# TACC/GraviT

Measured on AMD Instinct MI355X. Metric: Mrays/s (primary+shadow) at 1080p, 10M-tri scene, higher is better.
Workload: dtype f32; 1 GPU; soup-10000000: 10000000 random triangles (Philox seed 12345, half-extent 0.005), 1920x1080, eye (.5,.5,3)->(.5,.5,.5), fov 30deg, 1 point light at the eye, depth 1 (primary + 1 shadow ray), AO off; scheduler=image, 1 domain, harness=native, settle_frames=0, normal_mode=flat

## Files before the change

### gravit_amd/csrc/api.hip

```cpp
#include <atomic>
#include <chrono>
#include <cmath>
#include <cstdlib>
#include <condition_variable>
#include <functional>
#include <mutex>
#include <new>
#include <thread>

#include "gvt_internal.h"

size_t trav_spill_ints_per_thread();
int trav_block_threads();
void abi_pool_destroy(void *);

static thread_local std::string g_err;
static Ctx g_default_ctx;
static thread_local Ctx *tl_ctx = nullptr;
#define g_ctx (gctx())
Ctx &gctx() { return tl_ctx ? *tl_ctx : g_default_ctx; }

void set_error(const char *fmt, ...) {
  char buf[1024];
  va_list ap;
  va_start(ap, fmt);
  vsnprintf(buf, sizeof buf, fmt, ap);
  va_end(ap);
  g_err = buf;
}
extern "C" const char *gvt_hip_last_error(void) { return g_err.c_str(); }

static int ctx_setup(Ctx &C, int device) {
  int count = 0;
  if (hipGetDeviceCount(&count) != hipSuccess || count <= 0) { set_error("no HIP device visible"); return GVT_HIP_ERR_NODEVICE; }
  if (device < 0 || device >= count) { set_error("device %d out of range (%d visible)", device, count); return GVT_HIP_ERR_INVALID; }
  HIPCHK(hipSetDevice(device));
  hipDeviceProp_t prop;
  HIPCHK(hipGetDeviceProperties(&prop, device));
  if (std::strncmp(prop.gcnArchName, "gfx950", 6) != 0) {
    set_error("device %d is %s; this library carries gfx950 (MI355X) code objects only", device, prop.gcnArchName);
    return GVT_HIP_ERR_NODEVICE;
  }
  C.device = device;
  C.n_cu = prop.multiProcessorCount;
  HIPCHK(hipStreamCreateWithFlags(&C.own_stream, hipStreamNonBlocking));
  C.stream = C.own_stream;
  C.trav_blocks = std::max(C.n_cu, C.n_cu * 32 / (trav_block_threads() / 64));
  const size_t spill_ints = (size_t)C.trav_blocks * trav_block_threads() * trav_spill_ints_per_thread();
  HIPCHK(hipMalloc((void **)&C.d_spill, spill_ints * sizeof(int)));
  HIPCHK(hipMalloc((void **)&C.d_counters, CW_COUNT * sizeof(unsigned)));
  HIPCHK(hipMemset(C.d_counters, 0, CW_COUNT * sizeof(unsigned)));
  HIPCHK(hipHostMalloc((void **)&C.h_pinned, 64 * sizeof(unsigned), hipHostMallocDefault));
  std::memset(C.h_pinned, 0, 64 * sizeof(unsigned));
  C.ready = true;
  return 0;
}

static void drain_events();
static void warm_up() {
  if (getenv("GVT_HIP_NO_WARMUP")) return;
  const size_t nT = 2048;
  std::vector<float> v(nT * 9);
  std::vector<int32_t> t(nT * 3);
  uint32_t r = 12345u;
  for (size_t i = 0; i < nT; i++) {
    float c[3];
    for (int k = 0; k < 3; k++) { r = r * 1664525u + 1013904223u; c[k] = (float)(r >> 8) * (1.0f / 16777216.0f); }
    for (int j = 0; j < 3; j++)
      for (int k = 0; k < 3; k++) { r = r * 1664525u + 1013904223u; v[9 * i + 3 * j + k] = c[k] + ((float)(r >> 8) * (1.0f / 16777216.0f) - 0.5f) * 0.02f; }
    t[3 * i] = (int32_t)(3 * i); t[3 * i + 1] = (int32_t)(3 * i + 1); t[3 * i + 2] = (int32_t)(3 * i + 2);
  }
  gvt_hip_mesh *m = gvt_hip_mesh_create(v.data(), nT * 3, t.data(), nT, nullptr, nullptr, nullptr, 0, nullptr, nullptr);
  if (m) {
    float org[64 * 3], dir[64 * 3];
    gvt_hip_hit hits[64];
    int32_t occ[64];
    for (int i = 0; i < 64; i++) { org[3 * i] = (float)(i % 8) / 8.f; org[3 * i + 1] = (float)(i / 8) / 8.f; org[3 * i + 2] = 2.f; dir[3 * i] = 0.f; dir[3 * i + 1] = 0.f; dir[3 * i + 2] = -1.f; }
    gvt_hip_intersect(m, org, dir, 64, 0.f, hits);
    gvt_hip_occluded(m, org, dir, 64, 0.f, occ);
    gvt_hip_mesh_destroy(m);
  }
  Ctx &C = g_default_ctx;
  hipStreamSynchronize(C.stream);
  drain_events();
  C.stats = gvt_hip_stats{};
  set_error("%s", "");
}

extern "C" int gvt_hip_init(int device) {
  Ctx &C = g_default_ctx;
  if (C.ready && C.device == device) { if (!tl_ctx) HIPCHK(hipSetDevice(device)); return 0; }
  if (C.ready) { set_error("gvt_hip_init: already initialised on device %d", C.device); return GVT_HIP_ERR_INVALID; }
  const int rc = ctx_setup(C, device);
  if (!rc && !tl_ctx) warm_up();
  return rc;
}

extern "C" gvt_hip_ctx *gvt_hip_ctx_create(int device) {
  Ctx *C = new Ctx();
  if (ctx_setup(*C, device) != 0) { delete C; return nullptr; }
  return (gvt_hip_ctx *)C;
}
extern "C" int gvt_hip_ctx_make_current(gvt_hip_ctx *c) {
  tl_ctx = (Ctx *)c;
  Ctx &C = gctx();
  if (C.ready) HIPCHK(hipSetDevice(C.device));
  return 0;
}
extern "C" void gvt_hip_ctx_destroy(gvt_hip_ctx *c) {
  Ctx *C = (Ctx *)c;
  if (!C) return;
  if (tl_ctx == C) tl_ctx = nullptr;
  if (C->ready) {
    hipSetDevice(C->device);
    hipStreamSynchronize(C->stream);
    for (auto &p : C->pending) { hipEventDestroy(p.a); hipEventDestroy(p.b); }
    for (auto e : C->event_pool) hipEventDestroy(e);
    if (C->abi_qin) gvt_hip_queue_destroy(C->abi_qin);
    if (C->abi_qout) gvt_hip_queue_destroy(C->abi_qout);
    abi_pool_destroy(C->abi_pool); C->abi_pool = nullptr;
    for (Ctx *L : C->abi_lanes) gvt_hip_ctx_destroy((gvt_hip_ctx *)L);
    C->abi_lanes.clear();
    hipSetDevice(C->device);
    for (int k = 0; k < SCRATCH_COUNT; k++) if (C->scratch[k]) hipFree(C->scratch[k]);
    hipFree(C->d_spill); hipFree(C->d_counters); hipHostFree(C->h_pinned);
    if (C->h_wire) hipHostFree(C->h_wire);
    if (C->wire_ev) hipEventDestroy(C->wire_ev);
    hipStreamDestroy(C->own_stream);
  }
  delete C;
}

int ensure_init() {
  if (gctx().ready) return 0;
  return gvt_hip_init(0);
}

extern "C" int gvt_hip_set_stream(void *s) {
  if (ensure_init()) return GVT_HIP_ERR_NODEVICE;
  HIPCHK(hipStreamSynchronize(g_ctx.stream));
  g_ctx.stream = s ? (hipStream_t)s : g_ctx.own_stream;
  return 0;
}
extern "C" int gvt_hip_synchronize(void) {
  if (ensure_init()) return GVT_HIP_ERR_NODEVICE;
  HIPCHK(hipStreamSynchronize(g_ctx.stream));
  return 0;
}

void *scratch_get(ScratchSlot slot, size_t bytes) {
  Ctx &C = g_ctx;
  if (bytes <= C.scratch_bytes[slot] && C.scratch[slot]) return C.scratch[slot];
  hipStreamSynchronize(C.stream);
  if (C.scratch[slot]) hipFree(C.scratch[slot]);
  size_t want = bytes + bytes / 4 + 4096;
  C.scratch[slot] = nullptr;
  C.scratch_bytes[slot] = 0;
  if (hipMalloc(&C.scratch[slot], want) != hipSuccess) { set_error("scratch hipMalloc(%zu) failed", want); return nullptr; }
  C.scratch_bytes[slot] = want;
  return C.scratch[slot];
}

void scratch_release(ScratchSlot slot) {
  Ctx &C = g_ctx;
  if (!C.scratch[slot]) return;
  hipStreamSynchronize(C.stream);
  hipFree(C.scratch[slot]);
  C.scratch[slot] = nullptr;
  C.scratch_bytes[slot] = 0;
}

ProfScope::ProfScope(int c) : cls(c) {
  Ctx &C = g_ctx;
  if (!C.profile || (C.profile == 2 && c != KC_CLOSEST && c != KC_ANY && c != KC_LONG) || (C.profile == 3 && c != KC_CLOSEST) || (C.profile == 4 && c != KC_ANY)) return;
  auto take = [&]() {
    hipEvent_t e;
    if (!C.event_pool.empty()) { e = C.event_pool.back(); C.event_pool.pop_back(); }
    else hipEventCreate(&e);
    return e;
  };
  a = take(); b = take();
  hipEventRecord(a, C.stream);
}
ProfScope::~ProfScope() {
  Ctx &C = g_ctx;
  if (!a) return;
  hipEventRecord(b, C.stream);
  C.pending.push_back({ a, b, cls });
}
static void drain_events() {
  Ctx &C = g_ctx;
  for (auto &p : C.pending) {
    hipEventSynchronize(p.b);
    float ms = 0.f;
    hipEventElapsedTime(&ms, p.a, p.b);
    double *slot[KC_COUNT] = { &C.stats.ms_closest, &C.stats.ms_any, &C.stats.ms_shade, &C.stats.ms_convert, &C.stats.ms_shuffle,
                               &C.stats.ms_camera, &C.stats.ms_build, &C.stats.ms_sort, &C.stats.ms_long };
    *slot[p.cls] += ms;
    C.event_pool.push_back(p.a);
    C.event_pool.push_back(p.b);
  }
  C.pending.clear();
}
extern "C" int gvt_hip_profile(int enable) {
  if (ensure_init()) return GVT_HIP_ERR_NODEVICE;
  drain_events();
  g_ctx.profile = enable < 0 ? 0 : enable;
  return 0;
}
extern "C" int gvt_hip_stats_read(gvt_hip_stats *out) {
  if (!out) { set_error("stats_read: null"); return GVT_HIP_ERR_INVALID; }
  if (ensure_init()) return GVT_HIP_ERR_NODEVICE;
  HIPCHK(hipStreamSynchronize(g_ctx.stream));
  drain_events();
  *out = g_ctx.stats;
  return 0;
}
extern "C" int gvt_hip_stats_reset(void) {
  if (ensure_init()) return GVT_HIP_ERR_NODEVICE;
  drain_events();
  g_ctx.stats = gvt_hip_stats{};
  return 0;
}

namespace {
struct KnobDef { const char *name; int Knobs::*field; int lo, hi; bool shipped; };
const KnobDef g_knobs[] = {
  { "skip_known", &Knobs::skip_known, 0, 1, true },           { "frame_timing", &Knobs::frame_timing, 0, 1, true },
  { "term_sink", &Knobs::term_sink, 0, 1, true },
  { "sort_rays", &Knobs::sort_rays, 0, 1, true },             { "leaf_max", &Knobs::leaf_max, 1, 4, true },
  { "long_steps", &Knobs::long_steps, 0, 1 << 20, true },     { "small_rays", &Knobs::small_rays, 0, 1 << 30, true },
  { "finish_rays", &Knobs::finish_rays, 0, 1 << 30, true },   { "round_room_mb", &Knobs::round_room_mb, 0, 1 << 30, true },
  { "abi_lanes", &Knobs::abi_lanes_n, 0, 8, true },           { "abi_chunk", &Knobs::abi_chunk, 16384, 1 << 30, true },
  { "inject_fail_tick", &Knobs::inject_fail_tick, -1, 1 << 30, true },
  { "long_min_rays", &Knobs::long_min_rays, 0, 1 << 30, true }, { "long_auto", &Knobs::long_auto, 0, 1, true },
  { "finish_auto", &Knobs::finish_auto, 0, 1, true },
  { "payload_overlap_kb", &Knobs::payload_overlap_kb, 0, 1 << 30, true },
  { "packet", &Knobs::packet, 0, 2, true },                   { "packet_sah_max", &Knobs::packet_sah_max, 0, 1 << 30, true },
  { "packet_min_rays", &Knobs::packet_min_rays, 0, 1 << 30, true },
  { "shadow_order", &Knobs::shadow_order, 0, 1, true },       { "shadow_order_min_rays", &Knobs::shadow_order_min_rays, 0, 1 << 30, true },
  { "xcd_stripes", &Knobs::xcd_stripes, 0, 1, true },           { "early_deposit", &Knobs::early_deposit, 0, 1, true },

  { "inline_kb", &Knobs::inline_kb, 0, 1024, true },          { "comm_cus", &Knobs::comm_cus, 0, 128, true },
  { "comm_stream", &Knobs::comm_stream, 0, 1, true },         { "spec_ticks", &Knobs::spec_ticks, 0, 1, true },
  { "finish_clusters", &Knobs::finish_clusters, 0, 1, true }, { "hop_local", &Knobs::hop_local, 0, 3, true },
  { "occluder_chunk", &Knobs::occluder_chunk, 0, 1 << 24, true },
  { "blocks_per_cu", &Knobs::blocks_per_cu, 1, 8, false },    { "blocks_per_cu_closest", &Knobs::blocks_per_cu_closest, 0, 8, false },
  { "refill_min", &Knobs::refill_min, 1, 64, false },         { "inner_min", &Knobs::inner_min, 1, 64, false },
  { "share", &Knobs::share, 0, 1, false },                    { "share_min_rays", &Knobs::share_min_rays, 0, 1 << 30, false },
  { "sort_gather", &Knobs::sort_gather, 0, 1, false },        { "sort_bits", &Knobs::sort_bits, 8, 32, false },
  { "long_steps_drain", &Knobs::long_steps_drain, 0, 1 << 20, false }, { "long_save", &Knobs::long_save, 0, 1, false },
  { "lean_frame", &Knobs::lean_frame, 0, 1, false },          { "report_poll", &Knobs::report_poll, 0, 1, false },
  { "first_round_async", &Knobs::first_round_async, 0, 1, false }, { "wave_single", &Knobs::wave_single, 0, 1, false },
  { "shadow_direct", &Knobs::shadow_direct, 0, 1, false },    { "top_ordered", &Knobs::top_ordered, 0, 1, false },
  { "top_lds", &Knobs::top_lds, 0, 1, false },                { "camera_tile", &Knobs::camera_tile, 0, 8, false },
  { "abi_pipe_min", &Knobs::abi_pipe_min, 0, 1 << 30, false },
  { "shadow_cls_lo", &Knobs::shadow_cls_lo, 0, 255, false },  { "shadow_cls_shift", &Knobs::shadow_cls_shift, 0, 6, false },
};
}

extern "C" int gvt_hip_set_option(const char *name, int value) {
  if (!name) { set_error("set_option: null name"); return GVT_HIP_ERR_INVALID; }
  if (!std::strcmp(name, "defaults")) { static_cast<Knobs &>(g_ctx) = Knobs{}; return 0; }
  for (const KnobDef &k : g_knobs) {
    if (std::strcmp(name, k.name)) continue;
    if (value < k.lo || value > k.hi) { set_error("set_option: %s must be %d..%d", name, k.lo, k.hi); return GVT_HIP_ERR_INVALID; }
    if (!std::strcmp(name, "camera_tile") && value != 0 && value != 8) { set_error("camera_tile: 0 or 8"); return GVT_HIP_ERR_INVALID; }
#ifndef GVT_EXPERIMENTS
    if (!k.shipped && value != Knobs{}.*(k.field)) {
      set_error("set_option: %s=%d needs the experiments build of the library (libgvt_hip_exp.so); the shipped library carries its measured-best value %d", name, value,
                Knobs{}.*(k.field));
      return GVT_HIP_ERR_INVALID;
    }
#endif
    static_cast<Knobs &>(g_ctx).*(k.field) = value;
    return 0;
  }
  set_error("set_option: unknown option '%s'", name);
  return GVT_HIP_ERR_INVALID;
}

static void default_material(gvt_hip_material *m) {
  std::memset(m, 0, sizeof *m);
  m->type = 0;
  m->kd[0] = m->kd[1] = m->kd[2] = .5f;
  m->ks[0] = m->ks[1] = m->ks[2] = .5f;
  m->alpha = 1.f;
  m->eta[0] = .19f; m->eta[1] = 1.45f; m->eta[2] = 1.50f;
  m->k[0] = 3.06f; m->k[1] = 2.40f; m->k[2] = 1.88f;
  m->roughness = 0.05f;
}

static void generate_normals(const float *verts, size_t nV, const int32_t *tris, size_t nT, std::vector<float> &normals) {
  normals.assign(nV * 3, 0.0f);
  for (size_t i = 0; i < nT; i++) {
    int I = tris[3 * i], J = tris[3 * i + 1], K = tris[3 * i + 2];
    V3 a = ld3(verts + 3 * I), b = ld3(verts + 3 * J), c = ld3(verts + 3 * K);
    V3 u = sub3(b, a), v = sub3(c, a), n;
    n.x = u.y * v.z - u.z * v.y;
    n.y = u.z * v.x - u.x * v.z;
    n.z = u.x * v.y - u.y * v.x;
    n = norm3(n);
    int idx[3] = { I, J, K };
    for (int k = 0; k < 3; k++) {
      float *d = &normals[3 * idx[k]];
      d[0] += n.x; d[1] += n.y; d[2] += n.z;
    }
  }
  for (size_t i = 0; i < nV; i++) {
    V3 n = norm3(ld3(&normals[3 * i]));
    normals[3 * i] = n.x; normals[3 * i + 1] = n.y; normals[3 * i + 2] = n.z;
  }
}

template <typename T> static bool upload(T **dst, const T *src, size_t n) {
  *dst = nullptr;
  if (hipMalloc((void **)dst, sizeof(T) * (n ? n : 1)) != hipSuccess) return false;
  if (n && hipMemcpy(*dst, src, sizeof(T) * n, hipMemcpyHostToDevice) != hipSuccess) return false;
  return true;
}

extern "C" gvt_hip_mesh *gvt_hip_mesh_create(const float *verts, size_t nV, const int32_t *tris, size_t nT, const float *vnormals,
                                             const float *vcolors, const gvt_hip_material *materials, size_t nMat,
                                             const int32_t *face_mat, const gvt_hip_material *mesh_mat) {
  if (ensure_init()) return nullptr;
  if ((nV && !verts) || (nT && !tris)) { set_error("mesh_create: null vertex/triangle array"); return nullptr; }
  if (nT >= (1u << 28)) { set_error("mesh_create: %zu triangles exceed the 2^28 leaf-slot encoding", nT); return nullptr; }
  for (size_t i = 0; i < nT * 3; i++)
    if (tris[i] < 0 || (size_t)tris[i] >= nV) { set_error("mesh_create: triangle %zu references vertex %d (nV=%zu)", i / 3, tris[i], nV); return nullptr; }
  if (face_mat)
    for (size_t i = 0; i < nT; i++)
      if (face_mat[i] >= 0 && (size_t)face_mat[i] >= nMat) { set_error("mesh_create: face_mat[%zu]=%d out of range", i, face_mat[i]); return nullptr; }
  gvt_hip_mesh *M = new gvt_hip_mesh();
  M->nV = nV; M->nT = nT; M->nMat = materials ? nMat : 0;
  if (mesh_mat) M->mesh_mat = *mesh_mat; else default_material(&M->mesh_mat);
  std::vector<float> gen;
  const float *nrm = vnormals;
  if (!nrm) { generate_normals(verts, nV, tris, nT, gen); nrm = gen.data(); }
  bool ok = upload(&M->d_verts, verts, nV * 3) && upload(&M->d_tris, tris, nT * 3) && upload(&M->d_normals, nrm, nV * 3);
  if (ok && vcolors) ok = upload(&M->d_vcolors, vcolors, nV * 3);
  if (ok && M->nMat) ok = upload(&M->d_materials, materials, M->nMat);
  if (ok && face_mat && M->nMat) ok = upload(&M->d_face_mat, face_mat, nT);
  if (!ok) { set_error("mesh_create: device upload failed (%s)", hipGetErrorString(hipGetLastError())); gvt_hip_mesh_destroy(M); return nullptr; }
  if (build_lbvh(M) != 0) { gvt_hip_mesh_destroy(M); return nullptr; }
  return M;
}

extern "C" void gvt_hip_mesh_destroy(gvt_hip_mesh *M) {
  if (!M) return;
  if (g_ctx.ready) hipStreamSynchronize(g_ctx.stream);
  hipFree(M->d_verts); hipFree(M->d_tris); hipFree(M->d_normals); hipFree(M->d_vcolors); hipFree(M->d_materials);
  hipFree(M->d_face_mat); hipFree(M->d_nodes); hipFree(M->d_tri); hipFree(M->d_slot_of); hipFree(M->d_nodes4); hipFree(M->d_nodes4c);
  refit_tables_free(M);
  delete M;
}

extern "C" int gvt_hip_mesh_update_vertices(gvt_hip_mesh *M, const float *verts, size_t nV, const float *vnormals, uint32_t flags, float *ms_out) {
  if (ensure_init()) return GVT_HIP_ERR_NODEVICE;
  if (!M) { set_error("mesh_update_vertices: null mesh"); return GVT_HIP_ERR_INVALID; }
  if (flags & ~GVT_HIP_UPDATE_DEVICE) { set_error("mesh_update_vertices: unknown flags 0x%x", flags); return GVT_HIP_ERR_INVALID; }
  if (nV != M->nV) { set_error("mesh_update_vertices: %zu vertices given, the mesh has %zu (topology changes need a new mesh)", nV, M->nV); return GVT_HIP_ERR_INVALID; }
  if (nV && !verts) { set_error("mesh_update_vertices: null vertex array"); return GVT_HIP_ERR_INVALID; }
  Ctx &C = g_ctx;
  hipStream_t st = C.stream;
  const hipMemcpyKind kind = (flags & GVT_HIP_UPDATE_DEVICE) ? hipMemcpyDeviceToDevice : hipMemcpyHostToDevice;
  if (nV) {
    HIPCHK(hipMemcpyAsync(M->d_verts, verts, sizeof(float) * 3 * nV, kind, st));
    if (vnormals) HIPCHK(hipMemcpyAsync(M->d_normals, vnormals, sizeof(float) * 3 * nV, kind, st));
  }
  hipEvent_t e0, e1;
  HIPCHK(hipEventCreate(&e0));
  if (hipEventCreate(&e1) != hipSuccess) { hipEventDestroy(e0); set_error("mesh_update_vertices: hipEventCreate failed"); return GVT_HIP_ERR_DEVICE; }
  int rc = hipEventRecord(e0, st) == hipSuccess ? 0 : GVT_HIP_ERR_DEVICE;
  if (!rc && nV && !vnormals) rc = regen_normals(M);
  if (!rc) rc = refit_lbvh(M);
  float ms = 0.f;
  if (!rc && (hipEventRecord(e1, st) != hipSuccess || hipEventSynchronize(e1) != hipSuccess || hipEventElapsedTime(&ms, e0, e1) != hipSuccess)) {
    set_error("mesh_update_vertices: %s", hipGetErrorString(hipGetLastError()));
    rc = GVT_HIP_ERR_DEVICE;
  }
  hipStreamSynchronize(st);
  hipEventDestroy(e0); hipEventDestroy(e1);
  if (!rc && ms_out) *ms_out = ms;
  return rc;
}

extern "C" int gvt_hip_mesh_get_info(const gvt_hip_mesh *M, gvt_hip_mesh_info *o) {
  if (!M || !o) { set_error("mesh_get_info: null"); return GVT_HIP_ERR_INVALID; }
  std::memset(o, 0, sizeof *o);
  o->n_tris = M->nT; o->n_verts = M->nV; o->n_nodes = M->nNodes; o->n_leaves = M->nLeaves;
  for (int k = 0; k < 3; k++) { o->bbox_lo[k] = M->lo[k]; o->bbox_hi[k] = M->hi[k]; }
  o->build_ms = M->build_ms; o->max_leaf = M->leaf_max; o->packet = M->packet_ok ? 1u : 0u; o->sah_inner = M->sah_inner;
  o->bytes_nodes = M->nNodes * sizeof(BvhNode) + M->nNodes4 * 64; o->bytes_tris = M->nT * 64;
  return 0;
}
extern "C" int gvt_hip_mesh_get_normals(const gvt_hip_mesh *M, float *out) {
  if (!M || !out) { set_error("mesh_get_normals: null"); return GVT_HIP_ERR_INVALID; }
  HIPCHK(hipMemcpy(out, M->d_normals, sizeof(float) * 3 * M->nV, hipMemcpyDeviceToHost));
  return 0;
}

int queue_reserve(gvt_hip_queue *q, size_t cap) {
  if (cap <= q->cap) return 0;
  Ctx &C = g_ctx;
  size_t ncap = cap + cap / 8 + 1024;
  if (ncap >= 0xffffffffull) { set_error("queue_reserve: %zu rays exceed the 32-bit slot counter", ncap); return GVT_HIP_ERR_INVALID; }
  float4 *np = nullptr;
  HIPCHK(hipMalloc((void **)&np, GVT_QUEUE_BYTES_PER_RAY * ncap));
  if (q->size) {
    for (int k = 0; k < 4; k++)
      HIPCHK(hipMemcpyAsync(np + (size_t)k * ncap, q->d_planes + (size_t)k * q->cap, sizeof(float4) * q->size, hipMemcpyDeviceToDevice, C.stream));
    HIPCHK(hipMemcpyAsync(np + 4 * ncap, q->d_planes + 4 * q->cap, sizeof(uint32_t) * q->size, hipMemcpyDeviceToDevice, C.stream));
    HIPCHK(hipMemcpyAsync((uint32_t *)(np + 4 * ncap) + ncap, (const uint32_t *)(q->d_planes + 4 * q->cap) + q->cap, 3 * sizeof(uint32_t) * q->size, hipMemcpyDeviceToDevice, C.stream));
  }
  HIPCHK(hipStreamSynchronize(C.stream));
  if (q->d_planes) HIPCHK(hipFree(q->d_planes));
  q->d_planes = np;
  q->cap = ncap;
  return 0;
}

extern "C" gvt_hip_queue *gvt_hip_queue_create(size_t capacity) {
  if (ensure_init()) return nullptr;
  gvt_hip_queue *q = new gvt_hip_queue();
  if (hipMalloc((void **)&q->d_count, 64) != hipSuccess || hipMemset(q->d_count, 0, 64) != hipSuccess) {
    set_error("queue_create: hipMalloc failed"); delete q; return nullptr;
  }
  if (capacity && queue_reserve(q, capacity) != 0) { gvt_hip_queue_destroy(q); return nullptr; }
  return q;
}
extern "C" void gvt_hip_queue_destroy(gvt_hip_queue *q) {
  if (!q) return;
  if (g_ctx.ready) hipStreamSynchronize(g_ctx.stream);
  hipFree(q->d_planes); hipFree(q->d_count);
  delete q;
}
extern "C" int gvt_hip_queue_reserve(gvt_hip_queue *q, size_t cap) {
  if (!q) { set_error("queue_reserve: null"); return GVT_HIP_ERR_INVALID; }
  return queue_reserve(q, cap);
}
extern "C" int gvt_hip_queue_clear(gvt_hip_queue *q) {
  if (!q) { set_error("queue_clear: null"); return GVT_HIP_ERR_INVALID; }
  q->size = 0;
  HIPCHK(hipMemsetAsync(q->d_count, 0, sizeof(unsigned), g_ctx.stream));
  return 0;
}
extern "C" int gvt_hip_queue_size(gvt_hip_queue *q, size_t *n) {
  if (!q || !n) { set_error("queue_size: null"); return GVT_HIP_ERR_INVALID; }
  *n = q->size;
  return 0;
}
extern "C" int gvt_hip_queue_sizes(gvt_hip_queue *const *queues, size_t n, uint64_t *out) {
  if ((n && !queues) || !out) { set_error("queue_sizes: null"); return GVT_HIP_ERR_INVALID; }
  for (size_t i = 0; i < n; i++) out[i] = queues[i] ? queues[i]->size : 0;
  return 0;
}

extern "C" int gvt_hip_abi_version(void) { return GVT_HIP_ABI_VERSION; }

extern "C" int gvt_hip_queue_append(gvt_hip_queue *q, const gvt_hip_ray *rays, size_t n, int src_on_device) {
  if (src_on_device != 0 && src_on_device != 1) {
    set_error("queue_append: the 4th argument is the boolean src_on_device (0 / 1), got %d; flag words go to gvt_hip_queue_append_flags", src_on_device);
    return GVT_HIP_ERR_INVALID;
  }
  return gvt_hip_queue_append_flags(q, rays, n, src_on_device ? (GVT_HIP_APPEND_DEVICE | GVT_HIP_APPEND_KEEP_STATE) : 0);
}
extern "C" int gvt_hip_queue_append_flags(gvt_hip_queue *q, const gvt_hip_ray *rays, size_t n, int flags) {
  if (!q || (n && !rays)) { set_error("queue_append: null"); return GVT_HIP_ERR_INVALID; }
  if (flags & ~(GVT_HIP_APPEND_DEVICE | GVT_HIP_APPEND_KEEP_STATE)) { set_error("queue_append: unknown flag bits %d", flags); return GVT_HIP_ERR_INVALID; }
  const int src_on_device = flags & GVT_HIP_APPEND_DEVICE;
  if (!n) return 0;
  Ctx &C = g_ctx;
  int rc = queue_reserve(q, q->size + n);
  if (rc) return rc;
  const gvt_hip_ray *d_src = rays;
  if (!src_on_device) {
    void *stage = scratch_get(SCR_GENERAL, sizeof(gvt_hip_ray) * n);
    if (!stage) return GVT_HIP_ERR_DEVICE;
    HIPCHK(hipMemcpyAsync(stage, rays, sizeof(gvt_hip_ray) * n, hipMemcpyHostToDevice, C.stream));
    d_src = (const gvt_hip_ray *)stage;
  }
  rc = convert_aos_to_planes(d_src, n, make_planes(q->d_planes, q->cap), q->size, (flags & GVT_HIP_APPEND_KEEP_STATE) != 0);
  if (rc) return rc;
  q->size += n;
  if ((rc = set_device_u32(q->d_count, (unsigned)q->size))) return rc;
  if (!src_on_device) HIPCHK(hipStreamSynchronize(C.stream));
  return 0;
}

extern "C" int gvt_hip_queue_export(gvt_hip_queue *q, gvt_hip_ray *dst, size_t cap, size_t *n, int dst_on_device) {
  if (!q || !n) { set_error("queue_export: null"); return GVT_HIP_ERR_INVALID; }
  *n = q->size;
  if (q->size > cap) { set_error("queue_export: %zu rays, capacity %zu", q->size, cap); return GVT_HIP_ERR_CAPACITY; }
  if (!q->size) return 0;
  if (!dst) { set_error("queue_export: null destination"); return GVT_HIP_ERR_INVALID; }
  Ctx &C = g_ctx;
  gvt_hip_ray *d_dst = dst;
  if (!dst_on_device) {
    d_dst = (gvt_hip_ray *)scratch_get(SCR_GENERAL, sizeof(gvt_hip_ray) * q->size);
    if (!d_dst) return GVT_HIP_ERR_DEVICE;
  }
  int rc = convert_planes_to_aos(make_planes(q->d_planes, q->cap), 0, q->size, d_dst);
  if (rc) return rc;
  if (!dst_on_device) HIPCHK(hipMemcpyAsync(dst, d_dst, sizeof(gvt_hip_ray) * q->size, hipMemcpyDeviceToHost, C.stream));
  HIPCHK(hipStreamSynchronize(C.stream));
  return 0;
}

static int fill_params(TraceParams &P, const float m[16], const float minv[16], const float normi[9], size_t n_lights, int normal_mode,
                       uint32_t seed, const gvt_hip_light *lights) {
  if (!m || !minv || !normi) { set_error("trace: null matrix"); return GVT_HIP_ERR_INVALID; }
  if (n_lights && !lights) { set_error("trace: null lights"); return GVT_HIP_ERR_INVALID; }
  if (n_lights > 64) { set_error("trace: %zu lights (max 64)", n_lights); return GVT_HIP_ERR_INVALID; }
  if (normal_mode != GVT_HIP_NORMALS_FLAT && normal_mode != GVT_HIP_NORMALS_SMOOTH) { set_error("trace: bad normal_mode %d", normal_mode); return GVT_HIP_ERR_INVALID; }
  std::memcpy(P.m.m, m, 64); std::memcpy(P.minv.m, minv, 64); std::memcpy(P.normi.n, normi, 36);
  P.normal_mode = normal_mode; P.seed = seed; P.n_lights = (int)n_lights;
  P.sink = TermSink{};
  P.update_in_place = 1;
  P.carried_rng = 0;
  return 0;
}

extern "C" int gvt_hip_trace_queue(gvt_hip_mesh *M, gvt_hip_queue *q_in, gvt_hip_queue *q_out, const float m[16], const float minv[16],
                                   const float normi[9], const gvt_hip_light *lights, size_t n_lights, int normal_mode, uint32_t seed) {
  return gvt_hip_trace_queue_sink(M, q_in, q_out, m, minv, normi, lights, n_lights, normal_mode, seed, nullptr, -1, nullptr);
}

extern "C" int gvt_hip_trace_queue_sink(gvt_hip_mesh *M, gvt_hip_queue *q_in, gvt_hip_queue *q_out, const float m[16], const float minv[16],
                                        const float normi[9], const gvt_hip_light *lights, size_t n_lights, int normal_mode, uint32_t seed,
                                        gvt_hip_top *top, int from_inst, gvt_hip_fb *fb) {
  if (ensure_init()) return GVT_HIP_ERR_NODEVICE;
  if (!M || !q_in || !q_out || q_in == q_out) { set_error("trace_queue: null or aliased queue"); return GVT_HIP_ERR_INVALID; }
  TraceParams P;
  int rc = fill_params(P, m, minv, normi, n_lights, normal_mode, seed, lights);
  if (rc) return rc;
  if (top && fb && g_ctx.term_sink) {
    P.sink.top = top->dev(); P.sink.from = from_inst;
    P.sink.fb = fb->d_rgba; P.sink.n_pix = (unsigned)(fb->w * fb->h);
  }
  const size_t n = q_in->size;
  rc = queue_reserve(q_out, q_out->size + n * (1 + n_lights));
  if (rc) return rc;
  P.update_in_place = 0;
  P.carried_rng = 1;
// ... 337 lines not shown
```

### gravit_amd/csrc/finish_kernel.inc

```
struct FinishArgs {
  WaveSet W;
  unsigned n;
  const gvt_hip_light *lights;
  int n_lights, normal_mode;
  TopDev top;
  float *fb;
  unsigned n_pix;
  const QueueDesc *queues;
  const int *owner;
  int rank;
  unsigned *counter;
  unsigned long long *tot;
  unsigned *queue_overflow;
  unsigned *trav_overflow;
  uint32_t seed;
  unsigned long long index_base;
  int skip_known;
  unsigned *const *count_ptr;
  const unsigned char *clear_mask;
  int n_inst;
  const unsigned *n_dev;
  const unsigned *valid;
};

__device__ __forceinline__ int uni(int x) { return __builtin_amdgcn_readfirstlane(x); }
__device__ __forceinline__ unsigned uni(unsigned x) { return (unsigned)__builtin_amdgcn_readfirstlane((int)x); }
__device__ __forceinline__ float uni(float x) { return __int_as_float(__builtin_amdgcn_readfirstlane(__float_as_int(x))); }
__device__ __forceinline__ V3 uni(V3 v) { return mk3(uni(v.x), uni(v.y), uni(v.z)); }
__device__ __forceinline__ void uni_ray(RayRec &r) {
  r.o = uni(r.o); r.t_min = uni(r.t_min); r.d = uni(r.d); r.t_max = uni(r.t_max); r.c = uni(r.c); r.t = uni(r.t);
  r.id = uni(r.id); r.depth = uni(r.depth); r.w = uni(r.w); r.type = uni(r.type); r.rng = uni(r.rng);
  r.km[0] = uni(r.km[0]); r.km[1] = uni(r.km[1]); r.km[2] = uni(r.km[2]);
}

#define FIN_CAP 384
#define FIN_PHYS (FIN_CAP + 256)
template <int CAP, int PHYS>
__device__ inline void wave_closest(const uint4 *__restrict__ nodes4, const uint4 *__restrict__ nodes4c, int root_entry, const float4 *__restrict__ tris, V3 O, V3 D, float tnear,
                                    const WaveLists &L, float &bt, int &bp, float &bu, float &bv, float &bden, unsigned *ovf_word) {
  bt = GVT_FLT_MAX; bu = 0.f; bv = 0.f; bden = 1.f; bp = -1;
  if (lane_id() == 0) { L.s_ref[0] = nodes4c ? root_entry : 0; L.s_tn[0] = 0.f; }
  __builtin_amdgcn_wave_barrier();
  if (nodes4c) wave_run<false, true, CAP, PHYS>(nodes4c, tris, O, D, slab_of(O, D), tnear, L, 1, 0, bt, bp, bu, bv, bden, ovf_word);
  else wave_run<false, false, CAP, PHYS>(nodes4, tris, O, D, slab_of(O, D), tnear, L, nodes4 ? 1 : 0, 0, bt, bp, bu, bv, bden, ovf_word);
  bt = uni(bt); bp = uni(bp); bu = uni(bu); bv = uni(bv); bden = uni(bden);
}
template <int CAP, int PHYS>
__device__ inline bool wave_any(const uint4 *__restrict__ nodes4, const uint4 *__restrict__ nodes4c, int root_entry, const float4 *__restrict__ tris, V3 O, V3 D, float tnear,
                                volatile int *s_ref, volatile int *l_ref, unsigned *ovf_word) {
  if (nodes4c) return wave_any_run<true, CAP, PHYS>(nodes4c, root_entry, tris, O, D, slab_of(O, D), tnear, s_ref, l_ref, ovf_word);
  return wave_any_run<false, CAP, PHYS>(nodes4, 0, tris, O, D, slab_of(O, D), tnear, s_ref, l_ref, ovf_word);
}

__global__ __launch_bounds__(256, 4) void k_finish(FinishArgs A) {
  __shared__ int s_ref_all[4][FIN_PHYS];
  __shared__ float s_tn_all[4][FIN_PHYS];
  __shared__ int l_ref_all[4][FIN_PHYS];
  __shared__ float l_tn_all[4][FIN_PHYS];
  const int wv = threadIdx.x >> 6;
  const int lane = (int)lane_id();
  volatile int *s_ref = s_ref_all[wv];
  volatile float *s_tn = s_tn_all[wv];
  volatile int *l_ref = l_ref_all[wv];
  volatile float *l_tn = l_tn_all[wv];
  const WaveLists L = { s_ref, s_tn, l_ref, l_tn };
  if (A.valid && !*A.valid) return;
  const unsigned n_rays = A.n_dev ? *A.n_dev : A.n;
  if (blockIdx.x == 0 && A.count_ptr)
    for (int i = threadIdx.x; i < A.n_inst; i += 256)
      if (A.clear_mask[i]) *A.count_ptr[i] = 0u;
  bool first = true;
  unsigned n_closest = 0, n_any = 0;
  auto move_on = [&](RayRec &r, int from, int &next) -> int {
    float ret_t;
    bool walked = false;
    float4 ra = make_float4(r.o.x, r.o.y, r.o.z, r.t_min);
    const float4 rb = make_float4(r.d.x, r.d.y, r.d.z, r.t_max);
    if (A.skip_known) {
      next = shuffle_walk(ra, rb, A.top, from, r.km, ret_t, walked);
      walked = uni((int)walked) != 0;
      if (walked) r.o = uni(mk3(ra.x, ra.y, ra.z));
      r.km[0] = uni(r.km[0]); r.km[1] = uni(r.km[1]); r.km[2] = uni(r.km[2]);
    } else next = top_nearest(ra, rb, A.top, from, ret_t);
    next = uni(next); ret_t = uni(ret_t);
    if (next < 0) {
      if (lane == 0) deposit_shadow(A.fb, A.n_pix, r.type, r.c, r.w, (unsigned)r.id);
      return 0;
    }
    if (!walked) r.o = uni(add3(r.o, scl3(r.d, ret_t * 0.95f)));
    if (A.rank < 0 || A.owner[next] == A.rank) return 1;
    if (lane == 0) {
      const QueueDesc Q = A.queues[next];
      const unsigned slot = atomicAdd(Q.count, 1u);
      if (slot < Q.cap) store_ray(make_planes(Q.planes, Q.cap), slot, r);
      else atomicOr(A.queue_overflow, 1u);
    }
    return 2;
  };
  for (;;) {
    const unsigned g = wave_ticket(first, A.counter, wv);
    if (g >= n_rays) break;
    const WaveSeg sg = A.W.segs[wave_find_seg(A.W, g)];
    RayRec r = load_ray(make_planes(sg.planes, sg.cap), g - sg.begin);
    uni_ray(r);
    int inst = uni(sg.inst);
    bool fresh = true;
    for (;;) {
      const WaveInst *wi = A.W.insts + inst;
      float bt, bu, bv, bden;
      int bp;
      wave_closest<FIN_CAP, FIN_PHYS>(wi->nodes4, wi->nodes4c, wi->root_entry4c, wi->tris, xfm_point(wi->minv, r.o), xfm_vector(wi->minv, r.d), GVT_RAY_EPSILON, L, bt, bp, bu, bv, bden, A.trav_overflow);
      n_closest++;
      if (bp < 0) {
        int next;
        if (move_on(r, inst, next) != 1) break;
        inst = next; fresh = true;
        continue;
      }
      if (r.type == 1) break;
      const float hu = bu / bden, hv = bv / bden;
      uint32_t g_seed = (fresh && r.rng == 0u) ? ray_stream_seed(A.seed, A.index_base + (uint64_t)g) : r.rng;
      fresh = false;
      const MeshView *M = &wi->mv;
      float t = bt;
      r.t = t;
      const float4 *sl = M->slots + 4 * (size_t)M->slot_of[bp];
      const float4 q0 = sl[0], q1 = sl[1], q2 = sl[2], q3 = sl[3];
      const V3 v0 = mk3(q0.x, q0.y, q0.z), v1 = mk3(q1.w, q2.w, q3.x), v2 = mk3(q3.y, q3.z, q3.w);
      int ia = 0, ib = 0, ic = 0;
      if (A.normal_mode == GVT_HIP_NORMALS_SMOOTH || M->vcolors) { ia = M->tris[3 * bp]; ib = M->tris[3 * bp + 1]; ic = M->tris[3 * bp + 2]; }
      const V3 negNg = cross3(sub3(v1, v0), sub3(v2, v0));
      const V3 normalflat = norm3(mat3_mul(wi->normi, negNg));
      V3 N;
      if (A.normal_mode == GVT_HIP_NORMALS_SMOOTH) {
        const V3 a = ld3(M->normals + 3 * ib), b = ld3(M->normals + 3 * ic), c = ld3(M->normals + 3 * ia);
        const V3 mn = add3(add3(scl3(a, hu), scl3(b, hv)), scl3(c, 1.0f - hu - hv));
        N = norm3(mat3_mul(wi->normi, mn));
      } else N = normalflat;
      if (dot3(neg3(r.d), normalflat) <= 0.f) N = neg3(N);
      MatEval me = mat_eval(M->mat);
      if (M->vcolors) {
        const V3 c0 = ld3(M->vcolors + 3 * ia), c1 = ld3(M->vcolors + 3 * ib), c2 = ld3(M->vcolors + 3 * ic);
        me.kd = add3(add3(scl3(c0, 1.f - hu - hv), scl3(c1, hu)), scl3(c2, hv));
        me.type = 0; me.ks = mk3(.5f, .5f, .5f); me.alpha = 1.f;
      } else if (M->face_mat && M->face_mat[bp] >= 0 && (unsigned)M->face_mat[bp] < M->n_mat) {
        me = mat_eval(M->materials[M->face_mat[bp]]);
      }
      if (r.type == 2) {
        t = (t > 1) ? 1.f / t : t;
        r.w = r.w * t;
      }
      N = uni(N); r.w = uni(r.w); r.t = uni(r.t); g_seed = uni(g_seed);
      me.type = uni(me.type); me.kd = uni(me.kd); me.ks = uni(me.ks); me.alpha = uni(me.alpha); me.eta = uni(me.eta); me.k = uni(me.k);
      me.roughness = uni(me.roughness); me.hsc = uni(me.hsc); me.back = uni(me.back); me.falloff = uni(me.falloff);
      for (int li = 0; li < A.n_lights; li++) {
        const gvt_hip_light L = A.lights[li];
        const V3 lightPos = (L.type == GVT_HIP_LIGHT_AREA) ? area_light_position(L, g_seed) : ld3(L.position);
        V3 c;
        if (!shade(me, r, N, L, lightPos, c)) continue;
        RayRec s;
        const float multiplier = 1.0f - GVT_RAY_EPSILON * 16;
        const float t_shadow = multiplier * r.t;
        const V3 origin = add3(r.o, scl3(r.d, t_shadow));
        const V3 dir = sub3(lightPos, origin);
        s.o = origin; s.t_min = GVT_RAY_EPSILON;
        s.d = norm3(dir);
        s.t_max = 3.0f;
        s.c = c; s.t = r.t;
        s.id = r.id; s.depth = r.depth; s.w = r.w; s.type = 1;
        s.rng = 0u;
        s.km[0] = 0u; s.km[1] = 0u; s.km[2] = 0u;
        uni_ray(s);
        g_seed = uni(g_seed);
        n_any++;
        if (wave_any<FIN_CAP, FIN_PHYS>(wi->nodes4, wi->nodes4c, wi->root_entry4c, wi->tris, xfm_point(wi->minv, s.o), xfm_vector(wi->minv, s.d), GVT_RAY_EPSILON, s_ref, l_ref, A.trav_overflow)) continue;
        int s_inst = inst;
        for (;;) {
          int next;
          if (move_on(s, s_inst, next) != 1) break;
          s_inst = next;
          const WaveInst *wj = A.W.insts + s_inst;
          n_closest++;
          if (wave_any<FIN_CAP, FIN_PHYS>(wj->nodes4, wj->nodes4c, wj->root_entry4c, wj->tris, xfm_point(wj->minv, s.o), xfm_vector(wj->minv, s.d), GVT_RAY_EPSILON, s_ref, l_ref, A.trav_overflow)) break;
        }
      }
      const int ndepth = r.depth - 1;
      const float p = 1.f - gvt_fastrand01(g_seed);
      if (!(ndepth > 0 && r.w > p)) break;
      r.type = 2;
      const float multiplier = 1.0f - 16.0f * GVT_FLT_EPSILON;
      const float t_secondary = multiplier * r.t;
      r.o = add3(r.o, scl3(r.d, t_secondary));
      const V3 nd = cos_weighted_dir(N, g_seed);
      r.d = nd;
      r.w = r.w * dot3(nd, N);
      r.depth = ndepth;
      r.rng = g_seed;
      r.km[0] = 0u; r.km[1] = 0u; r.km[2] = 0u;
      uni_ray(r);
    }
    __builtin_amdgcn_wave_barrier();
  }
  if (lane == 0 && (n_closest || n_any)) { atomicAdd(A.tot + TOT_CLOSEST, (unsigned long long)n_closest); atomicAdd(A.tot + TOT_ANY, (unsigned long long)n_any); }
}
```

### gravit_amd/csrc/gvt_internal.h

```cpp
#pragma once
#include <hip/hip_runtime.h>

#include <cstdarg>
#include <cstdio>
#include <cstring>
#include <string>
#include <vector>

#include "gvt_device.h"

enum KernelClass { KC_CLOSEST = 0, KC_ANY, KC_SHADE, KC_CONVERT, KC_SHUFFLE, KC_CAMERA, KC_BUILD, KC_SORT, KC_LONG, KC_COUNT };

struct PendingEvent {
  hipEvent_t a, b;
  int cls;
};

#define SHADOW_CLASSES 8
static_assert(CW_SHADOW_CLS + SHADOW_CLASSES <= CW_PEEK, "the class counts are read through gvt_hip_counters_peek");
static_assert(CW_SHADOW_CLS + SHADOW_CLASSES <= CW_COUNT && CW_PEEK <= CW_COUNT, "every named counter word lies inside the allocation");

enum ScratchSlot {
  SCR_GENERAL,
  SCR_SHADOW,
  SCR_IDX_A,
  SCR_IDX_B,
  SCR_LIGHTS,
  SCR_NEXT_INST,
  SCR_NEXT_T,
  SCR_SORT_KEYS_IN, SCR_SORT_KEYS_OUT, SCR_SORT_VALS_IN, SCR_SORT_VALS_OUT,
  SCR_SORT_TEMP, SCR_SORT_GATHER,
  SCR_BLOCK_COUNTS,
  SCR_LONG,
  SCR_SHADOW_INST, SCR_OUT_FROM,
  SCR_PKT_RETRY,
  SCR_STEPS,
  SCR_VOL_WORK, SCR_VOL_OVF,
  SCR_VOL_RANGES,
  SCR_BUILD,
  SCR_HOP,
  SCR_WIRE_TABLE,
  SCR_VOL_KEEP,
  SCR_VOL_BRICKS, SCR_VOL_FUSED,
  SCR_VOL_GRIDS,
  SCR_VOL_OCC_RAYS, SCR_VOL_OCC,
  SCR_VOL_GHOSTS,
  SCR_VOL_AMR,
  SCRATCH_COUNT
};
struct Knobs {
  int blocks_per_cu = 4;
  int blocks_per_cu_closest = 5;
  int refill_min = 16;
  int inner_min = 32;
  int share = 1;
  int share_min_rays = 131072;
  int sort_rays = 0;
  int sort_gather = 0;
  int sort_bits = 20;
  int long_steps = 96;
  int long_steps_drain = 0;
  int long_save = 1;
  int long_min_rays = 65536;
  int packet = 1;
  int shadow_order = 1;
  int shadow_cls_lo = 24, shadow_cls_shift = 3;
  int xcd_stripes = 1;
  int early_deposit = 1;
  int shadow_order_min_rays = 262144;
  int packet_min_rays = 524288;
  int packet_sah_max = 128;
  int round_room_mb = 16384;
  int finish_rays = 32768;
  int finish_auto = 1;
  int small_rays = 4096;
  int abi_lanes_n = 4;
  int abi_chunk = 262144;
  int abi_pipe_min = 131072;
  int lean_frame = 1;
  int skip_known = 0;
  int long_auto = 1;
  int payload_overlap_kb = 1024;
  int inline_kb = 16;
  int comm_cus = 0;
  int hop_local = 1;
  int finish_clusters = 1;
  int spec_ticks = 1;
  int comm_stream = 0;
  int frame_timing = 0;
  int inject_fail_tick = -1;
  int report_poll = 1;
  int first_round_async = 1;
  int wave_single = 1;
  int shadow_direct = 1;
  int term_sink = 1;
  int camera_tile = 8;
  int top_ordered = 1;
  int top_lds = 1;
  int leaf_max = 2;
  int occluder_chunk = 0;
};

struct Ctx : Knobs {
  bool ready = false;
  int device = -1;
  hipStream_t own_stream = nullptr;
  hipStream_t stream = nullptr;
  int profile = 0;
  int long_steps_override = 0;
  std::vector<PendingEvent> pending;
  std::vector<hipEvent_t> event_pool;
  gvt_hip_stats stats{};
  int n_cu = 256;
  uint64_t early_deposit_launches = 0;
  bool shadow_order_denied = false;
  int cu_reserved = 0;
  int trav_blocks = 0;
  int *d_spill = nullptr;
  unsigned *d_counters = nullptr;
  unsigned *h_pinned = nullptr;
  void *h_wire = nullptr;
  hipEvent_t wire_ev = nullptr;
  bool wire_busy = false;
  void *scratch[SCRATCH_COUNT] = { nullptr };
  size_t scratch_bytes[SCRATCH_COUNT] = { 0 };
  std::vector<unsigned char> lights_cached;
  const void *lights_cached_dst = nullptr;
  gvt_hip_queue *abi_qin = nullptr, *abi_qout = nullptr;
  std::vector<Ctx *> abi_lanes;
  void *abi_pool = nullptr;
};
Ctx &gctx();
void set_error(const char *fmt, ...);
int ensure_init();
inline bool staging_queues(Ctx &C) {
  if (!C.abi_qin) { C.abi_qin = gvt_hip_queue_create(0); C.abi_qout = gvt_hip_queue_create(0); }
  return C.abi_qin && C.abi_qout;
}
void *scratch_get(ScratchSlot slot, size_t bytes);
void scratch_release(ScratchSlot slot);

#define HIPCHK(expr)                                                                              \
  do {                                                                                            \
    hipError_t _e = (expr);                                                                       \
    if (_e != hipSuccess) {                                                                       \
      set_error("%s failed: %s (%s:%d)", #expr, hipGetErrorString(_e), __FILE__, __LINE__);       \
      return GVT_HIP_ERR_DEVICE;                                                                  \
    }                                                                                             \
  } while (0)

struct ProfScope {
  int cls;
  hipEvent_t a = nullptr, b = nullptr;
  explicit ProfScope(int cls);
  ~ProfScope();
};

struct gvt_hip_mesh {
  size_t nV = 0, nT = 0;
  float *d_verts = nullptr;
  int *d_tris = nullptr;
  float *d_normals = nullptr;
  float *d_vcolors = nullptr;
  gvt_hip_material *d_materials = nullptr;
  size_t nMat = 0;
  int *d_face_mat = nullptr;
  gvt_hip_material mesh_mat;
  BvhNode *d_nodes = nullptr;
  size_t nNodes = 0;
  float4 *d_tri = nullptr;
  unsigned *d_slot_of = nullptr;
  uint4 *d_nodes4 = nullptr;
  size_t nNodes4 = 0;
  std::vector<unsigned> levels4;
  uint4 *d_nodes4c = nullptr;
  int root_entry4c = 0;
  int leaf_max = 2;
  size_t nLeaves = 0;
  float lo[3] = { 0, 0, 0 }, hi[3] = { 0, 0, 0 };
  float build_ms = 0.f;
  float sah_inner = 0.f;
  bool packet_ok = false;
  uint2 *d_range2 = nullptr;
  uint2 *d_range4 = nullptr;
  unsigned *d_vlist = nullptr;
  unsigned *d_vstart = nullptr;
};

struct gvt_hip_queue {
  float4 *d_planes = nullptr;
  size_t cap = 0;
  size_t size = 0;
  unsigned *d_count = nullptr;
};

struct gvt_hip_top {
  size_t n = 0;
  std::vector<int> order;
  std::vector<float> h_lo, h_hi;
  float4 *d_lo = nullptr;
  float4 *d_hi = nullptr;
  float4 *d_nlo = nullptr, *d_nhi = nullptr;
  size_t n_nodes = 0;
  TopDev dev() const { return TopDev{ d_lo, d_hi, (int)n, d_nlo, d_nhi, (int)n_nodes }; }
  unsigned *d_hist = nullptr;
  void **d_qdesc = nullptr;
  unsigned *h_hist = nullptr;
  void *h_qdesc = nullptr;
  std::vector<unsigned char> qdesc_uploaded;
};

struct gvt_hip_fb {
  int w = 0, h = 0;
  float *d_rgba = nullptr;
};

struct gvt_hip_depth {
  int w = 0, h = 0;
  float *d_t = nullptr;
};

struct QueueDesc {
  float4 *planes;
  unsigned long long cap;
  unsigned *count;
  unsigned keep;
};

struct TermSink {
  TopDev top;
  int from;
  float *fb;
  unsigned n_pix;
};
struct TraceParams {
  Mat4 m, minv;
  Mat3 normi;
  int normal_mode;
  uint32_t seed;
  int n_lights;
  TermSink sink;
  int update_in_place;
  int carried_rng;
  int hop;
  const int *hop_owner;
  int hop_rank;
  int one_writer;
};

struct MeshView {
  const float4 *slots;
  const unsigned *slot_of;
  const float *verts;
  const int *tris;
  const float *normals;
  const float *vcolors;
  const gvt_hip_material *materials;
  unsigned n_mat;
  const int *face_mat;
  gvt_hip_material mat;
};

struct WaveSeg {
  float4 *planes;
  unsigned long long cap;
  unsigned begin, n;
  int inst, pad;
};
struct WaveInst {
  Mat4 minv;
  Mat3 normi;
  int root_entry4c;
  int pad[2];
  const uint4 *nodes4;
  const float4 *tris;
  const uint4 *nodes4c;
  MeshView mv;
};
struct WaveSet {
  const WaveSeg *segs;
  const WaveInst *insts;
  int n_seg;
  alignas(8) int n_inst;
};

int build_lbvh(gvt_hip_mesh *M);
int trav_overflow_fetch_async();
int trav_overflow_result();
int build_nodes4(gvt_hip_mesh *M);
int build_nodes4c(gvt_hip_mesh *M);
int refit_lbvh(gvt_hip_mesh *M);
int regen_normals(gvt_hip_mesh *M);
void refit_tables_free(gvt_hip_mesh *M);
int sort_pairs_u32(unsigned *keys_in, unsigned *keys_out, unsigned *vals_in, unsigned *vals_out, size_t n, int end_bit);
int queue_reserve(gvt_hip_queue *q, size_t cap);
int trace_core(gvt_hip_mesh *M, RayPlanes in, size_t n, uint64_t index_base, gvt_hip_queue *out, const TraceParams &P,
               const gvt_hip_light *lights_host);
int launch_closest(gvt_hip_mesh *M, RayPlanes q, const unsigned *idx, size_t n, bool xform, const Mat4 &minv, float tnear,
                   gvt_hip_hit *d_hits, bool counter_is_zero = false);
int launch_visit_stats(gvt_hip_mesh *M, RayPlanes q, size_t n, float tnear, unsigned *d_out);
int launch_wide_visit_stats(gvt_hip_mesh *M, RayPlanes q, size_t n, float tnear, const unsigned char *d_marks, unsigned *d_out);
int wide_root_marks(gvt_hip_mesh *M, int width, unsigned char *d_marks, size_t *n_wide);
int launch_any_flags(gvt_hip_mesh *M, RayPlanes q, size_t n, bool xform, const Mat4 &minv, float tnear, int *d_flags);
int set_device_u32(unsigned *p, unsigned v);
#define PINNED_STAGE_BYTES (32 * 1024)
int pinned_stage_begin(void **h);
int pinned_stage_end();
struct WaveSingle {
  RayPlanes planes;
  gvt_hip_mesh *mesh;
  Mat4 minv;
  Mat3 normi;
  int inst;
  int coherent;
  unsigned row_rays;
  const unsigned *n_dev;
  int pass0_begun;
};
struct ChainOpts {
  unsigned *const *d_count_ptr = nullptr;
  const unsigned char *d_mask = nullptr;
  int n_inst = 0;
  bool defer_end = false;
  const unsigned *n_dev0_multi = nullptr;
  bool multi_packets = false;
  bool simple_meshes = false;
};
int wave_trace_chain(const WaveSet &W, size_t n_total, int passes, gvt_hip_queue *out, int *d_out_from, const TraceParams &P,
                     const gvt_hip_light *lights_host, const WaveSingle *single, const ChainOpts &O);
int finish_round(const WaveSet &W, size_t n_total, const TraceParams &P, const gvt_hip_light *lights_host, const void *d_qdesc, const int *d_owner, int rank,
                 unsigned *d_queue_overflow, unsigned *const *d_count_ptr, const unsigned char *d_mask, const unsigned *spec_words = nullptr);
bool finish_lights_resident(const gvt_hip_light *lights_host, int nL);
MeshView mesh_view(const gvt_hip_mesh *M);
bool walks_packets(const Ctx &C, const gvt_hip_mesh *M, size_t n);
bool plain_lambert(const gvt_hip_mesh *M);
bool no_area_light(const gvt_hip_light *lights, int nL);
int convert_aos_to_planes(const gvt_hip_ray *d_src, size_t n, RayPlanes dst, size_t dst_off, bool keep_state);
int convert_planes_to_aos(RayPlanes src, size_t src_off, size_t n, gvt_hip_ray *d_dst);
int convert_od_to_planes(const float *d_org, const float *d_dir, size_t n, RayPlanes dst);
```

### gravit_amd/csrc/packet_kernel.inc

```
#define PKT_STACK 128
#define PKT_MAX_STEPS 2048

template <bool ANY>
__device__ __forceinline__ bool packet_walk(const uint4 *__restrict__ nodes4, const float4 *__restrict__ tris, V3 O, V3 D, float tnear, bool live, float &bt, int &bp,
                                             float &bu, float &bv, float &bden, bool &active) {
  const float dx = fabsf(D.x) < 1e-30f ? copysignf(1e-30f, D.x) : D.x;
  const float dy = fabsf(D.y) < 1e-30f ? copysignf(1e-30f, D.y) : D.y;
  const float dz = fabsf(D.z) < 1e-30f ? copysignf(1e-30f, D.z) : D.z;
  const float ix = 1.0f / dx, iy = 1.0f / dy, iz = 1.0f / dz;
  const float ox = O.x * ix, oy = O.y * iy, oz = O.z * iz;
  bt = GVT_FLT_MAX; bu = 0.f; bv = 0.f; bden = 1.f;
  bp = -1;
  active = live;
  int stk0 = 0, stk1 = 0;
  int sp = 0;
  int cur = nodes4 ? 0 : TRAV_DONE;
  int steps = 0;
  bool bail = false;
#define PK_PUSH(REF)                                                                                                   \
  {                                                                                                                    \
    if (sp < 64) stk0 = ((int)lane_id() == sp) ? (REF) : stk0;                                                         \
    else if (sp < PKT_STACK) stk1 = ((int)lane_id() == sp - 64) ? (REF) : stk1;                                         \
    else bail = true;                                                                                                  \
    if (sp < PKT_STACK) sp++;                                                                                          \
  }
#define PK_POP()                                                                                                       \
  {                                                                                                                    \
    if (sp == 0) cur = TRAV_DONE;                                                                                      \
    else { sp--; cur = sp < 64 ? __builtin_amdgcn_readlane(stk0, sp) : __builtin_amdgcn_readlane(stk1, sp - 64); }     \
  }
  while (cur != TRAV_DONE && !bail) {
    if (++steps > PKT_MAX_STEPS) { bail = true; break; }
    if (cur >= 0) {
      const uint4 *nd = nodes4 + (size_t)GVT_NODE4_F4 * (size_t)cur;
      float tn[4];
      int rr[4];
      node4_test(nd, make_slab(ix, iy, iz, ox, oy, oz), ANY ? GVT_FLT_MAX : bt, tn, rr);
      float key[4];
      int ref[4];
#pragma unroll
      for (int c = 0; c < 4; c++) {
        const unsigned long long m = __ballot(active && tn[c] < GVT_FLT_MAX);
        ref[c] = __builtin_amdgcn_readfirstlane(rr[c]);
        key[c] = m ? __builtin_amdgcn_readlane(tn[c], __ffsll((long long)m) - 1) : GVT_FLT_MAX;
      }
#define PK_CE(A_, B_) { const bool sw_ = key[B_] < key[A_]; const float ka_ = sw_ ? key[B_] : key[A_], kb_ = sw_ ? key[A_] : key[B_]; \
                        const int ra_ = sw_ ? ref[B_] : ref[A_], rb_ = sw_ ? ref[A_] : ref[B_]; key[A_] = ka_; key[B_] = kb_; ref[A_] = ra_; ref[B_] = rb_; }
      PK_CE(0, 1) PK_CE(2, 3) PK_CE(0, 2) PK_CE(1, 3) PK_CE(1, 2)
#undef PK_CE
      int nxt = TRAV_DONE;
      bool have = false;
#pragma unroll
      for (int c = 3; c >= 0; c--) {
        if (key[c] < GVT_FLT_MAX) {
          if (have) PK_PUSH(nxt)
          nxt = ref[c]; have = true;
        }
      }
      if (have) cur = nxt;
      else PK_POP()
    } else {
      const unsigned code = (unsigned)~cur;
      const unsigned first = code >> 3, ntri = code & 7u;
      const float4 *ts = tris + 4 * (size_t)first;
      for (unsigned k = 0; k < ntri; k++) {
        const float4 s0 = ts[4 * k], s1 = ts[4 * k + 1], s2 = ts[4 * k + 2];
        if (active) {
          const V3 e1 = mk3(s1.x, s1.y, s1.z), e2 = mk3(s2.x, s2.y, s2.z);
          float TT, U, V, aden;
          if (tri_test_raw(O, D, mk3(s0.x, s0.y, s0.z), e1, e2, cross3(e1, e2), tnear, TT, U, V, aden)) {
            const float t = TT / aden;
            if (t <= GVT_FLT_MAX) {
              if (ANY) { bp = 0; active = false; }
              else {
                const int prim = __float_as_int(s0.w);
                if (bp < 0 || t < bt || (t == bt && prim < bp)) { bt = t; bp = prim; bu = U; bv = V; bden = aden; }
              }
            }
          }
        }
      }
      if (ANY && !__ballot(active)) break;
      PK_POP()
    }
  }
#undef PK_PUSH
#undef PK_POP
  return bail;
}

template <bool ANY>
__global__ __launch_bounds__(256) void k_packet(RayPlanes q, unsigned n, const unsigned *__restrict__ n_dev, Mat4 minv, Trav T, float tnear,
                                                 gvt_hip_hit *__restrict__ hits, const int *__restrict__ valid, RayPlanes out, unsigned *out_count,
                                                 TermSink sink, LongQ LQ, unsigned *__restrict__ retry_idx, unsigned *retry_count,
                                                 unsigned long long *tot_any, unsigned *bail_count) {
  __shared__ unsigned pend_all[4 * 64];
  volatile unsigned *pend = &pend_all[(threadIdx.x >> 6) * 64];
  if (n_dev) n = *n_dev;
  const unsigned p = blockIdx.x * 4u + (threadIdx.x >> 6);
  const unsigned j = p * 64u + lane_id();
  bool live = j < n && (!ANY || !valid || valid[j] >= 0);
  if (!__ballot(live)) return;
  V3 O = mk3(0, 0, 0), D = mk3(0, 0, 1);
  if (live) {
    const float4 a = q.p0[j], b = q.p1[j];
    O = xfm_point(minv, mk3(a.x, a.y, a.z)); D = xfm_vector(minv, mk3(b.x, b.y, b.z));
  }
  float bt, bu, bv, bden;
  int bp;
  bool active;
  const bool bail = packet_walk<ANY>(T.nodes4, T.tris, O, D, tnear, live, bt, bp, bu, bv, bden, active);
  const unsigned n_live = (unsigned)__popcll(__ballot(live));
  if (ANY && tot_any && lane_id() == 0) atomicAdd(tot_any, (unsigned long long)n_live);
  if (bail) {
    if (ANY) {
      const unsigned slot = wave_alloc(retry_count, active);
      if (active) retry_idx[slot] = j;
    } else {
      const unsigned slot = wave_alloc(LQ.count, live);
      if (live) { LongRec R; R.j = j; R.i = j; R.bt = bt; R.bp = bp; R.bu = bu; R.bv = bv; R.bden = bden; R.ns = 0u; LQ.recs[slot] = R; }
    }
    if (lane_id() == 0) atomicAdd(bail_count, 1u);
    return;
  }
  if (!ANY) {
    if (live) { gvt_hip_hit h; h.t = bt; h.prim = bp; h.u = (bp >= 0) ? bu / bden : 0.f; h.v = (bp >= 0) ? bv / bden : 0.f; hits[j] = h; }
    return;
  }
  const bool survive = live && bp < 0;
  const unsigned long long sm = __ballot(survive);
  if (sm) {
    if (survive) pend[lanes_below(sm)] = j;
    flush_pending(pend, __popcll(sm), q, out, out_count, sink);
  }
}

__global__ __launch_bounds__(256) void k_packet_multi(WaveSet W, unsigned n, const unsigned *__restrict__ n_dev, float tnear, gvt_hip_hit *__restrict__ hits, LongQ LQ,
                                                       unsigned *bail_count) {
  if (n_dev) n = *n_dev;
  const unsigned p = blockIdx.x * 4u + (threadIdx.x >> 6);
  const unsigned j0 = p * 64u;
  if (j0 >= n) return;
  const unsigned j = j0 + lane_id();
  const int s_lo = wave_find_seg(W, j0), s_hi = wave_find_seg(W, min(j0 + 63u, n - 1u));
  for (int sgi = s_lo; sgi <= s_hi; sgi++) {
    const WaveSeg sg = W.segs[sgi];
    const bool live = j < n && j >= sg.begin && j - sg.begin < sg.n;
    if (!__ballot(live)) continue;
    const WaveInst *wi = W.insts + sg.inst;
    V3 O = mk3(0, 0, 0), D = mk3(0, 0, 1);
    if (live) {
      const unsigned local = j - sg.begin;
      const float4 a = sg.planes[local], b = sg.planes[sg.cap + local];
      O = xfm_point(wi->minv, mk3(a.x, a.y, a.z)); D = xfm_vector(wi->minv, mk3(b.x, b.y, b.z));
    }
    float bt, bu, bv, bden;
    int bp;
    bool active;
    const bool bail = packet_walk<false>(wi->nodes4, wi->tris, O, D, tnear, live, bt, bp, bu, bv, bden, active);
    if (bail) {
      const unsigned slot = wave_alloc(LQ.count, live);
      if (live) { LongRec R; R.j = j; R.i = j; R.bt = bt; R.bp = bp; R.bu = bu; R.bv = bv; R.bden = bden; R.ns = 0u; LQ.recs[slot] = R; }
      if (lane_id() == 0) atomicAdd(bail_count, 1u);
    } else if (live) { gvt_hip_hit h; h.t = bt; h.prim = bp; h.u = (bp >= 0) ? bu / bden : 0.f; h.v = (bp >= 0) ? bv / bden : 0.f; hits[j] = h; }
  }
}
```

### gravit_amd/csrc/shade.inc

```
__device__ inline V3 light_contribution(const gvt_hip_light &L, V3 hit, V3 samplePos) {
  V3 c = ld3(L.color);
  if (L.type == GVT_HIP_LIGHT_AMBIENT) return c;
  V3 p = (L.type == GVT_HIP_LIGHT_AREA) ? samplePos : ld3(L.position);
  float distance = 1.f / len3(sub3(p, hit));
  distance = (distance > 1.f) ? 1.f : distance;
  return scl3(c, distance);
}

__device__ inline V3 area_light_position(const gvt_hip_light &L, uint32_t &seed) {
  V3 v = ld3(L.normal), u, w;
  if (v.x == 0.f && v.y == 1.f && v.z == 0.f) {
    u = mk3(1, 0, 0); w = mk3(0, 0, 1);
  } else {
    const V3 up = mk3(0, 1, 0);
    u.x = up.y * v.z - v.y * up.z; u.y = up.z * v.x - v.z * up.x; u.z = up.x * v.y - v.x * up.y;
    w.x = v.y * u.z - u.y * v.z; w.y = v.z * u.x - u.z * v.x; w.z = v.x * u.y - u.x * v.y;
  }
  float xLocation = (float)(((double)gvt_fastrand_lcg(seed, 0, 1) - 0.5) * (double)L.width);
  float zLocation = (float)(((double)gvt_fastrand_lcg(seed, 0, 1) - 0.5) * (double)L.height);
  float xCoord = xLocation * u.x + zLocation * w.x;
  float yCoord = xLocation * u.y + zLocation * w.y;
  float zCoord = xLocation * u.z + zLocation * w.z;
  return mk3(L.position[0] + xCoord, L.position[1] + yCoord, L.position[2] + zCoord);
}

struct MatEval {
  int type;
  V3 kd, ks;
  float alpha;
  V3 eta, k;
  float roughness;
  V3 hsc;
  float back, falloff;
};
__device__ inline MatEval mat_eval(const gvt_hip_material &m) {
  MatEval e;
  e.type = m.type; e.kd = ld3(m.kd); e.ks = ld3(m.ks); e.alpha = m.alpha; e.eta = ld3(m.eta); e.k = ld3(m.k); e.roughness = m.roughness;
  e.hsc = ld3(m.horizonScatteringColor); e.back = m.backScattering; e.falloff = m.horizonScatteringFallOff;
  return e;
}
__device__ inline float clamp01(float x) { const float a = (x < 0.f) ? 0.f : x; return (1.f < a) ? 1.f : a; }

template <bool LAMBERT = false>
__device__ inline bool shade(const MatEval &m, const RayRec &ray, V3 N, const gvt_hip_light &L, V3 lightPos, V3 &out) {
  const int mtype = LAMBERT ? 0 : m.type;
  const V3 kd = m.kd, ks = m.ks;
  const float alpha = m.alpha;
  V3 hitPoint = add3(ray.o, scl3(ray.d, ray.t));
  V3 wi = norm3(sub3(lightPos, hitPoint));
  float dNw = dot3(N, wi);
  float NdotL = (0.f < dNw) ? dNw : 0.f;
  V3 Li = light_contribution(L, hitPoint, lightPos);
  if (NdotL == 0.f || (Li.x == 0.f && Li.y == 0.f && Li.z == 0.f)) return false;
  V3 color;
  if (mtype == 0) {
    color = scl3(kd, NdotL * ray.w);
  } else if (mtype == 1) {
    V3 R = sub3(scl3(scl3(N, 2.f), NdotL), wi);
    float vr = dot3(R, neg3(ray.d));
    float VdotR = (0.f < vr) ? vr : 0.f;
    float power = VdotR * powf(VdotR, alpha);
    color = scl3(kd, NdotL * ray.w);
    color = add3(color, scl3(ks, power * ray.w));
  } else if (mtype == 2) {
    V3 H = norm3(sub3(wi, ray.d));
    float hn = dot3(H, N);
    float NdotH = (0.f < hn) ? hn : 0.f;
    float power = NdotH * powf(NdotH, alpha);
    V3 diffuse = scl3(kd, NdotL * ray.w);
    V3 specular = scl3(ks, power * ray.w);
    color = add3(diffuse, specular);
  } else if (mtype >= 3 && mtype <= 5) {
    const V3 wo = neg3(ray.d);
    const float one_over_pi = 0.31830988618379069122f;
    V3 r = mk3(0, 0, 0);
    if (mtype == 5) {
      r = scl3(kd, clamp01(dot3(wi, N)));
    } else if (mtype == 4) {
      const float cosThetaI = clamp01(dot3(wi, N));
      const float backScatter = powf(clamp01(dot3(wo, wi)), m.back);
      const V3 a = scl3(ks, backScatter * cosThetaI * one_over_pi);
      const float cosThetaO = clamp01(dot3(wo, N));
      const float sinThetaO = sqrtf(1.0f - cosThetaO * cosThetaO);
      const float horizonScatter = powf(sinThetaO, m.falloff);
      const V3 b = scl3(m.hsc, horizonScatter * cosThetaI * one_over_pi);
      r = add3(a, b);
    } else {
      const float expo = 1.0f / m.roughness;
      const float cosThetaO = dot3(wo, N), cosThetaI = dot3(wi, N);
      if (!(cosThetaI <= 0.0f || cosThetaO <= 0.0f)) {
        const V3 s_ = add3(wi, wo);
        const V3 wh = scl3(s_, 1.0f / sqrtf(dot3(s_, s_)));
        const float cosThetaH = dot3(wh, N);
        const float cosTheta = dot3(wi, wh);
        const float cosi = cosTheta, c2 = cosi * cosi;
        const V3 tmp = add3(mul3(m.eta, m.eta), mul3(m.k, m.k));
        const V3 two_eta_c = scl3(scl3(m.eta, 2.0f), cosi);
        const V3 one = mk3(1.0f, 1.0f, 1.0f), vc2 = mk3(c2, c2, c2);
        const V3 num1 = add3(sub3(scl3(tmp, c2), two_eta_c), one), den1 = add3(add3(scl3(tmp, c2), two_eta_c), one);
        const V3 num2 = add3(sub3(tmp, two_eta_c), vc2), den2 = add3(add3(tmp, two_eta_c), vc2);
        const V3 Rpar = mk3(num1.x / den1.x, num1.y / den1.y, num1.z / den1.z);
        const V3 Rper = mk3(num2.x / den2.x, num2.y / den2.y, num2.z / den2.z);
        const V3 F = scl3(add3(Rpar, Rper), 0.5f);
        const float D = (expo + 2) * (1.0f / (2.0f * 3.14159265358979323846f)) * powf(fabsf(cosThetaH), expo);
        const float g1 = 2.0f * cosThetaH * cosThetaO / cosTheta, g2 = 2.0f * cosThetaH * cosThetaI / cosTheta;
        const float gm = (g1 < g2) ? g1 : g2;
        const float G = (1.0f < gm) ? 1.0f : gm;
        r = scl3(scl3(scl3(mul3(ks, F), D), G), 1.0f / (4.0f * cosThetaO));
      }
    }
    color = scl3(scl3(r, 2.f), ray.w);
  } else {
    color = mk3(0, 0, 0);
  }
  color = mul3(color, Li);
  float c[3] = { color.x, color.y, color.z };
  for (int i = 0; i < 3; i++) {
    float a = (c[i] < 0.f) ? 0.f : c[i];
    c[i] = (1.f < a) ? 1.f : a;
  }
  out = mk3(c[0], c[1], c[2]);
  return true;
}

__device__ inline V3 cos_weighted_dir(V3 n, uint32_t &seed) {
  float Xi1 = gvt_fastrand01(seed);
  float Xi2 = gvt_fastrand01(seed);
  float theta = (float)gvt_acos(__builtin_sqrt(1.0 - (double)Xi1));
  float phi = (float)(2.0 * 3.1415926535897932384626433832795 * (double)Xi2);
  float xs = gvt_sinf(theta) * gvt_cosf(phi);
  float ys = gvt_cosf(theta);
  float zs = gvt_sinf(theta) * gvt_sinf(phi);
  V3 y = n, h = y;
  if (fabsf(h.x) <= fabsf(h.y) && fabsf(h.x) <= fabsf(h.z)) h.x = 1.0f;
  else if (fabsf(h.y) <= fabsf(h.x) && fabsf(h.y) <= fabsf(h.z)) h.y = 1.0f;
  else h.z = 1.0f;
  V3 x = cross3(h, y);
  V3 z = cross3(x, y);
  V3 d = add3(add3(scl3(x, xs), scl3(y, ys)), scl3(z, zs));
  return norm3(d);
}

struct ShadeArgs {
  RayPlanes in;
  const unsigned *idx;
  unsigned n;
  unsigned long long index_base;
  const gvt_hip_hit *hits;
  int first_pass;
  int carried_rng;
  RayPlanes out; unsigned *out_count;
  RayPlanes shadow; unsigned *shadow_count;
  unsigned *next_idx; unsigned *next_count;
  const gvt_hip_light *lights;
  Mat3 normi;
  int normal_mode, n_lights;
  uint32_t seed;
  unsigned *zero_word;
  TermSink sink;
  int update_in_place;
  const unsigned *n_dev;
  WaveSet W;
  const int *hop_inst;
  int *out_from;
  int *shadow_inst;
  unsigned shadow_stride;
  const unsigned char *steps;
  unsigned *cls_cnt;
  unsigned cls_stride;
  int cls_lo, cls_shift;
  int early_deposit;
};

__device__ __forceinline__ void store_shadow_early(const ShadeArgs &A, unsigned slot, const RayRec &s) {
  A.shadow.p0[slot] = make_float4(s.o.x, s.o.y, s.o.z, s.t_min);
  A.shadow.p1[slot] = make_float4(s.d.x, s.d.y, s.d.z, s.t_max);
  const bool dep = len3(s.c) > 0.f && (unsigned)s.id < A.sink.n_pix;
  if (dep) {
    const V3 cw = scl3(s.c, s.w);
    ((float4 *)A.sink.fb)[(unsigned)s.id] = make_float4(0.0f + cw.x, 0.0f + cw.y, 0.0f + cw.z, 1.0f);
  }
  ((uint32_t *)A.shadow.p2)[slot] = dep ? (uint32_t)s.id : 0xffffffffu;
}

__device__ __forceinline__ unsigned shadow_class(int steps, int lo, int shift) {
  const int c = (steps - lo) >> shift;
  return (unsigned)(c < 0 ? 0 : (c > SHADOW_CLASSES - 1 ? SHADOW_CLASSES - 1 : c));
}

#define SHADE_BLOCK 512
template <bool MULTI, bool LEAN = false>
__global__ __launch_bounds__(SHADE_BLOCK, 4) void k_shade(ShadeArgs A, MeshView M1) {
  __shared__ unsigned sh_alloc[2 * (2 + 64)];
  __shared__ unsigned sh_cls[2 * SHADOW_CLASSES];
  for (int k = threadIdx.x; k < 2 * (2 + 64); k += SHADE_BLOCK) sh_alloc[k] = 0u;
  if (threadIdx.x < 2 * SHADOW_CLASSES) sh_cls[threadIdx.x] = 0u;
  __syncthreads();
  const unsigned j = blockIdx.x * blockDim.x + threadIdx.x;
  if (j == 0 && A.zero_word) *A.zero_word = 0u;
  const unsigned n = A.n_dev ? *A.n_dev : A.n;
  const bool in_range = j < n;
  __shared__ unsigned sh_wcls[SHADE_BLOCK / 64];
  if (!MULTI && A.cls_cnt) {
    int st = in_range ? (int)A.steps[j] : 0;
    for (int o = 32; o >= 1; o >>= 1) st = max(st, __shfl_xor(st, o));
    if (lane_id() == 0) sh_wcls[threadIdx.x >> 6] = shadow_class(st, A.cls_lo, A.cls_shift);
  }
  unsigned i = in_range ? (A.idx ? A.idx[j] : j) : 0u;
  const unsigned gi = i;
  RayPlanes in = A.in;
  const MeshView *M = &M1;
  Mat3 normi = A.normi;
  int inst = A.sink.from;
  if (MULTI && in_range) {
    const WaveSeg sg = A.W.segs[wave_find_seg(A.W, i)];
    in = make_planes(sg.planes, sg.cap);
    i -= sg.begin;
    inst = sg.inst;
    if (A.hop_inst) { const int h_ = A.hop_inst[gi]; if (h_ >= 0) inst = h_; }
    M = &A.W.insts[inst].mv;
    normi = A.W.insts[inst].normi;
  }
  RayRec r;
  gvt_hip_hit h;
  h.prim = -1; h.t = 0.f; h.u = 0.f; h.v = 0.f;
  bool miss = false, shaded = false, bounce = false;
  uint32_t g_seed = 0;
  V3 N = mk3(0, 0, 0);
  MatEval me = mat_eval(M->mat);
  if (in_range) {
    r = load_ray(in, i);
    h = A.hits[j];
    if (!LEAN) g_seed = (A.first_pass && (!A.carried_rng || r.rng == 0u)) ? ray_stream_seed(A.seed, A.index_base + gi) : r.rng;
    if (h.prim < 0) {
      miss = true;
    } else if (r.type != 1) {
      shaded = true;
      float t = h.t;
      r.t = t;
      const float4 *sl = M->slots + 4 * (size_t)M->slot_of[h.prim];
      const float4 s0 = sl[0], s1 = sl[1], s2 = sl[2], s3 = sl[3];
      const V3 v0 = mk3(s0.x, s0.y, s0.z), v1 = mk3(s1.w, s2.w, s3.x), v2 = mk3(s3.y, s3.z, s3.w);
      int ia = 0, ib = 0, ic = 0;
      if (A.normal_mode == GVT_HIP_NORMALS_SMOOTH || (!LEAN && M->vcolors)) { ia = M->tris[3 * h.prim]; ib = M->tris[3 * h.prim + 1]; ic = M->tris[3 * h.prim + 2]; }
      const V3 negNg = cross3(sub3(v1, v0), sub3(v2, v0));
      const V3 normalflat = norm3(mat3_mul(normi, negNg));
      if (A.normal_mode == GVT_HIP_NORMALS_SMOOTH) {
        const V3 a = ld3(M->normals + 3 * ib), b = ld3(M->normals + 3 * ic), c = ld3(M->normals + 3 * ia);
        const V3 mn = add3(add3(scl3(a, h.u), scl3(b, h.v)), scl3(c, 1.0f - h.u - h.v));
        N = norm3(mat3_mul(normi, mn));
      } else {
        N = normalflat;
      }
      if (dot3(neg3(r.d), normalflat) <= 0.f) N = neg3(N);
      if (LEAN) {
      } else if (M->vcolors) {
        const V3 c0 = ld3(M->vcolors + 3 * ia), c1 = ld3(M->vcolors + 3 * ib), c2 = ld3(M->vcolors + 3 * ic);
        me.kd = add3(add3(scl3(c0, 1.f - h.u - h.v), scl3(c1, h.u)), scl3(c2, h.v));
        me.type = 0; me.ks = mk3(.5f, .5f, .5f); me.alpha = 1.f;
      } else if (M->face_mat && M->face_mat[h.prim] >= 0 && (unsigned)M->face_mat[h.prim] < M->n_mat) {
        me = mat_eval(M->materials[M->face_mat[h.prim]]);
      }
      if (r.type == 2) {
        t = (t > 1) ? 1.f / t : t;
        r.w = r.w * t;
      }
    }
  }
  if (!(LEAN && !MULTI)) {
    bool forward = miss;
    if (miss && A.sink.fb) {
      float ret_t;
      const float4 a = make_float4(r.o.x, r.o.y, r.o.z, r.t_min), b = make_float4(r.d.x, r.d.y, r.d.z, r.t_max);
      if (top_nearest(a, b, A.sink.top, inst, ret_t) < 0) {
        forward = false;
        deposit_shadow(A.sink.fb, A.sink.n_pix, r.type, r.c, r.w, (unsigned)r.id);
      }
    }
    const unsigned slot = block_alloc(A.out_count, forward, &sh_alloc[0]);
    if (forward) { store_ray(A.out, slot, r); if (MULTI) A.out_from[slot] = inst; }
  }
  for (int li = 0; li < A.n_lights; li++) {
    bool emit = false;
    RayRec s;
    if (shaded) {
      const gvt_hip_light L = A.lights[li];
      const V3 lightPos = (!LEAN && L.type == GVT_HIP_LIGHT_AREA) ? area_light_position(L, g_seed) : ld3(L.position);
      V3 c;
      if (shade<LEAN>(me, r, N, L, lightPos, c)) {
        emit = true;
        const float multiplier = 1.0f - GVT_RAY_EPSILON * 16;
        const float t_shadow = multiplier * r.t;
        const V3 origin = add3(r.o, scl3(r.d, t_shadow));
        const V3 dir = sub3(lightPos, origin);
        s.o = origin; s.t_min = GVT_RAY_EPSILON;
        s.d = norm3(dir);
        s.t_max = 3.0f;
        s.c = c; s.t = r.t;
        s.id = r.id; s.depth = r.depth; s.w = r.w; s.type = 1;
        s.rng = 0u;
        s.km[0] = 0u; s.km[1] = 0u; s.km[2] = 0u;
      }
    }
    if (A.shadow_stride) {
      if (j < A.shadow_stride) {
        const unsigned slot = (unsigned)li * A.shadow_stride + j;
        A.shadow_inst[slot] = emit ? (MULTI ? inst : 0) : -1;
        if (emit) store_ray(A.shadow, slot, s);
      }
    } else if (!MULTI && A.cls_cnt) {
      const unsigned cls = (unsigned)__builtin_amdgcn_readfirstlane((int)sh_wcls[threadIdx.x >> 6]);
      const unsigned long long mask = ballot64(emit);
      unsigned woff = 0;
      if (mask) {
        if ((int)lane_id() == __ffsll((long long)mask) - 1) woff = atomicAdd(&sh_cls[cls], (unsigned)__popcll(mask));
        woff = (unsigned)__builtin_amdgcn_readlane((int)woff, __ffsll((long long)mask) - 1);
      }
      __syncthreads();
      if (threadIdx.x < SHADOW_CLASSES && sh_cls[threadIdx.x]) sh_cls[SHADOW_CLASSES + threadIdx.x] = atomicAdd(&A.cls_cnt[threadIdx.x], sh_cls[threadIdx.x]);
      __syncthreads();
      if (emit) {
        const unsigned slot = cls * A.cls_stride + sh_cls[SHADOW_CLASSES + cls] + woff + lanes_below(mask);
        if (LEAN && A.early_deposit) store_shadow_early(A, slot, s);
        else store_ray(A.shadow, slot, s);
      }
    } else {
      const unsigned slot = block_alloc(A.shadow_count, emit, &sh_alloc[2 * (2 + li)]);
      if (emit) {
        if (LEAN && !MULTI && A.early_deposit) store_shadow_early(A, slot, s);
        else store_ray(A.shadow, slot, s);
        if (MULTI) A.shadow_inst[slot] = inst;
      }
    }
  }
  if (!LEAN && shaded) {
    const int ndepth = r.depth - 1;
    const float p = 1.f - gvt_fastrand01(g_seed);
    if (ndepth > 0 && r.w > p) {
      r.type = 2;
      const float multiplier = 1.0f - 16.0f * GVT_FLT_EPSILON;
      const float t_secondary = multiplier * r.t;
      r.o = add3(r.o, scl3(r.d, t_secondary));
      const V3 nd = cos_weighted_dir(N, g_seed);
      r.d = nd;
      r.w = r.w * dot3(nd, N);
      r.depth = ndepth;
      r.km[0] = 0u; r.km[1] = 0u; r.km[2] = 0u;
      bounce = true;
    }
    if (bounce || A.update_in_place) {
      r.rng = g_seed;
      store_ray(in, i, r);
    }
  }
  if (!LEAN) {
    const unsigned slot = block_alloc(A.next_count, bounce, &sh_alloc[2]);
    if (bounce) A.next_idx[slot] = gi;
  }
}
```

### gravit_amd/csrc/trace.hip

```cpp
#include "gvt_internal.h"

#ifndef TRAV_BLOCK
#define TRAV_BLOCK 256
#endif
#define TRAV_WAVES_PER_BLOCK (TRAV_BLOCK / 64)
#ifndef TRAV_STACK
#define TRAV_STACK 24
#endif
#ifndef KT_BLOCKS_CLOSEST
#define KT_BLOCKS_CLOSEST 5
#endif
#ifndef RETIRE_BATCH
#define RETIRE_BATCH 1
#endif
#ifndef KT_BLOCKS_ANY
#define KT_BLOCKS_ANY 4
#endif
#define TRAV_SPILL 128

namespace {

struct Trav {
  const BvhNode *__restrict__ nodes;
  const float4 *__restrict__ tris;
  const uint4 *__restrict__ nodes4;
};

#include "diag_kernels.inc"

#include "trace_lane.inc"

#include "trace_wave.inc"

#include "packet_kernel.inc"

#include "shade.inc"

#include "finish_kernel.inc"

#include "convert.inc"

inline unsigned blocks_for(size_t n, unsigned b = 256) { return (unsigned)((n + b - 1) / b); }

int trav_grid(size_t n) {
  Ctx &C = gctx();
  size_t need = (n + TRAV_BLOCK - 1) / TRAV_BLOCK;
  return (int)(need < (size_t)C.trav_blocks ? (need ? need : 1) : (size_t)C.trav_blocks);
}

template <bool ANY, bool XFORM, int MODE, bool MULTI = false, typename... Args> void launch_trace(int grid, hipStream_t st, RayPlanes q, const unsigned *idx, unsigned n, Mat4 minv, Args... args) {
  minv.m[3] = minv.m[12] * 0.0f; minv.m[7] = minv.m[13] * 0.0f; minv.m[11] = minv.m[14] * 0.0f;
  k_trace<ANY, XFORM, MODE, MULTI><<<grid, TRAV_BLOCK, 0, st>>>(q, idx, n, minv, args...);
}

static size_t long_scratch_bytes(size_t n) { return sizeof(LongRec) * n + sizeof(int) * LONG_SAVE * (size_t)LONG_STK_CAP; }
static LongQ long_queue(LongRec *recs, size_t n) {
  Ctx &C = gctx();
  LongQ LQ{};
  LQ.recs = recs; LQ.count = C.d_counters + CW_LONG;
  LQ.steps = C.long_steps_override > 0 ? C.long_steps_override : C.long_steps;
  LQ.steps_drain = C.long_steps_drain > 0 && C.long_steps_drain < LQ.steps ? C.long_steps_drain : LQ.steps;
  LQ.stk = C.long_save ? (int *)(LQ.recs + n) : nullptr;
  LQ.stk_cap = LONG_STK_CAP;
  return LQ;
}

int trav_grid2(size_t n, bool closest = false) {
  Ctx &C = gctx();
  size_t want = (size_t)C.n_cu * (((size_t)((closest && C.blocks_per_cu_closest) ? C.blocks_per_cu_closest : C.blocks_per_cu) * 4) / TRAV_WAVES_PER_BLOCK);
  if (!want) want = C.n_cu;
  size_t need = (n + TRAV_BLOCK - 1) / TRAV_BLOCK;
  if (want > (size_t)C.trav_blocks) want = (size_t)C.trav_blocks;
  return (int)(need < want ? (need ? need : 1) : want);
}

}

int debug_stamps(unsigned long long *out, int reset) {
#if GVT_STAMP
  hipDeviceSynchronize();
  hipMemcpyFromSymbol(out, HIP_SYMBOL(g_stamp), sizeof(unsigned long long) * 24);
  if (reset) { unsigned long long z[24] = { 0 }; hipMemcpyToSymbol(HIP_SYMBOL(g_stamp), z, sizeof z); }
  return 0;
#else
  for (int i = 0; i < 24; i++) out[i] = 0;
  return -1;
#endif
}
int trav_overflow_fetch_async() {
  Ctx &C = gctx();
  HIPCHK(hipMemcpyAsync(C.h_pinned + 8, C.d_counters + CW_TRAV_OVF, sizeof(unsigned), hipMemcpyDeviceToHost, C.stream));
  return 0;
}
int trav_overflow_result() {
  Ctx &C = gctx();
  if (!C.h_pinned[8]) return 0;
  C.h_pinned[8] = 0;
  hipMemsetAsync(C.d_counters + CW_TRAV_OVF, 0, sizeof(unsigned), C.stream);
  set_error("BVH traversal stack overflow (more than %d pending entries for one ray): results of this call are incomplete", TRAV_STACK + TRAV_SPILL);
  return GVT_HIP_ERR_DEVICE;
}
size_t trav_spill_ints_per_thread() { return TRAV_SPILL; }
int trav_block_threads() { return TRAV_BLOCK; }

int convert_aos_to_planes(const gvt_hip_ray *d_src, size_t n, RayPlanes dst, size_t dst_off, bool keep_state) {
  if (!n) return 0;
  ProfScope ps(KC_CONVERT);
  k_aos_to_planes<<<blocks_for(n), 256, 0, gctx().stream>>>((const float4 *)d_src, (unsigned)n, dst, dst_off, keep_state ? 1 : 0);
  HIPCHK(hipGetLastError());
  return 0;
}
int convert_planes_to_aos(RayPlanes src, size_t src_off, size_t n, gvt_hip_ray *d_dst) {
  if (!n) return 0;
  ProfScope ps(KC_CONVERT);
  k_planes_to_aos<<<blocks_for(n), 256, 0, gctx().stream>>>(src, src_off, (unsigned)n, (float4 *)d_dst);
  HIPCHK(hipGetLastError());
  return 0;
}
int convert_od_to_planes(const float *d_org, const float *d_dir, size_t n, RayPlanes dst) {
  if (!n) return 0;
  ProfScope ps(KC_CONVERT);
  k_od_to_planes<<<blocks_for(n), 256, 0, gctx().stream>>>(d_org, d_dir, (unsigned)n, dst);
  HIPCHK(hipGetLastError());
  return 0;
}

MeshView mesh_view(const gvt_hip_mesh *M) {
  MeshView mv;
  mv.slots = M->d_tri; mv.slot_of = M->d_slot_of; mv.verts = M->d_verts; mv.tris = M->d_tris; mv.normals = M->d_normals; mv.vcolors = M->d_vcolors;
  mv.materials = M->d_materials; mv.n_mat = (unsigned)M->nMat; mv.face_mat = M->d_face_mat; mv.mat = M->mesh_mat;
  return mv;
}
bool walks_packets(const Ctx &C, const gvt_hip_mesh *M, size_t n) { return C.packet == 2 || (C.packet == 1 && M->packet_ok && n >= (size_t)C.packet_min_rays); }
bool plain_lambert(const gvt_hip_mesh *M) { return !M->d_vcolors && !M->d_face_mat && M->mesh_mat.type == 0; }
bool no_area_light(const gvt_hip_light *lights, int nL) { return std::all_of(lights, lights + nL, [](const gvt_hip_light &l) { return l.type != GVT_HIP_LIGHT_AREA; }); }

static bool lights_cached_at(const Ctx &C, const void *dst, const gvt_hip_light *lights_host, int nL) {
  const size_t bytes = sizeof(gvt_hip_light) * (size_t)nL;
  return C.lights_cached_dst == dst && C.lights_cached.size() == bytes && std::memcmp(C.lights_cached.data(), lights_host, bytes) == 0;
}
bool finish_lights_resident(const gvt_hip_light *lights_host, int nL) {
  Ctx &C = gctx();
  return !nL || (C.scratch[SCR_LIGHTS] && lights_cached_at(C, C.scratch[SCR_LIGHTS], lights_host, nL));
}
static int lights_on_device(const gvt_hip_light *lights_host, int nL, gvt_hip_light **d_lights, bool may_upload = true) {
  Ctx &C = gctx();
  *d_lights = (gvt_hip_light *)scratch_get(SCR_LIGHTS, sizeof(gvt_hip_light) * (nL > 0 ? nL : 1));
  if (!*d_lights) return GVT_HIP_ERR_DEVICE;
  if (!nL || lights_cached_at(C, *d_lights, lights_host, nL)) return 0;
  if (!may_upload) { set_error("finish_round: a speculative launch needs the light list resident"); return GVT_HIP_ERR_INVALID; }
  const size_t bytes = sizeof(gvt_hip_light) * (size_t)nL;
  C.lights_cached.assign((const unsigned char *)lights_host, (const unsigned char *)lights_host + bytes);
  C.lights_cached_dst = *d_lights;
  HIPCHK(hipMemcpyAsync(*d_lights, C.lights_cached.data(), bytes, hipMemcpyHostToDevice, C.stream));
  HIPCHK(hipStreamSynchronize(C.stream));
  return 0;
}

struct ChainBufs {
  gvt_hip_hit *hits; unsigned *idx_a, *idx_b; gvt_hip_light *lights;
  size_t shadow_cap; RayPlanes shadow;
  unsigned char *steps;
};
static int chain_bufs(ChainBufs &B, size_t n, int nL, const gvt_hip_light *lights_host, size_t ordered_slots = 0) {
  Ctx &C = gctx();
  B.hits = (gvt_hip_hit *)scratch_get(SCR_GENERAL, sizeof(gvt_hip_hit) * n);
  B.shadow_cap = n * (size_t)(nL > 0 ? nL : 1);
  size_t slots = ordered_slots ? ordered_slots : B.shadow_cap;
  float4 *d_shadow = (float4 *)scratch_get(SCR_SHADOW, sizeof(float4) * 4 * slots);
  B.steps = (ordered_slots && d_shadow) ? (unsigned char *)scratch_get(SCR_STEPS, n) : nullptr;
  if (ordered_slots && (!d_shadow || !B.steps)) {
    (void)hipGetLastError();
    C.shadow_order_denied = true;
    B.steps = nullptr;
    slots = B.shadow_cap;
    d_shadow = (float4 *)scratch_get(SCR_SHADOW, sizeof(float4) * 4 * slots);
  }
  B.idx_a = (unsigned *)scratch_get(SCR_IDX_A, sizeof(unsigned) * n);
  B.idx_b = (unsigned *)scratch_get(SCR_IDX_B, sizeof(unsigned) * n);
  if (!B.hits || !d_shadow || !B.idx_a || !B.idx_b) return GVT_HIP_ERR_DEVICE;
  B.shadow = make_planes(d_shadow, slots);
  B.shadow.p4 = nullptr; B.shadow.p5 = nullptr;
  return lights_on_device(lights_host, nL, &B.lights);
}

static int sort_ray_list(const gvt_hip_mesh *M, RayPlanes q, const unsigned **idx, size_t n, size_t n_cap, const Mat4 &minv, const unsigned *n_dev = nullptr) {
  Ctx &C = gctx();
  unsigned *k_in = (unsigned *)scratch_get(SCR_SORT_KEYS_IN, sizeof(unsigned) * n_cap), *k_out = (unsigned *)scratch_get(SCR_SORT_KEYS_OUT, sizeof(unsigned) * n_cap);
  unsigned *v_in = (unsigned *)scratch_get(SCR_SORT_VALS_IN, sizeof(unsigned) * n_cap), *v_out = (unsigned *)scratch_get(SCR_SORT_VALS_OUT, sizeof(unsigned) * n_cap);
  if (!k_in || !k_out || !v_in || !v_out) return GVT_HIP_ERR_DEVICE;
  const float ex = M->hi[0] - M->lo[0], ey = M->hi[1] - M->lo[1], ez = M->hi[2] - M->lo[2];
  const float3 blo = make_float3(M->lo[0], M->lo[1], M->lo[2]);
  const float3 inv = make_float3(ex > 0 ? 1.f / ex : 0.f, ey > 0 ? 1.f / ey : 0.f, ez > 0 ? 1.f / ez : 0.f);
  {
    ProfScope ps(KC_SORT);
    k_ray_keys<<<blocks_for(n), 256, 0, C.stream>>>(q, *idx, (unsigned)n, minv, blo, inv, k_in, v_in, C.sort_bits, n_dev);
    if (int rc = sort_pairs_u32(k_in, k_out, v_in, v_out, n, C.sort_bits)) return rc;
  }
  HIPCHK(hipGetLastError());
  *idx = v_out;
  return 0;
}

struct TraceSrc { RayPlanes q; Mat4 minv; Trav T; WaveSet W; TermSink sink; MultiSrc MS; const int *hop; unsigned row; };
static unsigned stripe_arg(unsigned row) { return (gctx().xcd_stripes && row) ? row : XCD_STRIPES_OFF; }
enum StepMode { BY_LANES, BY_PACKETS, BY_WAVES };
static int wave_grid(size_t n) { return (int)std::min<size_t>((n + 3) / 4, (size_t)gctx().n_cu * 3); }

template <bool XFORM, bool MULTI>
static void closest_step(StepMode mode, const TraceSrc &S, const unsigned *idx, size_t n, const unsigned *n_dev, float tnear, gvt_hip_hit *d_hits, const LongQ &LQ,
                         LongRec *d_long, bool later_pass = false) {
  Ctx &C = gctx();
  hipStream_t st = C.stream;
  unsigned *c = C.d_counters;
  const int tail_grid = C.n_cu * 3;
  RayPlanes none{};
  if (mode == BY_PACKETS) {
    ProfScope ps(KC_CLOSEST);
    LongQ LP{ d_long, c + CW_LONG, nullptr, 0u, 0, 0 };
    if constexpr (MULTI) k_packet_multi<<<blocks_for(n), 256, 0, st>>>(S.W, (unsigned)n, n_dev, tnear, d_hits, LP, c + CW_PACKETS);
    else k_packet<false><<<blocks_for(n), 256, 0, st>>>(S.q, (unsigned)n, n_dev, S.minv, S.T, tnear, d_hits, nullptr, none, nullptr, TermSink{}, LP, nullptr, nullptr, nullptr, c + CW_PACKETS);
    k_long_closest<XFORM, MULTI><<<tail_grid, 256, 0, st>>>(S.q, d_long, c + CW_LONG, S.minv, S.T, tnear, d_hits, c + CW_LONG_WORK, S.W);
  } else if (mode == BY_WAVES) {
    ProfScope ps(KC_CLOSEST);
    k_long_seed<<<blocks_for(n), 256, 0, st>>>(d_long, c + CW_LONG, idx, (unsigned)n, n_dev);
    k_long_closest<XFORM, MULTI><<<wave_grid(n), 256, 0, st>>>(S.q, d_long, c + CW_LONG, S.minv, S.T, tnear, d_hits, c + CW_LONG_WORK, S.W, nullptr, later_pass ? S.hop : nullptr);
  } else {
    {
      ProfScope ps(KC_CLOSEST);
      launch_trace<false, XFORM, 0, MULTI>(trav_grid2(n, true), st, S.q, idx, (unsigned)n, S.minv, S.T, tnear, d_hits, nullptr, none, nullptr, c + CW_WORK, C.d_spill,
                                           C.refill_min, C.inner_min, n_dev, C.share, (unsigned)C.share_min_rays, S.sink, LQ, S.MS, MULTI ? XCD_STRIPES_OFF : stripe_arg(S.row));
    }
    if (LQ.steps) {
      ProfScope ps(KC_LONG);
      k_long_closest<XFORM, MULTI><<<tail_grid, 256, 0, st>>>(S.q, LQ.recs, LQ.count, S.minv, S.T, tnear, d_hits, c + CW_LONG_WORK, S.W, LQ.stk, S.hop);
    }
  }
}

template <bool MULTI>
static void any_step(StepMode mode, const TraceSrc &S, const unsigned *idx, size_t grid_rays, unsigned n, const unsigned *n_dev, RayPlanes out, unsigned *out_count, bool early = false) {
  Ctx &C = gctx();
  unsigned *c = C.d_counters;
  ProfScope ps(KC_ANY);
  if constexpr (!MULTI) {
    if (early && mode == BY_LANES) {
      launch_trace<true, true, 2, false>(trav_grid2(grid_rays), C.stream, S.q, idx, n, S.minv, S.T, GVT_RAY_EPSILON, nullptr, nullptr, out, out_count, c + CW_WORK, C.d_spill,
                                         C.refill_min, C.inner_min, n_dev, C.share, (unsigned)C.share_min_rays, S.sink, LongQ{}, S.MS, stripe_arg(S.row));
      C.early_deposit_launches++;
      return;
    }
  }
  if (mode == BY_WAVES) k_wave_any<MULTI><<<wave_grid(grid_rays), 256, 0, C.stream>>>(S.q, c + CW_SHADOW, S.minv, S.T, GVT_RAY_EPSILON, out, out_count, c + CW_WORK, S.sink, S.MS);
  else launch_trace<true, true, 1, MULTI>(trav_grid2(grid_rays), C.stream, S.q, idx, n, S.minv, S.T, GVT_RAY_EPSILON, nullptr, nullptr, out, out_count, c + CW_WORK, C.d_spill,
                                          C.refill_min, C.inner_min, n_dev, C.share, (unsigned)C.share_min_rays, S.sink, LongQ{}, S.MS, MULTI ? XCD_STRIPES_OFF : stripe_arg(S.row));
}

static ShadeArgs shade_args(const ChainBufs &B, const unsigned *idx, size_t n, int pass, const unsigned *n_dev, unsigned *next, unsigned *c_next, RayPlanes outp,
                            unsigned *out_count, const TraceParams &P) {
  unsigned *c = gctx().d_counters;
  ShadeArgs A{};
  A.idx = idx; A.n = (unsigned)n; A.hits = B.hits; A.first_pass = (pass == 0); A.carried_rng = 1; A.out = outp; A.out_count = out_count;
  A.shadow = B.shadow; A.shadow_count = c + CW_SHADOW; A.next_idx = next; A.next_count = c_next; A.lights = B.lights; A.normi = P.normi; A.normal_mode = P.normal_mode;
  A.n_lights = P.n_lights; A.seed = P.seed; A.zero_word = c + CW_WORK; A.sink = P.sink; A.n_dev = n_dev;
  return A;
}

template <bool MULTI>
static void shade_step(const ShadeArgs &A, const MeshView &mv, bool lean = false) {
  ProfScope ps(KC_SHADE);
  if (lean) k_shade<MULTI, true><<<blocks_for(A.n, SHADE_BLOCK), SHADE_BLOCK, 0, gctx().stream>>>(A, mv);
  else k_shade<MULTI><<<blocks_for(A.n, SHADE_BLOCK), SHADE_BLOCK, 0, gctx().stream>>>(A, mv);
}

int launch_closest(gvt_hip_mesh *M, RayPlanes q, const unsigned *idx, size_t n, bool xform, const Mat4 &minv, float tnear,
                   gvt_hip_hit *d_hits, bool counter_is_zero) {
  if (!n) return 0;
  Ctx &C = gctx();
  if (!M->d_nodes4) { int rc4 = build_nodes4(M); if (rc4) return rc4; }
  if (!counter_is_zero) HIPCHK(hipMemsetAsync(C.d_counters, 0, (CW_LONG_WORK + 1) * sizeof(unsigned), C.stream));
  LongQ LQ{};
  if (M->d_nodes4 && C.long_steps > 0 && n >= (size_t)C.long_min_rays) {
    LongRec *recs = (LongRec *)scratch_get(SCR_LONG, long_scratch_bytes(n));
    if (!recs) return GVT_HIP_ERR_DEVICE;
    LQ = long_queue(recs, n);
  }
  TraceSrc S{};
  S.q = q; S.minv = minv; S.T = Trav{ M->d_nodes, M->d_tri, M->d_nodes4 };
  if (xform) closest_step<true, false>(BY_LANES, S, idx, n, nullptr, tnear, d_hits, LQ, LQ.recs);
  else closest_step<false, false>(BY_LANES, S, idx, n, nullptr, tnear, d_hits, LQ, LQ.recs);
  HIPCHK(hipGetLastError());
  C.stats.rays_closest += n;
  C.stats.launches_closest++;
  return 0;
}

int launch_visit_stats(gvt_hip_mesh *M, RayPlanes q, size_t n, float tnear, unsigned *d_out) {
  if (!n) return 0;
  Ctx &C = gctx();
  if (!M->d_nodes4) { int rc4 = build_nodes4(M); if (rc4) return rc4; }
  Trav T{ M->d_nodes, M->d_tri, M->d_nodes4 };
  unsigned *counter = C.d_counters + CW_WORK;
  HIPCHK(hipMemsetAsync(counter, 0, sizeof(unsigned), C.stream));
  k_visit_stats<<<trav_grid(n), TRAV_BLOCK, 0, C.stream>>>(q, (unsigned)n, T, tnear, d_out, counter, C.d_spill);
  HIPCHK(hipGetLastError());
  return 0;
}

int launch_wide_visit_stats(gvt_hip_mesh *M, RayPlanes q, size_t n, float tnear, const unsigned char *d_marks, unsigned *d_out) {
  if (!n) return 0;
  Ctx &C = gctx();
  Trav T{ M->d_nodes, M->d_tri, M->d_nodes4 };
  unsigned *counter = C.d_counters + CW_WORK;
  HIPCHK(hipMemsetAsync(counter, 0, sizeof(unsigned), C.stream));
  k_wide_visit_stats<<<trav_grid(n), TRAV_BLOCK, 0, C.stream>>>(q, (unsigned)n, T, tnear, d_marks, d_out, counter, C.d_spill);
  HIPCHK(hipGetLastError());
  return 0;
}

int launch_any_flags(gvt_hip_mesh *M, RayPlanes q, size_t n, bool xform, const Mat4 &minv, float tnear, int *d_flags) {
  if (!n) return 0;
  Ctx &C = gctx();
  if (!M->d_nodes4) { int rc4 = build_nodes4(M); if (rc4) return rc4; }
  Trav T{ M->d_nodes, M->d_tri, M->d_nodes4 };
  unsigned *counter = C.d_counters + CW_WORK;
  HIPCHK(hipMemsetAsync(counter, 0, sizeof(unsigned), C.stream));
  RayPlanes none{};
  {
    ProfScope ps(KC_ANY);
    if (xform) launch_trace<true, true, 0>(trav_grid2(n), C.stream, q, nullptr, (unsigned)n, minv, T, tnear, nullptr, d_flags, none, nullptr, counter, C.d_spill, C.refill_min, C.inner_min, nullptr, C.share, (unsigned)C.share_min_rays, TermSink{}, LongQ{}, MultiSrc{}, stripe_arg(0u));
    else launch_trace<true, false, 0>(trav_grid2(n), C.stream, q, nullptr, (unsigned)n, minv, T, tnear, nullptr, d_flags, none, nullptr, counter, C.d_spill, C.refill_min, C.inner_min, nullptr, C.share, (unsigned)C.share_min_rays, TermSink{}, LongQ{}, MultiSrc{}, stripe_arg(0u));
  }
  HIPCHK(hipGetLastError());
  C.stats.rays_any += n;
  C.stats.launches_any++;
  return 0;
}

int trace_core(gvt_hip_mesh *M, RayPlanes in, size_t n, uint64_t index_base, gvt_hip_queue *out, const TraceParams &P,
               const gvt_hip_light *lights_host) {
  Ctx &C = gctx();
  C.stats.trace_calls++;
  if (!n) return 0;
  hipStream_t st = C.stream;
  const int nL = P.n_lights;
  ChainBufs B;
  int rc = chain_bufs(B, n, nL, lights_host);
  if (rc) return rc;
  RayPlanes outp = make_planes(out->d_planes, out->cap);
  unsigned *c = C.d_counters;
  static_assert(CW_BOUNCE_A == CW_SHADOW + 1, "the pass's two counts are reset and read back as one run");
  k_trace_begin<<<1, 64, 0, st>>>(out->d_count, (unsigned)out->size, c);
  const MeshView mv = mesh_view(M);
  TraceSrc SA{};
  SA.q = B.shadow; SA.minv = P.minv; SA.T = Trav{ M->d_nodes, M->d_tri, M->d_nodes4 }; SA.sink = P.sink;

  size_t n_active = n;
  const size_t out_size0 = out->size;
  const unsigned *idx = nullptr;
  unsigned *next = B.idx_a;
  int pass = 0;
  while (n_active) {
    if (C.sort_rays && n_active >= 8192 && (rc = sort_ray_list(M, in, &idx, n_active, n, P.minv))) return rc;
    if (idx && C.sort_rays && C.sort_gather && n_active >= 8192) {
      float4 *od = (float4 *)scratch_get(SCR_SORT_GATHER, sizeof(float4) * 2 * n);
      if (!od) return GVT_HIP_ERR_DEVICE;
      {
        ProfScope ps(KC_SORT);
        k_gather_od<<<blocks_for(n_active), 256, 0, st>>>(in, idx, (unsigned)n_active, P.minv, od, od + n);
      }
      HIPCHK(hipGetLastError());
      RayPlanes sorted{ od, od + n, nullptr, nullptr, nullptr };
      rc = launch_closest(M, sorted, nullptr, n_active, false, P.minv, GVT_RAY_EPSILON, B.hits, pass == 0);
    } else
      rc = launch_closest(M, in, idx, n_active, true, P.minv, GVT_RAY_EPSILON, B.hits, pass == 0);
    if (rc) return rc;
    if (pass > 0) HIPCHK(hipMemsetAsync(c + CW_SHADOW, 0, 2 * sizeof(unsigned), st));
    ShadeArgs A = shade_args(B, idx, n_active, pass, nullptr, next, c + CW_BOUNCE_A, outp, out->d_count, P);
    A.in = in; A.index_base = index_base; A.carried_rng = P.carried_rng; A.update_in_place = P.update_in_place;
    shade_step<false>(A, mv);
    HIPCHK(hipGetLastError());
    C.stats.rays_shaded += n_active;
    const size_t shadow_ub = n_active * (size_t)nL;
    if (shadow_ub) {
      any_step<false>(BY_LANES, SA, nullptr, shadow_ub, 0u, c + CW_SHADOW, outp, out->d_count);
      HIPCHK(hipGetLastError());
      C.stats.launches_any++;
    }
    HIPCHK(hipMemcpyAsync(C.h_pinned, c + CW_SHADOW, 2 * sizeof(unsigned), hipMemcpyDeviceToHost, st));
    HIPCHK(hipMemcpyAsync(C.h_pinned + 2, out->d_count, sizeof(unsigned), hipMemcpyDeviceToHost, st));
    if ((rc = trav_overflow_fetch_async())) return rc;
    HIPCHK(hipStreamSynchronize(st));
    if ((rc = trav_overflow_result())) return rc;
    const unsigned n_shadow = C.h_pinned[0], n_next = C.h_pinned[1];
    C.stats.rays_any += n_shadow;
    n_active = n_next;
    idx = next;
    next = (next == B.idx_a) ? B.idx_b : B.idx_a;
    pass++;
    if (n_active) {
      out->size = C.h_pinned[2];
      if ((rc = queue_reserve(out, out->size + n_active * (size_t)(1 + nL)))) return rc;
      outp = make_planes(out->d_planes, out->cap);
    }
  }
  C.stats.rays_forwarded += C.h_pinned[2] - out_size0;
  out->size = C.h_pinned[2];
  return 0;
}

extern "C" int gvt_hip_math_probe(int kind, const float *in, size_t n, float *out) {
  if (ensure_init()) return GVT_HIP_ERR_NODEVICE;
  if (kind < 0 || kind > 2 || (n && (!in || !out)) || n > 0xffffffffull) { set_error("math_probe: bad argument"); return GVT_HIP_ERR_INVALID; }
  if (!n) return 0;
  Ctx &C = gctx();
  float *d = (float *)scratch_get(SCR_GENERAL, sizeof(float) * 2 * n);
  if (!d) return GVT_HIP_ERR_DEVICE;
  HIPCHK(hipMemcpyAsync(d, in, sizeof(float) * n, hipMemcpyHostToDevice, C.stream));
  k_math_probe<<<blocks_for(n), 256, 0, C.stream>>>(kind, d, (unsigned)n, d + n);
  HIPCHK(hipGetLastError());
  HIPCHK(hipMemcpyAsync(out, d + n, sizeof(float) * n, hipMemcpyDeviceToHost, C.stream));
  HIPCHK(hipStreamSynchronize(C.stream));
  return 0;
}

namespace {
__global__ void k_wave_pass_begin(unsigned *c, int pass, unsigned n_host, unsigned *out_count, const unsigned *n_dev0 = nullptr, WaveSeg *segs = nullptr, int n_seg = 0,
                                  unsigned *const *__restrict__ count_ptr = nullptr) {
  if (blockIdx.x || threadIdx.x) return;
  if (segs) {
    unsigned run = 0;
    for (int k = 0; k < n_seg; k++) { const unsigned n = *count_ptr[segs[k].inst]; segs[k].begin = run; segs[k].n = n; run += n; }
    *const_cast<unsigned *>(n_dev0) = run;
  }
  unsigned long long *tot = cw_totals(c);
  const int cur = cw_bounce(pass), prev = cw_bounce(pass + 1);
  if (pass == 0) { *out_count = 0u; c[CW_BOUNCE_A] = 0u; c[CW_BOUNCE_B] = 0u; tot[TOT_CLOSEST] += n_dev0 ? *n_dev0 : n_host; }
  else { tot[TOT_ANY] += c[CW_SHADOW]; tot[TOT_CLOSEST] += c[prev]; c[cur] = 0u; }
  c[CW_LONG_FRAME] += c[CW_LONG];
  cw_zero_work(c); c[CW_SHADOW] = 0u; c[CW_LONG] = 0u; c[CW_LONG_WORK] = 0u; c[CW_PKT_RETRY] = 0u;
  for (int k = 0; k < SHADOW_CLASSES; k++) c[CW_SHADOW_CLS + k] = 0u;
}
__global__ void k_wave_end(unsigned *c, unsigned *const *__restrict__ count_ptr, const unsigned char *__restrict__ mask, int n_inst) {
  const int i = blockIdx.x * blockDim.x + threadIdx.x;
  if (i == 0) cw_totals(c)[TOT_ANY] += c[CW_SHADOW];
  if (count_ptr && i < n_inst && mask[i]) *count_ptr[i] = 0u;
}
}

struct Chain {
  size_t n; int passes;
  const TraceParams &P; const gvt_hip_light *lights_host; gvt_hip_queue *out; RayPlanes outp;
  ChainBufs B;
  int *d_shadow_inst;
  LongRec *d_long;
  bool use_long, small;
  const unsigned *nd0;
};
struct Pass { int pass; const unsigned *n_dev, *idx; unsigned *next, *c_next; };

static int any_packets(const Chain &K, const TraceSrc &S) {
  Ctx &C = gctx();
  unsigned *c = C.d_counters;
  unsigned *d_retry = (unsigned *)scratch_get(SCR_PKT_RETRY, sizeof(unsigned) * K.B.shadow_cap);
  if (!d_retry) return GVT_HIP_ERR_DEVICE;
  ProfScope ps(KC_ANY);
  k_packet<true><<<blocks_for(K.B.shadow_cap), 256, 0, C.stream>>>(S.q, (unsigned)K.B.shadow_cap, nullptr, S.minv, S.T, GVT_RAY_EPSILON, nullptr, K.d_shadow_inst, K.outp, K.out->d_count,
                                                                 S.sink, LongQ{}, d_retry, c + CW_PKT_RETRY, cw_totals(c) + TOT_ANY, c + CW_PACKETS);
  launch_trace<true, true, 1>(trav_grid2(4096), C.stream, S.q, d_retry, 0u, S.minv, S.T, GVT_RAY_EPSILON, nullptr, nullptr, K.outp, K.out->d_count, c + CW_WORK, C.d_spill,
                              C.refill_min, C.inner_min, c + CW_PKT_RETRY, C.share, (unsigned)C.share_min_rays, S.sink, LongQ{}, MultiSrc{}, stripe_arg(0u));
  return 0;
}

static int single_pass(const Chain &K, Pass p, const WaveSingle &W1, size_t cls_stride) {
  Ctx &C = gctx();
  unsigned *c = C.d_counters;
  gvt_hip_mesh *M = W1.mesh;
  const size_t n = K.n;
  const int nL = K.P.n_lights;
  const bool have4 = M->d_nodes4 != nullptr, by_class = K.B.steps != nullptr;
  if (C.sort_rays && p.pass > 0 && n >= 8192 && have4)
    if (int rc = sort_ray_list(M, W1.planes, &p.idx, n, n, W1.minv, p.n_dev)) return rc;
  TraceSrc S{};
  S.q = W1.planes; S.minv = W1.minv; S.T = Trav{ M->d_nodes, M->d_tri, M->d_nodes4 };
  S.row = (W1.coherent && p.pass == 0 && !p.idx) ? W1.row_rays : 0u;
  LongQ LQ{};
  if (K.use_long && have4) LQ = long_queue(K.d_long, n);
  LQ.steps_out = K.B.steps;
  const bool small1 = K.small && have4;
  const bool pkt = walks_packets(C, M, n) && W1.coherent && p.pass == 0 && have4 && !small1;
  const bool pkt_any = pkt && C.packet == 2;
  closest_step<true, false>(pkt ? BY_PACKETS : small1 ? BY_WAVES : BY_LANES, S, p.idx, n, p.n_dev, GVT_RAY_EPSILON, K.B.hits, LQ, K.d_long);
  ShadeArgs A = shade_args(K.B, p.idx, n, p.pass, p.n_dev, p.next, p.c_next, K.outp, K.out->d_count, K.P);
  A.in = W1.planes; A.normi = W1.normi; A.sink.from = W1.inst;
  if (pkt_any) { A.shadow_inst = K.d_shadow_inst; A.shadow_stride = (unsigned)n; }
  A.steps = K.B.steps; A.cls_cnt = by_class ? c + CW_SHADOW_CLS : nullptr; A.cls_stride = (unsigned)cls_stride; A.cls_lo = C.shadow_cls_lo; A.cls_shift = C.shadow_cls_shift;
  const bool lean_shade = W1.coherent && p.pass == 0 && K.passes == 1 && K.P.sink.fb && K.P.sink.top.n_inst == 1 && nL >= 1 && plain_lambert(M) && no_area_light(K.lights_host, nL);
  const bool early_deposit = lean_shade && nL == 1 && K.P.one_writer && !small1 && !pkt_any && C.early_deposit;
  A.early_deposit = early_deposit ? 1 : 0;
  shade_step<false>(A, mesh_view(M), lean_shade);
  if (!nL) return 0;
  TraceSrc SA = S;
  SA.q = K.B.shadow; SA.sink = A.sink; SA.row = 0u;
  if (pkt_any) return any_packets(K, SA);
  if (by_class) { SA.MS.cls_cnt = c + CW_SHADOW_CLS; SA.MS.cls_stride = (unsigned)cls_stride; SA.MS.cls_total = c + CW_SHADOW; }
  any_step<false>(small1 ? BY_WAVES : BY_LANES, SA, nullptr, K.B.shadow_cap, 0u, by_class ? nullptr : c + CW_SHADOW, K.outp, K.out->d_count, early_deposit);
  return 0;
}

static void merged_pass(const Chain &K, const Pass &p, const WaveSet &W, const ChainOpts &O, int *d_hop, int *d_out_from) {
  Ctx &C = gctx();
  unsigned *c = C.d_counters;
  const TraceParams &P = K.P;
  const size_t n = K.n;
  const int nL = P.n_lights;
  TraceSrc S{};
  S.W = W; S.MS.W = W; S.hop = d_hop;
  if (d_hop) {
    S.sink = P.sink;
    S.MS.hop_inst = d_hop; S.MS.hop_read = p.pass > 0; S.MS.hop_owner = P.hop_owner; S.MS.hop_rank = P.hop_rank; S.MS.hop_tot = cw_totals(c) + TOT_CLOSEST; S.MS.hop_early = P.hop == 1 ? 1 : 0;
  }
  LongQ LQ{};
  if (K.use_long) LQ = long_queue(K.d_long, n);
  const bool pktm = O.multi_packets && p.pass == 0 && !K.small && p.idx == nullptr;
  closest_step<true, true>(pktm ? BY_PACKETS : K.small ? BY_WAVES : BY_LANES, S, p.idx, n, p.n_dev, GVT_RAY_EPSILON, K.B.hits, LQ, K.d_long, p.pass > 0);
  ShadeArgs A = shade_args(K.B, p.idx, n, p.pass, p.n_dev, p.next, p.c_next, K.outp, K.out->d_count, P);
  A.W = W; A.out_from = d_out_from; A.shadow_inst = K.d_shadow_inst; A.hop_inst = d_hop;
  const bool direct = C.shadow_direct && p.pass == 0 && !K.small;
  const bool direct_dev = direct && K.nd0 != nullptr && nL == 1;
  A.shadow_stride = direct ? (unsigned)n : 0u;
  const bool lean_multi = O.simple_meshes && p.pass == 0 && K.passes == 1 && nL >= 1 && no_area_light(K.lights_host, nL);
  shade_step<true>(A, MeshView{}, lean_multi);
  if (!nL) return;
  TraceSrc SA{};
  SA.q = K.B.shadow; SA.sink = P.sink;
  SA.MS = MultiSrc{ W, K.d_shadow_inst, d_out_from, direct ? cw_totals(c) + TOT_ANY : nullptr };
  if (d_hop && P.sink.fb && P.hop == 2) { SA.MS.hop_owner = P.hop_owner; SA.MS.hop_rank = P.hop_rank; SA.MS.hop_tot = cw_totals(c) + TOT_CLOSEST; }
  if (K.small) any_step<true>(BY_WAVES, SA, nullptr, K.B.shadow_cap, 0u, nullptr, K.outp, K.out->d_count);
  else any_step<true>(BY_LANES, SA, nullptr, K.B.shadow_cap, direct ? (unsigned)K.B.shadow_cap : 0u, direct ? (direct_dev ? K.nd0 : nullptr) : c + CW_SHADOW, K.outp, K.out->d_count);
}

int wave_trace_chain(const WaveSet &W, size_t n_total, int passes, gvt_hip_queue *out, int *d_out_from, const TraceParams &P,
                     const gvt_hip_light *lights_host, const WaveSingle *single, const ChainOpts &O) {
  Ctx &C = gctx();
  if (!n_total) return 0;
  hipStream_t st = C.stream;
  const int nL = P.n_lights;
  const size_t n = n_total;
  const bool by_class_wanted = single && single->mesh->d_nodes4 && C.shadow_order && nL == 1 && n >= (size_t)C.shadow_order_min_rays && n > (size_t)C.small_rays &&
                               C.long_steps > 0 && n >= (size_t)C.long_min_rays && !(walks_packets(C, single->mesh, n) && single->coherent);
  const size_t cls_stride = (n + 63) & ~(size_t)63;
  const size_t ordered_slots = (by_class_wanted && !C.shadow_order_denied && cls_stride * SHADOW_CLASSES * 64 <= ((size_t)8 << 30)) ? cls_stride * SHADOW_CLASSES : 0;
  const size_t shadow_slots = ordered_slots ? ordered_slots : n * (size_t)(nL > 0 ? nL : 1);
  if (shadow_slots >= 0xffffffffull) { set_error("round: %zu shadow slots exceed the 32-bit slot counters", shadow_slots); return GVT_HIP_ERR_INVALID; }
  Chain K{ n, passes, P, lights_host, out, make_planes(out->d_planes, out->cap) };
  int rc = chain_bufs(K.B, n, nL, lights_host, ordered_slots);
  if (rc) return rc;
  K.d_shadow_inst = (int *)scratch_get(SCR_SHADOW_INST, sizeof(int) * K.B.shadow_cap);
  K.d_long = (LongRec *)scratch_get(SCR_LONG, long_scratch_bytes(n));
  if (!K.d_shadow_inst || !K.d_long) return GVT_HIP_ERR_DEVICE;
  int *d_hop = nullptr;
  if (!single && P.hop && P.sink.fb) {
    d_hop = (int *)scratch_get(SCR_HOP, sizeof(int) * n);
    if (!d_hop) return GVT_HIP_ERR_DEVICE;
    HIPCHK(hipMemsetAsync(d_hop, 0xff, sizeof(int) * n, st));
  }
  unsigned *c = C.d_counters;
  K.use_long = C.long_steps > 0 && n >= (size_t)C.long_min_rays;
  K.small = n <= (size_t)C.small_rays;
  K.nd0 = single ? single->n_dev : O.n_dev0_multi;
  for (int pass = 0; pass < passes; pass++) {
    unsigned *const lists[2] = { K.B.idx_a, K.B.idx_b };
    const Pass p{ pass, pass ? c + cw_bounce(pass - 1) : K.nd0, pass ? lists[(pass - 1) & 1] : nullptr, lists[pass & 1], c + cw_bounce(pass) };
    if (!(pass == 0 && single && single->pass0_begun))
      k_wave_pass_begin<<<1, 64, 0, st>>>(c, pass, (unsigned)n, out->d_count, K.nd0, (pass == 0 && O.n_dev0_multi && !single) ? const_cast<WaveSeg *>(W.segs) : nullptr, W.n_seg, O.d_count_ptr);
    if (!single) merged_pass(K, p, W, O, d_hop, d_out_from);
    else if ((rc = single_pass(K, p, *single, cls_stride))) return rc;
    HIPCHK(hipGetLastError());
    C.stats.launches_closest++;
    C.stats.launches_any++;
  }
  if (!O.defer_end) k_wave_end<<<(unsigned)((std::max(O.n_inst, 1) + 255) / 256), 256, 0, st>>>(c, O.d_count_ptr, O.d_mask, O.n_inst);
  HIPCHK(hipGetLastError());
  C.stats.trace_calls++;
  return 0;
}

int finish_round(const WaveSet &W, size_t n_total, const TraceParams &P, const gvt_hip_light *lights_host, const void *d_qdesc, const int *d_owner, int rank,
                 unsigned *d_queue_overflow, unsigned *const *d_count_ptr, const unsigned char *d_mask, const unsigned *spec_words) {
  Ctx &C = gctx();
  if (!n_total) return 0;
  const int nL = P.n_lights;
  gvt_hip_light *d_lights;
  if (int rc = lights_on_device(lights_host, nL, &d_lights, spec_words == nullptr)) return rc;
  FinishArgs A;
  A.n_dev = spec_words ? spec_words + 2 : nullptr; A.valid = spec_words ? spec_words + 1 : nullptr;
  A.W = W; A.n = (unsigned)n_total; A.lights = d_lights; A.n_lights = nL; A.normal_mode = P.normal_mode;
  A.top = P.sink.top; A.fb = P.sink.fb; A.n_pix = P.sink.n_pix;
  A.queues = (const QueueDesc *)d_qdesc; A.owner = d_owner; A.rank = rank;
  A.counter = C.d_counters + CW_WORK; A.tot = cw_totals(C.d_counters);
  A.queue_overflow = d_queue_overflow; A.trav_overflow = C.d_counters + CW_TRAV_OVF;
  A.seed = P.seed; A.index_base = 0ull; A.skip_known = C.skip_known;
  A.count_ptr = d_count_ptr; A.clear_mask = d_mask; A.n_inst = W.n_inst;
  {
    ProfScope ps(KC_CLOSEST);
    k_finish<<<(int)std::min<size_t>((n_total + 3) / 4, (size_t)C.n_cu * 4), 256, 0, C.stream>>>(A);
  }
  HIPCHK(hipGetLastError());
  C.stats.launches_closest++;
  C.stats.trace_calls++;
  return 0;
}

int set_device_u32(unsigned *p, unsigned v) {
  k_set_u32<<<1, 64, 0, gctx().stream>>>(p, v);
  HIPCHK(hipGetLastError());
  return 0;
}

#define WIRE_MAX_QUEUES 256
static_assert(sizeof(QueueDesc) * WIRE_MAX_QUEUES + sizeof(unsigned) * (3 * WIRE_MAX_QUEUES + 1) <= PINNED_STAGE_BYTES, "the queue table fits the staging block");

int pinned_stage_begin(void **h) {
  Ctx &C = gctx();
  if (!C.h_wire) {
    HIPCHK(hipHostMalloc(&C.h_wire, PINNED_STAGE_BYTES, hipHostMallocDefault));
    HIPCHK(hipEventCreateWithFlags(&C.wire_ev, hipEventDisableTiming));
  }
  if (C.wire_busy) HIPCHK(hipEventSynchronize(C.wire_ev));
  *h = C.h_wire;
  return 0;
}
int pinned_stage_end() {
  Ctx &C = gctx();
  HIPCHK(hipEventRecord(C.wire_ev, C.stream));
  C.wire_busy = true;
  return 0;
}

namespace {
int wire_table(gvt_hip_queue *const *queues, size_t n, const uint64_t *runs, bool append, WireTable &W) {
  Ctx &C = gctx();
  const size_t o_begin = sizeof(QueueDesc) * n, o_off = o_begin + sizeof(unsigned) * (n + 1), o_fill = o_off + sizeof(unsigned) * n,
               bytes = o_fill + sizeof(unsigned) * n;
  char *d = (char *)scratch_get(SCR_WIRE_TABLE, bytes);
  if (!d) return GVT_HIP_ERR_DEVICE;
  void *stage = nullptr;
  int rc;
  if ((rc = pinned_stage_begin(&stage))) return rc;
  char *h = (char *)stage;
  QueueDesc *q = (QueueDesc *)h;
  unsigned *begin = (unsigned *)(h + o_begin), *off = (unsigned *)(h + o_off), *fill = (unsigned *)(h + o_fill);
  unsigned at = 0;
  for (size_t i = 0; i < n; i++) {
    q[i].planes = queues[i]->d_planes; q[i].cap = queues[i]->cap; q[i].count = queues[i]->d_count; q[i].keep = 0u;
    begin[i] = at;
    off[i] = append ? (unsigned)queues[i]->size : 0u;
    fill[i] = append ? (unsigned)(queues[i]->size + runs[i]) : 0u;
    at += (unsigned)runs[i];
  }
  begin[n] = at;
  HIPCHK(hipMemcpyAsync(d, h, bytes, hipMemcpyHostToDevice, C.stream));
  if ((rc = pinned_stage_end())) return rc;
  W.q = (const QueueDesc *)d; W.begin = (const unsigned *)(d + o_begin); W.off = (const unsigned *)(d + o_off); W.fill = (const unsigned *)(d + o_fill);
  W.n = (int)n;
  return 0;
}
}

extern "C" int gvt_hip_queues_export_wire(gvt_hip_queue *const *queues, size_t n, gvt_hip_ray *dst_device, size_t cap_rays, uint64_t *counts_out,
                                          uint64_t *total_out) {
  if (ensure_init()) return GVT_HIP_ERR_NODEVICE;
  if (!queues || !total_out || n < 1 || n > WIRE_MAX_QUEUES) { set_error("queues_export_wire: null argument or %zu queues (1..%d)", n, WIRE_MAX_QUEUES); return GVT_HIP_ERR_INVALID; }
  uint64_t runs[WIRE_MAX_QUEUES];
  uint64_t total = 0;
  for (size_t i = 0; i < n; i++) {
    if (!queues[i]) { set_error("queues_export_wire: queue %zu is null", i); return GVT_HIP_ERR_INVALID; }
    runs[i] = queues[i]->size;
    total += runs[i];
  }
  *total_out = total;
  if (counts_out) std::copy(runs, runs + n, counts_out);
  if (total > cap_rays) { set_error("queues_export_wire: %llu rays, capacity %zu", (unsigned long long)total, cap_rays); return GVT_HIP_ERR_CAPACITY; }
  if (!total) return 0;
  if (!dst_device) { set_error("queues_export_wire: null destination"); return GVT_HIP_ERR_INVALID; }
  if (total >= 0xffffffffull) { set_error("queues_export_wire: %llu rays exceed the 32-bit ray index", (unsigned long long)total); return GVT_HIP_ERR_INVALID; }
  Ctx &C = gctx();
  WireTable W;
  int rc = wire_table(queues, n, runs, false, W);
  if (rc) return rc;
  {
    ProfScope ps(KC_CONVERT);
    const unsigned blocks = (unsigned)((total + WIRE_BLOCK - 1) / WIRE_BLOCK);
    k_queues_to_wire<<<blocks, WIRE_BLOCK, 0, C.stream>>>(W, (unsigned)total, (float4 *)dst_device);
  }
  HIPCHK(hipGetLastError());
  for (size_t i = 0; i < n; i++) queues[i]->size = 0;
  HIPCHK(hipStreamSynchronize(C.stream));
  return 0;
}

extern "C" int gvt_hip_queues_append_wire(gvt_hip_queue *const *queues, size_t n, const gvt_hip_ray *src_device, const uint64_t *counts) {
  if (ensure_init()) return GVT_HIP_ERR_NODEVICE;
  if (!queues || !counts || n < 1 || n > WIRE_MAX_QUEUES) { set_error("queues_append_wire: null argument or %zu queues (1..%d)", n, WIRE_MAX_QUEUES); return GVT_HIP_ERR_INVALID; }
  uint64_t total = 0;
  for (size_t i = 0; i < n; i++) {
    if (!queues[i]) { set_error("queues_append_wire: queue %zu is null", i); return GVT_HIP_ERR_INVALID; }
    for (size_t k = 0; k < i && counts[i]; k++)
      if (queues[k] == queues[i] && counts[k]) { set_error("queues_append_wire: queue %zu appears twice", i); return GVT_HIP_ERR_INVALID; }
    total += counts[i];
  }
  if (!total) return 0;
  if (!src_device) { set_error("queues_append_wire: null source"); return GVT_HIP_ERR_INVALID; }
  if (total >= 0xffffffffull) { set_error("queues_append_wire: %llu rays exceed the 32-bit ray index", (unsigned long long)total); return GVT_HIP_ERR_INVALID; }
  int rc;
  for (size_t i = 0; i < n; i++)
    if (counts[i] && (rc = queue_reserve(queues[i], queues[i]->size + counts[i]))) return rc;
  Ctx &C = gctx();
  WireTable W;
  if ((rc = wire_table(queues, n, counts, true, W))) return rc;
  {
    ProfScope ps(KC_CONVERT);
    const unsigned blocks = (unsigned)((total + WIRE_BLOCK - 1) / WIRE_BLOCK);
    k_wire_to_queues<<<blocks, WIRE_BLOCK, 0, C.stream>>>((const float4 *)src_device, (unsigned)total, W);
  }
  HIPCHK(hipGetLastError());
  for (size_t i = 0; i < n; i++) queues[i]->size += counts[i];
  return 0;
}
```

### gravit_amd/csrc/trace_lane.inc

```
#ifndef GVT_TRI_NG_FROM_SLOT
#define GVT_TRI_NG_FROM_SLOT 1
#endif
#ifndef GVT_STAMP
#define GVT_STAMP 0
#endif
#if GVT_STAMP
__device__ unsigned long long g_stamp[24];
#endif
#ifndef TRAV_CHUNK
#define TRAV_CHUNK 256
#endif
#ifndef KT_SHARE_DELAY
#define KT_SHARE_DELAY 24
#endif
#define TRAV_DONE ((int)0x80000000)

#define LONG_SAVE 48
#define LONG_STK_CAP 65536u
struct LongRec { unsigned j, i; float bt; int bp; float bu, bv, bden; unsigned ns; };
struct LongQ {
  LongRec *recs;
  unsigned *count;
  int *stk;
  unsigned stk_cap;
  int steps;
  int steps_drain;
  unsigned char *steps_out;
};

typedef float f2 __attribute__((ext_vector_type(2)));
struct RaySlab {
  float ix, iy, iz;
  f2 ox, oy, oz;
};
__device__ __forceinline__ RaySlab make_slab(float ix, float iy, float iz, float ox, float oy, float oz) {
  RaySlab S;
  S.ix = ix; S.iy = iy; S.iz = iz;
  const float ex = fabsf(ox) * 4.76837158e-7f, ey = fabsf(oy) * 4.76837158e-7f, ez = fabsf(oz) * 4.76837158e-7f;
  S.ox = (f2){ ox + ex, ox - ex }; S.oy = (f2){ oy + ey, oy - ey }; S.oz = (f2){ oz + ez, oz - ez };
  return S;
}
__device__ __forceinline__ f2 splat2(float v) { return (f2){ v, v }; }
template <bool LIM = true>
__device__ __forceinline__ void node4_test(const uint4 *__restrict__ nd, const RaySlab &S, float lim, float tn[4], int rr[4], bool *hit = nullptr) {
  if (LIM) lim = cull_bound(lim);
  const uint4 w0 = nd[0], w1 = nd[1], w2 = nd[2], w3 = nd[3];
  const float sx = __uint_as_float(w0.w) * S.ix, sy = __uint_as_float(w3.z) * S.iy, sz = __uint_as_float(w3.w) * S.iz;
  const f2 bx = __builtin_elementwise_fma(splat2(__uint_as_float(w0.x)), splat2(S.ix), -S.ox);
  const f2 by = __builtin_elementwise_fma(splat2(__uint_as_float(w0.y)), splat2(S.iy), -S.oy);
  const f2 bz = __builtin_elementwise_fma(splat2(__uint_as_float(w0.z)), splat2(S.iz), -S.oz);
  const unsigned qnx = S.ix >= 0.f ? w1.x : w1.y, qfx = S.ix >= 0.f ? w1.y : w1.x;
  const unsigned qny = S.iy >= 0.f ? w1.z : w1.w, qfy = S.iy >= 0.f ? w1.w : w1.z;
  const unsigned qnz = S.iz >= 0.f ? w2.x : w2.y, qfz = S.iz >= 0.f ? w2.y : w2.x;
  rr[0] = (int)w2.z; rr[1] = (int)w2.w; rr[2] = (int)w3.x; rr[3] = (int)w3.y;
#define GVT_Q2(Q, SH) ((f2){ (float)(((Q) >> (SH)) & 0xffu), (float)(((Q) >> ((SH) + 8)) & 0xffu) })
#define GVT_SLAB2(SH, A, B)                                                                                          \
  {                                                                                                                  \
    const f2 nx_ = __builtin_elementwise_fma(GVT_Q2(qnx, SH), splat2(sx), splat2(bx.x));                              \
    const f2 ny_ = __builtin_elementwise_fma(GVT_Q2(qny, SH), splat2(sy), splat2(by.x));                              \
    const f2 nz_ = __builtin_elementwise_fma(GVT_Q2(qnz, SH), splat2(sz), splat2(bz.x));                              \
    const f2 fx_ = __builtin_elementwise_fma(GVT_Q2(qfx, SH), splat2(sx), splat2(bx.y));                              \
    const f2 fy_ = __builtin_elementwise_fma(GVT_Q2(qfy, SH), splat2(sy), splat2(by.y));                              \
    const f2 fz_ = __builtin_elementwise_fma(GVT_Q2(qfz, SH), splat2(sz), splat2(bz.y));                              \
    const float na_ = fmaxf(fmaxf(nx_.x, ny_.x), fmaxf(nz_.x, 0.f)), nb_ = fmaxf(fmaxf(nx_.y, ny_.y), fmaxf(nz_.y, 0.f)); \
    const float fa_ = fminf(fminf(fx_.x, fy_.x), fz_.x) * 1.0000004f, fb_ = fminf(fminf(fx_.y, fy_.y), fz_.y) * 1.0000004f; \
    const bool ha_ = na_ <= (LIM ? fminf(fa_, lim) : fa_), hb_ = nb_ <= (LIM ? fminf(fb_, lim) : fb_);                \
    tn[A] = ha_ ? na_ : GVT_FLT_MAX;                                                          \
    tn[B] = hb_ ? nb_ : GVT_FLT_MAX;                                                                                 \
    if (hit) { hit[A] = ha_; hit[B] = hb_; }                                                                         \
  }
  GVT_SLAB2(0, 0, 1) GVT_SLAB2(16, 2, 3)
#undef GVT_SLAB2
#undef GVT_Q2
}

__device__ __forceinline__ void sort4(float (&tn)[4], int (&rr)[4]) {
  auto ce = [&](int a, int b) {
    const bool sw = tn[b] < tn[a];
    const float ta = sw ? tn[b] : tn[a], tb = sw ? tn[a] : tn[b];
    const int ra = sw ? rr[b] : rr[a], rb = sw ? rr[a] : rr[b];
    tn[a] = ta; tn[b] = tb; rr[a] = ra; rr[b] = rb;
  };
  ce(0, 1); ce(2, 3); ce(0, 2); ce(1, 3); ce(1, 2);
}

__device__ __forceinline__ int *kt_spill_ptr(int *spill_base, int k) {
  unsigned t = threadIdx.x;
  asm volatile("" : "+v"(t));
  return spill_base + ((size_t)(blockIdx.x * TRAV_BLOCK + t) * TRAV_SPILL + (size_t)k);
}

__device__ inline int wave_find_seg(const WaveSet &W, unsigned g) {
  int lo = 0, hi = W.n_seg - 1;
  while (lo < hi) {
    const int mid = (lo + hi + 1) >> 1;
    if (W.segs[mid].begin <= g) lo = mid; else hi = mid - 1;
  }
  return lo;
}

__device__ inline void flush_pending(volatile unsigned *pend, int n_pend, const RayPlanes &q, const RayPlanes &out, unsigned *out_count, const TermSink &K,
                                     const int *__restrict__ ray_inst = nullptr, int *__restrict__ out_from = nullptr) {
  if (!K.fb) {
    unsigned base = 0;
    if (lane_id() == 0) base = atomicAdd(out_count, (unsigned)n_pend);
    base = (unsigned)__builtin_amdgcn_readfirstlane((int)base);
    for (int k = (int)lane_id(); k < n_pend; k += 64) {
      const unsigned src = pend[k];
      out.p0[base + k] = q.p0[src]; out.p1[base + k] = q.p1[src]; out.p2[base + k] = q.p2[src]; out.p3[base + k] = q.p3[src];
      if (out.p4) out.p4[base + k] = 0u;
      store_no_known(out, base + k);
      if (out_from) out_from[base + k] = ray_inst[src];
    }
    return;
  }
  const bool alone = K.top.n_inst == 1 && !ray_inst && K.from >= 0;
  for (int k0 = 0; k0 < n_pend; k0 += 64) {
    const int k = k0 + (int)lane_id();
    bool go_on = false;
    float4 a, b, c, d;
    int from = K.from;
    if (k < n_pend) {
      const unsigned src = pend[k];
      c = q.p2[src]; d = q.p3[src];
      if (!alone) {
        a = q.p0[src]; b = q.p1[src];
        if (ray_inst) from = ray_inst[src];
        float ret_t;
        go_on = top_nearest(a, b, K.top, from, ret_t) >= 0;
      }
      if (!go_on) deposit_shadow(K.fb, K.n_pix, __float_as_int(d.w), mk3(c.x, c.y, c.z), d.z, (unsigned)__float_as_int(d.x));
    }
    const unsigned long long m = ballot64(go_on);
    if (m) {
      unsigned base = 0;
      if (lane_id() == 0) base = atomicAdd(out_count, (unsigned)__popcll(m));
      base = (unsigned)__builtin_amdgcn_readfirstlane((int)base);
      if (go_on) { const unsigned slot = base + lanes_below(m); out.p0[slot] = a; out.p1[slot] = b; out.p2[slot] = c; out.p3[slot] = d; if (out.p4) out.p4[slot] = 0u; store_no_known(out, slot); if (out_from) out_from[slot] = from; }
    }
  }
}

template <unsigned frac8> __device__ __noinline__ uint3 kt_fetch(unsigned *counter, unsigned n, unsigned row, unsigned state) {
  const unsigned wpb = (unsigned)(TRAV_BLOCK / 64), n_waves_total = gridDim.x * wpb, share_w = n / n_waves_total;
  const unsigned chunk = max(64u, ((share_w * frac8 / 8u) + 16u) & ~31u), dyn = max(64u, (share_w / 16u) & ~63u);
  unsigned ub = 1u, ue = 0u;
  if (row == XCD_STRIPES_OFF) {
    unsigned base = 0, len = chunk;
    if (!(state & 16u)) base = (blockIdx.x * wpb + (threadIdx.x >> 6)) * chunk;
    else {
      if (lane_id() == 0) base = atomicAdd(counter, dyn);
      base = (unsigned)__builtin_amdgcn_readfirstlane((int)base) + n_waves_total * chunk;
      len = dyn;
    }
    if (base < n) { ub = base; ue = min(base + len, n); }
    return make_uint3(ub, ue, 16u);
  }
  const XcdStripeMap SM = xcd_stripe_map(n, dyn, row);
  const unsigned ks = max(1u, (chunk + dyn / 2u) / dyn), home = blockIdx.x & 7u;
  unsigned st_steal = state & 15u, st_left = (state & 16u) ? state >> 5 : ks;
  bool got = false;
  if (st_left) {
    const unsigned s = (blockIdx.x >> 3) * wpb + (threadIdx.x >> 6);
    got = xcd_stripe_unit(SM, home, s * ks + (ks - st_left), &ub, &ue);
    st_left = got ? st_left - 1u : 0u;
  }
  while (!got && st_steal < XCD_STRIPES) {
    const unsigned x = (home + st_steal) & 7u;
    unsigned t = 0;
    if (lane_id() == 0) t = atomicAdd(counter + cw_work_stripe(x), 1u);
    t = (unsigned)__builtin_amdgcn_readfirstlane((int)t) + ((gridDim.x + 7u - x) >> 3) * wpb * ks;
    got = xcd_stripe_unit(SM, x, t, &ub, &ue);
    if (!got) st_steal++;
  }
  if (!got) { ub = 1u; ue = 0u; }
  return make_uint3(ub, ue, st_steal | 16u | (st_left << 5));
}

#define KT_TAB 32
struct KtInst { Mat4 minv; const uint4 *nodes4; const float4 *tris; };
struct KtSeg { float4 *planes; unsigned long long cap; unsigned begin; int inst; };
struct MultiSrc {
  WaveSet W;
  int *ray_inst;
  int *out_from;
  unsigned long long *tot_any;
  const unsigned *cls_cnt;
  unsigned cls_stride;
  unsigned *cls_total;
  int *hop_inst;
  int hop_read;
  const int *hop_owner;
  int hop_rank;
  int hop_early;
  unsigned long long *hop_tot;
};
template <bool ANY, bool XFORM, int MODE, bool MULTI = false>
__global__ __launch_bounds__(TRAV_BLOCK, (ANY ? KT_BLOCKS_ANY : KT_BLOCKS_CLOSEST)) void k_trace(RayPlanes q, const unsigned *__restrict__ idx, unsigned n, Mat4 minv, Trav T, float tnear,
                                                       gvt_hip_hit *__restrict__ hits, int *__restrict__ flags, RayPlanes out, unsigned *out_count,
                                                       unsigned *counter, int *spill_base, int refill_min, int inner_min, const unsigned *__restrict__ n_dev, int share, unsigned share_min, TermSink sink, LongQ LQ,
                                                       MultiSrc MS = MultiSrc{}, unsigned stripe_row = XCD_STRIPES_OFF) {
  const unsigned n_waves_total = gridDim.x * (unsigned)(TRAV_BLOCK / 64);
  const float z12 = minv.m[3], z13 = minv.m[7], z14 = minv.m[11];
  if (n_dev) n = *n_dev;
  constexpr int N_CLS = (ANY && !MULTI) ? SHADOW_CLASSES : 0;
  __shared__ unsigned s_cls[N_CLS + 1];
  const bool by_class = N_CLS > 0 && MS.cls_cnt != nullptr;
  if (by_class) {
    if (threadIdx.x == 0) {
      unsigned acc = 0;
      for (int k = 0; k < N_CLS; k++) { s_cls[k] = acc; acc += MS.cls_cnt[N_CLS - 1 - k]; }
      s_cls[N_CLS] = acc;
      if (blockIdx.x == 0 && MS.cls_total) *MS.cls_total = acc;
    }
    __syncthreads();
    n = s_cls[N_CLS];
  }
  const unsigned share_w = n / n_waves_total;
  const unsigned chunk = max(64u, ((share_w * (ANY ? 5u : 3u) / 8u) + 16u) & ~31u);
  const unsigned dyn = max(64u, (share_w / 16u) & ~63u);
  __shared__ int stack[TRAV_STACK * TRAV_BLOCK];
  int *lds = &stack[threadIdx.x];
  int *spill_m = spill_base + (size_t)(blockIdx.x * TRAV_BLOCK + threadIdx.x) * TRAV_SPILL;
#define KT_SPILL(K) (*(MULTI ? spill_m + (K) : kt_spill_ptr(spill_base, (K))))
  __shared__ KtInst s_inst[MULTI ? KT_TAB : 1];
  __shared__ KtSeg s_seg[(MULTI && !ANY) ? KT_TAB : 1];
  bool tab = false;
  if (MULTI) {
    tab = MS.W.n_inst > 0 && MS.W.n_inst <= KT_TAB && MS.W.n_seg <= KT_TAB;
    if (tab) {
      for (int t = (int)threadIdx.x; t < MS.W.n_inst; t += TRAV_BLOCK) { const WaveInst *wi = MS.W.insts + t; s_inst[t].minv = wi->minv; s_inst[t].nodes4 = wi->nodes4; s_inst[t].tris = wi->tris; }
      if (!ANY)
        for (int t = TRAV_BLOCK - 1 - (int)threadIdx.x; t < MS.W.n_seg; t += TRAV_BLOCK) { const WaveSeg sg = MS.W.segs[t]; KtSeg k; k.planes = sg.planes; k.cap = sg.cap; k.begin = sg.begin; k.inst = sg.inst; s_seg[t] = k; }
      __syncthreads();
    }
  }
#define KT_PUSH(REF)                                                                  \
  {                                                                                   \
    if (sp < TRAV_STACK) { lds[sp * TRAV_BLOCK] = (REF); sp++; }                      \
    else if (sp - TRAV_STACK < TRAV_SPILL) { KT_SPILL(sp - TRAV_STACK) = (REF); sp++; }  \
    else atomicOr(counter + (CW_TRAV_OVF - CW_WORK), 1u);           \
  }
#define KT_POP()                                                                      \
  {                                                                                   \
    if (sp == sb) cur = TRAV_DONE;                                                    \
    else { sp--; if (sp < TRAV_STACK) cur = lds[sp * TRAV_BLOCK]; else cur = KT_SPILL(sp - TRAV_STACK); } \
  }
  __shared__ unsigned pend_all[(TRAV_BLOCK / 64) * 128];
  volatile unsigned *pend = &pend_all[(threadIdx.x >> 6) * 128];
  int n_pend = 0;
  unsigned c_next = 0, c_end = 0;
  bool exhausted = false;
  bool first_chunk = true;
  unsigned st_state = 0;
  bool active = false;
  unsigned j = 0;
  V3 O = mk3(0, 0, 0), D = mk3(0, 0, 1);
  RaySlab S = make_slab(0.f, 0.f, 0.f, 0.f, 0.f, 0.f);
  float bt = GVT_FLT_MAX, bu = 0.f, bv = 0.f, bden = 1.f;
  int bp = -1, sp = 0, cur = TRAV_DONE;
  int sb = 0;
  bool sharing = false;
  int drain_iters = 0;
  int nsteps = 0;
#define KT_PARKED (nsteps < 0)
  const uint4 *nodes4_l = T.nodes4;
  const float4 *tris_l = T.tris;
  int inst_l = 0;
  unsigned gidx = 0;
  unsigned n_started = 0;
  unsigned n_hops = 0;
#if GVT_STAMP
  unsigned long long st_refill = 0, st_inner = 0, st_leaf = 0, st_retire = 0, n_inner_it = 0, n_outer_it = 0, t_mark = 0, t_begin = __builtin_amdgcn_s_memtime();
  unsigned long long t_exh = 0, it_exh = 0, out_exh = 0, act_exh = 0, n_inner_lanes = 0, n_leaf_lanes = 0;
#endif
  for (;;) {
#if GVT_STAMP == 1
    { unsigned long long t_ = __builtin_amdgcn_s_memtime(); if (n_outer_it) st_retire += t_ - t_mark; t_mark = t_; }
#endif
    unsigned long long idle = ballot64(!active);
    int nidle = __popcll(idle);
    if (!exhausted && (nidle >= refill_min || nidle == 64)) {
      while (nidle > 0) {
        if (c_next == c_end) {
          if constexpr (!MULTI) {
            const uint3 f = kt_fetch<ANY ? 5u : 3u>(counter, n, stripe_row, st_state);
            const unsigned ub = (unsigned)__builtin_amdgcn_readfirstlane((int)f.x), ue = (unsigned)__builtin_amdgcn_readfirstlane((int)f.y);
            st_state = (unsigned)__builtin_amdgcn_readfirstlane((int)f.z);
            if (ub > ue) {
              exhausted = true;
#if GVT_STAMP
              if (!t_exh) { t_exh = __builtin_amdgcn_s_memtime(); it_exh = n_inner_it; out_exh = n_outer_it; act_exh = 64 - nidle; }
#endif
              break;
            }
            c_next = ub; c_end = ue;
            if (ub == ue) continue;
          } else {
          unsigned base = 0;
          unsigned this_chunk = chunk;
          if (first_chunk) {
            first_chunk = false;
            base = (blockIdx.x * (unsigned)(TRAV_BLOCK / 64) + (threadIdx.x >> 6)) * chunk;
          } else {
            if (lane_id() == 0) base = atomicAdd(counter, dyn);
            base = (unsigned)__builtin_amdgcn_readfirstlane((int)base) + n_waves_total * chunk;
            this_chunk = dyn;
          }
          if (base >= n) {
            exhausted = true;
#if GVT_STAMP
            if (!t_exh) { t_exh = __builtin_amdgcn_s_memtime(); it_exh = n_inner_it; out_exh = n_outer_it; act_exh = 64 - nidle; }
#endif
            break;
          }
          c_next = base;
          c_end = min(base + this_chunk, n);
          }
        }
        const unsigned take = min(c_end - c_next, (unsigned)nidle);
        const unsigned rank = lanes_below(idle);
        bool start = false;
        if (!active && rank < take) {
          j = c_next + rank;
          unsigned i = idx ? idx[j] : j;
          if (by_class) {
            int k = 0;
#pragma unroll
            for (int t = 1; t < N_CLS; t++) k += (j >= s_cls[t]) ? 1 : 0;
            i = (unsigned)(N_CLS - 1 - k) * MS.cls_stride + (j - s_cls[k]);
          }
          float4 a, b;
          start = true;
          if (MULTI) {
            if (ANY) {
              inst_l = MS.ray_inst[i];
              start = inst_l >= 0;
              if (start) { a = q.p0[i]; b = q.p1[i]; }
            } else if (tab) {
              int lo = 0, hi = MS.W.n_seg - 1;
              while (lo < hi) { const int mid = (lo + hi + 1) >> 1; if (s_seg[mid].begin <= i) lo = mid; else hi = mid - 1; }
              const unsigned local = i - s_seg[lo].begin;
              const float4 *pl = s_seg[lo].planes;
              a = pl[local]; b = pl[s_seg[lo].cap + local];
              inst_l = s_seg[lo].inst; gidx = i;
              if (MS.hop_read) { const int h_ = MS.hop_inst[i]; if (h_ >= 0) inst_l = h_; }
            } else {
              const WaveSeg sg = MS.W.segs[wave_find_seg(MS.W, i)];
              const unsigned local = i - sg.begin;
              a = sg.planes[local]; b = sg.planes[sg.cap + local];
              inst_l = sg.inst; gidx = i;
              if (MS.hop_read) { const int h_ = MS.hop_inst[i]; if (h_ >= 0) inst_l = h_; }
            }
            if (start && tab) {
              nodes4_l = s_inst[inst_l].nodes4; tris_l = s_inst[inst_l].tris;
              O = xfm_point(s_inst[inst_l].minv, mk3(a.x, a.y, a.z)); D = xfm_vector(s_inst[inst_l].minv, mk3(b.x, b.y, b.z));
            } else if (start) {
              const WaveInst *wi = MS.W.insts + inst_l;
              nodes4_l = wi->nodes4; tris_l = wi->tris;
              O = xfm_point(wi->minv, mk3(a.x, a.y, a.z)); D = xfm_vector(wi->minv, mk3(b.x, b.y, b.z));
            }
          } else {
            a = q.p0[i]; b = q.p1[i];
            O = mk3(a.x, a.y, a.z); D = mk3(b.x, b.y, b.z);
            if (XFORM) {
              const float *m = minv.m;
              O = xfm_point(minv, O);
              D = mk3((m[0] * D.x + m[4] * D.y) + (m[8] * D.z + z12), (m[1] * D.x + m[5] * D.y) + (m[9] * D.z + z13), (m[2] * D.x + m[6] * D.y) + (m[10] * D.z + z14));
            }
            if (ANY && MODE >= 1) j = i;
          }
          if (start) {
            const float dx = fabsf(D.x) < 1e-30f ? copysignf(1e-30f, D.x) : D.x;
            const float dy = fabsf(D.y) < 1e-30f ? copysignf(1e-30f, D.y) : D.y;
            const float dz = fabsf(D.z) < 1e-30f ? copysignf(1e-30f, D.z) : D.z;
            const float ix = 1.0f / dx, iy = 1.0f / dy, iz = 1.0f / dz;
            S = make_slab(ix, iy, iz, O.x * ix, O.y * iy, O.z * iz);
            bt = GVT_FLT_MAX; bu = 0.f; bv = 0.f; bden = 1.f; bp = -1;
            sp = 0; sb = 0; nsteps = 0;
            cur = (MULTI ? nodes4_l : T.nodes4) != nullptr ? 0 : TRAV_DONE;
            active = true;
          }
        }
        if (MULTI && ANY) n_started += (unsigned)__popcll(ballot64(start));
        c_next += take;
        idle = ballot64(!active);
        nidle = __popcll(idle);
      }
    }
    if (nidle == 64) break;
    const bool share_on = ANY && (share & 1) != 0;
    if (exhausted) drain_iters++;
    const bool share_now = share_on && exhausted && drain_iters > KT_SHARE_DELAY && n >= share_min;
    if (share_now && nidle > 0) {
      unsigned long long idle_m = idle;
      unsigned long long don_m = ballot64(active && cur != TRAV_DONE && (sp - sb) >= 2);
      const unsigned wave_tid0 = threadIdx.x & ~63u;
      for (int pairs = 0; idle_m && don_m && pairs < 16; pairs++) {
        const int h = __ffsll((long long)idle_m) - 1, d = __ffsll((long long)don_m) - 1;
        const int sbd = __shfl(sb, d);
        const unsigned gj = (unsigned)__shfl((int)j, d);
        const float gOx = __shfl(O.x, d), gOy = __shfl(O.y, d), gOz = __shfl(O.z, d);
        const float gDx = __shfl(D.x, d), gDy = __shfl(D.y, d), gDz = __shfl(D.z, d);
        RaySlab gS;
        gS.ix = __shfl(S.ix, d); gS.iy = __shfl(S.iy, d); gS.iz = __shfl(S.iz, d);
        gS.ox = (f2){ __shfl(S.ox.x, d), __shfl(S.ox.y, d) }; gS.oy = (f2){ __shfl(S.oy.x, d), __shfl(S.oy.y, d) }; gS.oz = (f2){ __shfl(S.oz.x, d), __shfl(S.oz.y, d) };
        const int gbp = __shfl(bp, d);
        const int ginst = __shfl(inst_l, d);
        if ((int)lane_id() == h) {
          if (MULTI) { inst_l = ginst; nodes4_l = MS.W.insts[ginst].nodes4; tris_l = MS.W.insts[ginst].tris; }
          const unsigned tid_d = wave_tid0 + (unsigned)d;
          cur = (sbd < TRAV_STACK) ? stack[sbd * TRAV_BLOCK + tid_d]
                                   : spill_base[((size_t)blockIdx.x * TRAV_BLOCK + tid_d) * TRAV_SPILL + (sbd - TRAV_STACK)];
          j = gj; O = mk3(gOx, gOy, gOz); D = mk3(gDx, gDy, gDz);
          S = gS; bp = gbp;
          sp = 0; sb = 0;
          active = true;
        }
        if ((int)lane_id() == d) sb++;
        idle_m &= idle_m - 1;
        don_m &= don_m - 1;
        sharing = true;
#if GVT_STAMP
        if (lane_id() == 0) atomicAdd(&g_stamp[23], 1ull);
#endif
      }
    }
#if GVT_STAMP == 1
    { unsigned long long t_ = __builtin_amdgcn_s_memtime(); st_refill += t_ - t_mark; t_mark = t_; n_outer_it++; }
#endif
    unsigned long long im = ballot64(cur >= 0);
    const float lim2 = fminf(cull_bound(bt), 3.40282326e38f);
    while (im) {
      const bool at_inner = cur >= 0;
      if (at_inner) {
        float tn[4];
        int rr[4];
        bool entered[4];
        node4_test<ANY>((const uint4 *)((const char *)(MULTI ? nodes4_l : T.nodes4) + ((unsigned)cur << 6)), S, GVT_FLT_MAX, tn, rr, ANY ? entered : nullptr);
#define KT_ENTERED(K) (ANY ? entered[K] : (tn[K] <= lim2))
        if (!ANY) sort4(tn, rr);
        int nxt = TRAV_DONE;
        bool have = false;
        if (sp + 3 <= TRAV_STACK) {
#pragma unroll
          for (int c4 = 3; c4 >= 0; c4--) {
            if (KT_ENTERED(c4)) {
              if (have) { lds[sp * TRAV_BLOCK] = nxt; sp++; }
              nxt = rr[c4]; have = true;
            }
          }
        } else {
#pragma unroll
          for (int c4 = 3; c4 >= 0; c4--) {
            if (KT_ENTERED(c4)) {
              if (have) KT_PUSH(nxt)
              nxt = rr[c4]; have = true;
            }
          }
        }
        if (have) cur = nxt;
        else KT_POP()
#undef KT_ENTERED
      }
#if GVT_STAMP == 1
      n_inner_it++; n_inner_lanes += (unsigned long long)__popcll(ballot64(at_inner));
#endif
      if (!ANY && at_inner && LQ.steps && ++nsteps > (exhausted ? LQ.steps_drain : LQ.steps) && cur != TRAV_DONE) { KT_PUSH(cur) cur = TRAV_DONE; nsteps = -1; }
      im = ballot64(cur >= 0);
      if (__popcll(im) < inner_min) break;
    }
#if GVT_STAMP == 1
    { unsigned long long t_ = __builtin_amdgcn_s_memtime(); st_inner += t_ - t_mark; t_mark = t_; }
#endif
    {
      const bool at_leaf = cur < 0 && cur != TRAV_DONE;
#if GVT_STAMP == 1
      n_leaf_lanes += (unsigned long long)__popcll(ballot64(at_leaf));
#endif
      if (at_leaf) {
        const unsigned code = (unsigned)~cur;
        const unsigned first = code >> 3, ntri = code & 7u;
        const float4 *ts = (MULTI ? tris_l : T.tris) + 4 * (size_t)first;
        bool occluded = false;
        for (unsigned kb = 0; kb < ntri && !(ANY && occluded); kb += 2) {
          float4 s0[2], s1[2], s2[2];
#pragma unroll
          for (unsigned k = 0; k < 2; k++)
            if (kb + k < ntri) { s0[k] = ts[4 * (kb + k)]; s1[k] = ts[4 * (kb + k) + 1]; s2[k] = ts[4 * (kb + k) + 2]; }
#pragma unroll
          for (unsigned k = 0; k < 2; k++) {
            if (kb + k < ntri && !(ANY && occluded)) {
              const V3 e1 = mk3(s1[k].x, s1[k].y, s1[k].z), e2 = mk3(s2[k].x, s2[k].y, s2[k].z);
              float TT, U, V, aden;
              if (tri_test_raw(O, D, mk3(s0[k].x, s0[k].y, s0[k].z), e1, e2, cross3(e1, e2), tnear, TT, U, V, aden)) {
                const float t = TT / aden;
                if (t <= GVT_FLT_MAX) {
                  if (ANY) occluded = true;
                  else {
                    const int prim = __float_as_int(s0[k].w);
                    if (bp < 0 || t < bt || (t == bt && prim < bp)) { bt = t; bp = prim; bu = U; bv = V; bden = aden; }
                  }
                }
              }
            }
          }
        }
        if (ANY && occluded) bp = 0;
      }
      if (at_leaf) {
        if (ANY && bp == 0) cur = TRAV_DONE;
        else KT_POP()
      }
    }
#if GVT_STAMP == 1
    { unsigned long long t_ = __builtin_amdgcn_s_memtime(); st_leaf += t_ - t_mark; t_mark = t_; }
#endif
    {
      const int nfin_w = __popcll(ballot64(active && cur == TRAV_DONE)), nidle_w = __popcll(ballot64(!active));
      const bool retire_now = RETIRE_BATCH == 0 || share_now || nfin_w + nidle_w >= (exhausted ? 64 : refill_min);
      if (!retire_now) continue;
    }
    if (sharing) {
      const unsigned long long FM = ballot64(active && cur == TRAV_DONE);
      unsigned long long fm = FM;
      while (fm) {
        const int f = __ffsll((long long)fm) - 1;
        const unsigned jf = (unsigned)__shfl((int)j, f);
        const unsigned long long G = ballot64(active && j == jf);
        const unsigned long long Gf = G & FM, A = G & ~FM;
        const int tgt = A ? __ffsll((long long)A) - 1 : __ffsll((long long)Gf) - 1;
        unsigned long long src = Gf & ~(1ull << tgt);
        bool merged_occluded = false;
        while (src) {
          const int sidx = __ffsll((long long)src) - 1;
          if (__shfl(bp, sidx) >= 0) merged_occluded = true;
          if ((int)lane_id() == sidx) active = false;
          src &= src - 1;
        }
        if (merged_occluded && ((G >> lane_id()) & 1ull) && active) { bp = 0; cur = TRAV_DONE; }
        fm &= ~Gf;
      }
    }
    if (MULTI && (ANY ? (MODE == 1 && MS.hop_tot != nullptr) : (MS.hop_inst != nullptr))) {
      const bool cand = active && cur == TRAV_DONE && bp < 0 && (ANY || !KT_PARKED) && !(exhausted && MS.hop_early);
      if (ballot64(cand)) {
        bool hopped = false;
        if (cand) {
          float4 *slot0;
          float4 a, b;
          if (ANY) { slot0 = q.p0 + j; b = q.p1[j]; }
          else {
            const WaveSeg sg = MS.W.segs[wave_find_seg(MS.W, gidx)];
            const unsigned local = gidx - sg.begin;
            slot0 = sg.planes + local; b = sg.planes[sg.cap + local];
          }
          a = *slot0;
          float ret_t;
          const int next = top_nearest(a, b, sink.top, inst_l, ret_t);
          if (next >= 0 && (!MS.hop_owner || MS.hop_owner[next] == MS.hop_rank)) {
            const V3 o = add3(mk3(a.x, a.y, a.z), scl3(mk3(b.x, b.y, b.z), ret_t * 0.95f));
            a.x = o.x; a.y = o.y; a.z = o.z;
            *slot0 = a;
            if (ANY) MS.ray_inst[j] = next; else MS.hop_inst[gidx] = next;
            inst_l = next;
            const WaveInst *wi = MS.W.insts + next;
            nodes4_l = wi->nodes4; tris_l = wi->tris;
            O = xfm_point(wi->minv, o); D = xfm_vector(wi->minv, mk3(b.x, b.y, b.z));
            const float dx = fabsf(D.x) < 1e-30f ? copysignf(1e-30f, D.x) : D.x;
            const float dy = fabsf(D.y) < 1e-30f ? copysignf(1e-30f, D.y) : D.y;
            const float dz = fabsf(D.z) < 1e-30f ? copysignf(1e-30f, D.z) : D.z;
            const float ix = 1.0f / dx, iy = 1.0f / dy, iz = 1.0f / dz;
            S = make_slab(ix, iy, iz, O.x * ix, O.y * iy, O.z * iz);
            bt = GVT_FLT_MAX; bu = 0.f; bv = 0.f; bden = 1.f; bp = -1;
            sp = 0; sb = 0; nsteps = 0;
            cur = nodes4_l != nullptr ? 0 : TRAV_DONE;
            hopped = true;
          }
        }
        n_hops += (unsigned)__popcll(ballot64(hopped));
      }
    }
    const bool fin = active && cur == TRAV_DONE;
    if (ANY && MODE == 1) {
      const bool survive = fin && bp < 0;
      const unsigned long long sm = ballot64(survive);
      if (sm) {
        if (survive) pend[n_pend + lanes_below(sm)] = j;
        n_pend += __popcll(sm);
      }
      if (n_pend >= 64) { flush_pending(pend, n_pend, q, out, out_count, sink, MULTI ? MS.ray_inst : nullptr, MULTI ? MS.out_from : nullptr); n_pend = 0; }
    }
    if (!ANY && LQ.steps) {
      const unsigned long long pm = ballot64(fin && KT_PARKED);
      if (pm) {
        unsigned base = 0;
        if ((int)lane_id() == __ffsll((long long)pm) - 1) base = atomicAdd(LQ.count, (unsigned)__popcll(pm));
        base = __shfl(base, __ffsll((long long)pm) - 1);
        if (fin && KT_PARKED) {
          const unsigned slot = base + lanes_below(pm);
          LongRec R; R.j = j; R.i = MULTI ? gidx : (idx ? idx[j] : j); R.bt = bt; R.bp = bp; R.bu = bu; R.bv = bv; R.bden = bden; R.ns = 0u;
          const int depth = sp - sb;
          if (LQ.stk && depth > 0 && depth <= LONG_SAVE && slot < LQ.stk_cap) {
            int *dst = LQ.stk + (size_t)slot * LONG_SAVE;
            for (int k = 0; k < depth; k++) dst[k] = (sb + k < TRAV_STACK) ? lds[(sb + k) * TRAV_BLOCK] : KT_SPILL(sb + k - TRAV_STACK);
            R.ns = (unsigned)depth;
          }
          LQ.recs[slot] = R;
        }
      }
    }
    if (ANY && MODE == 2) {
      if (fin && bp >= 0) {
        const unsigned px = ((const unsigned *)q.p2)[j];
        if (px != 0xffffffffu) ((float4 *)sink.fb)[px] = make_float4(0.f, 0.f, 0.f, 0.f);
      }
    }
    if (fin) {
      if (ANY) { if (MODE == 0) flags[j] = (bp >= 0) ? 1 : 0; }
      else {
        if (!KT_PARKED) { gvt_hip_hit h; h.t = bt; h.prim = bp; h.u = (bp >= 0) ? bu / bden : 0.f; h.v = (bp >= 0) ? bv / bden : 0.f; hits[j] = h; }
        if (LQ.steps_out) LQ.steps_out[j] = (unsigned char)(KT_PARKED ? 255 : min(nsteps, 254));
      }
      active = false;
    }
  }
#if GVT_STAMP
  if (lane_id() == 0) { atomicAdd(&g_stamp[0], st_refill); atomicAdd(&g_stamp[1], st_inner); atomicAdd(&g_stamp[2], st_leaf); atomicAdd(&g_stamp[3], st_retire); atomicAdd(&g_stamp[4], n_inner_it); atomicAdd(&g_stamp[5], n_outer_it); atomicAdd(&g_stamp[6], 1ull); atomicAdd(&g_stamp[7], (unsigned long long)__builtin_amdgcn_s_memtime() - t_begin); atomicAdd(&g_stamp[14], n_inner_lanes); atomicAdd(&g_stamp[15], n_leaf_lanes); atomicMax(&g_stamp[16], ~t_begin); atomicMax(&g_stamp[17], (unsigned long long)__builtin_amdgcn_s_memtime()); atomicMax(&g_stamp[18], t_exh); atomicAdd(&g_stamp[19], t_exh ? t_exh - t_begin : 0ull); atomicMax(&g_stamp[20], (unsigned long long)__builtin_amdgcn_s_memtime() - t_begin); atomicMax(&g_stamp[21], t_exh ? t_exh - t_begin : 0ull); atomicMax(&g_stamp[22], ~(t_exh ? t_exh - t_begin : ~0ull));
    if (t_exh) { atomicAdd(&g_stamp[8], (unsigned long long)__builtin_amdgcn_s_memtime() - t_exh); atomicAdd(&g_stamp[9], n_inner_it - it_exh); atomicAdd(&g_stamp[10], n_outer_it - out_exh); atomicAdd(&g_stamp[11], act_exh); atomicMax(&g_stamp[12], (unsigned long long)__builtin_amdgcn_s_memtime() - t_exh); atomicMax(&g_stamp[13], n_inner_it - it_exh); } }
#endif
  if (ANY && MODE == 1) { if (n_pend) flush_pending(pend, n_pend, q, out, out_count, sink, MULTI ? MS.ray_inst : nullptr, MULTI ? MS.out_from : nullptr); }
  if (MULTI && ANY && MS.tot_any && n_started && lane_id() == 0) atomicAdd(MS.tot_any, (unsigned long long)n_started);
  if (MULTI && MS.hop_tot && n_hops && lane_id() == 0) atomicAdd(MS.hop_tot, (unsigned long long)n_hops);
#undef KT_PUSH
#undef KT_POP
#undef KT_SPILL
#undef KT_PARKED
}
```

### gravit_amd/csrc/trace_wave.inc

```
#define LONG_CAP 512
#define LONG_PHYS (LONG_CAP + 256)

struct WaveLists { volatile int *s_ref; volatile float *s_tn; volatile int *l_ref; volatile float *l_tn; };

__device__ __forceinline__ bool within_best(float etn, float bt) { return etn <= cull_bound(bt); }
__device__ __forceinline__ bool closer(float t, int p, float bt, int bp) { return bp < 0 || t < bt || (t == bt && p < bp); }

#define CL_GROUPS 12
template <bool CLUSTER>
struct WaveFan {
  static constexpr int OPEN = CLUSTER ? CL_GROUPS : 64;
  static constexpr int NODES = CLUSTER ? 16 : 3;
  static constexpr int LEAVES = CLUSTER ? 20 : 4;
};

template <bool ANY, bool CLUSTER>
__device__ __forceinline__ void wave_nodes(const uint4 *__restrict__ nodes, const RaySlab &S, const WaveLists &L, int take, int &ns, int &nl, float bt) {
  const int lane = (int)lane_id();
  const int g = CLUSTER ? lane / 5 : lane, role = CLUSTER ? lane - 5 * g : 0;
  const bool mine = g < take;
  int ent = 0;
  float etn = 0.f;
  if (mine) { ent = L.s_ref[ns - 1 - g]; if constexpr (!ANY) etn = L.s_tn[ns - 1 - g]; }
  __builtin_amdgcn_wave_barrier();
  ns -= take;
  bool act = mine && (ANY || within_best(etn, bt));
  const uint4 *nd;
  if constexpr (CLUSTER) {
    const unsigned mask = (unsigned)ent & 15u;
    act = act && (role == 0 || ((mask >> (role - 1)) & 1u));
    const unsigned slot = ((unsigned)ent >> 4) + (role ? 1u + (unsigned)__popc(mask & ((1u << (role - 1)) - 1u)) : 0u);
    nd = nodes + (size_t)GVT_NODE4_F4 * slot;
  } else nd = nodes + (size_t)GVT_NODE4_F4 * ent;
  float tn[4];
  int rr[4];
  bool entered[4] = { false, false, false, false };
  auto in = [&](int c) { return ANY ? entered[c] : tn[c] < GVT_FLT_MAX; };
  unsigned verdict = 0u;
  if (act) {
    if constexpr (ANY) node4_test(nd, S, GVT_FLT_MAX, tn, rr, entered);
    else node4_test(nd, S, bt, tn, rr);
    if (CLUSTER && role == 0) verdict = (in(0) ? 1u : 0u) | (in(1) ? 2u : 0u) | (in(2) ? 4u : 0u) | (in(3) ? 8u : 0u);
    if constexpr (!ANY) sort4(tn, rr);
  }
  bool open = act;
  if constexpr (CLUSTER) {
    const unsigned pv = (unsigned)__shfl((int)verdict, 5 * g);
    open = act && (role == 0 || ((pv >> (role - 1)) & 1u));
  }
#pragma unroll
  for (int c = 3; c >= 0; c--) {
    const bool hit = open && in(c);
    const bool inner = hit && rr[c] >= 0 && !(CLUSTER && role == 0), leaf = hit && rr[c] < 0;
    const unsigned long long mi = ballot64(inner), ml = ballot64(leaf);
    if (inner) { const int pos = ns + (int)lanes_below(mi); L.s_ref[pos] = rr[c]; if constexpr (!ANY) L.s_tn[pos] = tn[c]; }
    if (leaf) { const int pos = nl + (int)lanes_below(ml); L.l_ref[pos] = rr[c]; if constexpr (!ANY) L.l_tn[pos] = tn[c]; }
    ns += __popcll(mi);
    nl += __popcll(ml);
  }
  __builtin_amdgcn_wave_barrier();
}

template <bool ANY>
__device__ __forceinline__ bool wave_leaves(const float4 *__restrict__ tris, V3 O, V3 D, float tnear, const WaveLists &L, int &nl,
                                            float &bt, int &bp, float &bu, float &bv, float &bden) {
  const int lane = (int)lane_id();
  const int take = min(nl, 64);
  const bool mine = lane < take;
  int ref = -1;
  float etn = 0.f;
  if (mine) { ref = L.l_ref[nl - 1 - lane]; if constexpr (!ANY) etn = L.l_tn[nl - 1 - lane]; }
  __builtin_amdgcn_wave_barrier();
  nl -= take;
  float lt = GVT_FLT_MAX, lu = 0.f, lv = 0.f, ld = 1.f;
  int lp = -1;
  bool hit_any = false;
  if (mine && (ANY || within_best(etn, bt))) {
    const unsigned code = (unsigned)~ref;
    const unsigned first = code >> 3, ntri = code & 7u;
    const float4 *ts = tris + 4 * (size_t)first;
    for (unsigned k = 0; k < ntri && !hit_any; k++) {
      const float4 s0 = ts[4 * k], s1 = ts[4 * k + 1], s2 = ts[4 * k + 2];
      const V3 e1 = mk3(s1.x, s1.y, s1.z), e2 = mk3(s2.x, s2.y, s2.z);
      float TT, U, V, aden;
      if (tri_test_raw(O, D, mk3(s0.x, s0.y, s0.z), e1, e2, cross3(e1, e2), tnear, TT, U, V, aden)) {
        const float t = TT / aden;
        if (t <= GVT_FLT_MAX) {
          if constexpr (ANY) hit_any = true;
          else {
            const int prim = __float_as_int(s0.w);
            if (closer(t, prim, lt, lp)) { lt = t; lp = prim; lu = U; lv = V; ld = aden; }
          }
        }
      }
    }
  }
  if constexpr (ANY) return ballot64(hit_any) != 0ull;
  if (ballot64(lp >= 0)) {
#pragma unroll
    for (int off = 32; off >= 1; off >>= 1) {
      const float ot = __shfl_xor(lt, off), ou = __shfl_xor(lu, off), ov = __shfl_xor(lv, off), od = __shfl_xor(ld, off);
      const int op = __shfl_xor(lp, off);
      if (op >= 0 && closer(ot, op, lt, lp)) { lt = ot; lp = op; lu = ou; lv = ov; ld = od; }
    }
    if (lp >= 0 && closer(lt, lp, bt, bp)) { bt = lt; bp = lp; bu = lu; bv = lv; bden = ld; }
  }
  return false;
}

template <bool ANY, bool CLUSTER, int CAP, int PHYS>
__device__ __forceinline__ bool wave_run(const uint4 *__restrict__ nodes, const float4 *__restrict__ tris, V3 O, V3 D, const RaySlab &S, float tnear, const WaveLists &L,
                                          int ns, int nl, float &bt, int &bp, float &bu, float &bv, float &bden, unsigned *ovf_word) {
  using F = WaveFan<CLUSTER>;
  const int lane = (int)lane_id();
  bool occluded = false;
  while (!occluded && (ns > 0 || nl > 0)) {
    const bool do_leaf = nl > 0 && (ns == 0 || nl >= 64 || nl > CAP - 256);
    if (!do_leaf) {
      int take = min(min(ns, F::OPEN), min((CAP - ns) / F::NODES, (CAP - nl) / F::LEAVES));
      take = max(take, 1);
      if (ns + F::NODES * take > PHYS || nl + F::LEAVES * take > PHYS) { if (lane == 0) atomicOr(ovf_word, 1u); break; }
      wave_nodes<ANY, CLUSTER>(nodes, S, L, take, ns, nl, bt);
    } else occluded = wave_leaves<ANY>(tris, O, D, tnear, L, nl, bt, bp, bu, bv, bden);
  }
  return occluded;
}
template <bool CLUSTER, int CAP, int PHYS>
__device__ __forceinline__ bool wave_any_run(const uint4 *__restrict__ nodes, int root_entry, const float4 *__restrict__ tris, V3 O, V3 D, const RaySlab &S, float tnear,
                                              volatile int *s_ref, volatile int *l_ref, unsigned *ovf_word) {
  if (lane_id() == 0) s_ref[0] = CLUSTER ? root_entry : 0;
  __builtin_amdgcn_wave_barrier();
  float bt = GVT_FLT_MAX, bu = 0.f, bv = 0.f, bden = 1.f;
  int bp = -1;
  return wave_run<true, CLUSTER, CAP, PHYS>(nodes, tris, O, D, S, tnear, WaveLists{ s_ref, nullptr, l_ref, nullptr }, (CLUSTER || nodes) ? 1 : 0, 0, bt, bp, bu, bv, bden, ovf_word);
}
__device__ __forceinline__ RaySlab slab_of(V3 O, V3 D) {
  const float dx = fabsf(D.x) < 1e-30f ? copysignf(1e-30f, D.x) : D.x;
  const float dy = fabsf(D.y) < 1e-30f ? copysignf(1e-30f, D.y) : D.y;
  const float dz = fabsf(D.z) < 1e-30f ? copysignf(1e-30f, D.z) : D.z;
  const float ix = 1.0f / dx, iy = 1.0f / dy, iz = 1.0f / dz;
  return make_slab(ix, iy, iz, O.x * ix, O.y * iy, O.z * iz);
}

__device__ __forceinline__ unsigned wave_ticket(bool &first, unsigned *counter, int wv) {
  if (first) { first = false; return blockIdx.x * 4u + (unsigned)wv; }
  unsigned r = 0;
  if (lane_id() == 0) r = atomicAdd(counter, 1u);
  return (unsigned)__builtin_amdgcn_readfirstlane((int)r) + gridDim.x * 4u;
}

template <bool XFORM, bool MULTI = false>
__global__ __launch_bounds__(256) void k_long_closest(RayPlanes q, const LongRec *__restrict__ recs, const unsigned *__restrict__ n_recs, Mat4 minv,
                                                       Trav T, float tnear, gvt_hip_hit *__restrict__ hits, unsigned *counter, WaveSet W = WaveSet{},
                                                       const int *__restrict__ stk = nullptr, const int *__restrict__ hop_inst = nullptr) {
  __shared__ int s_ref_all[4][LONG_PHYS];
  __shared__ float s_tn_all[4][LONG_PHYS];
  __shared__ int l_ref_all[4][LONG_PHYS];
  __shared__ float l_tn_all[4][LONG_PHYS];
  const int wv = threadIdx.x >> 6;
  const int lane = (int)lane_id();
  volatile int *s_ref = s_ref_all[wv];
  volatile float *s_tn = s_tn_all[wv];
  volatile int *l_ref = l_ref_all[wv];
  volatile float *l_tn = l_tn_all[wv];
  const unsigned n = *n_recs;
  bool first = true;
  for (;;) {
    const unsigned r = wave_ticket(first, counter, wv);
    if (r >= n) break;
    const LongRec R = recs[r];
    float4 a, b;
    V3 O, D;
    if (MULTI) {
      const WaveSeg sg = W.segs[wave_find_seg(W, R.i)];
      const unsigned local = R.i - sg.begin;
      a = sg.planes[local]; b = sg.planes[sg.cap + local];
      int inst = sg.inst;
      if (hop_inst) { const int h_ = hop_inst[R.i]; if (h_ >= 0) inst = h_; }
      const WaveInst *wi = W.insts + inst;
      T.nodes4 = wi->nodes4; T.tris = wi->tris;
      O = xfm_point(wi->minv, mk3(a.x, a.y, a.z)); D = xfm_vector(wi->minv, mk3(b.x, b.y, b.z));
    } else {
      a = q.p0[R.i]; b = q.p1[R.i];
      O = mk3(a.x, a.y, a.z); D = mk3(b.x, b.y, b.z);
      if (XFORM) { O = xfm_point(minv, O); D = xfm_vector(minv, D); }
    }
    const RaySlab S = slab_of(O, D);
    float bt = R.bt, bu = R.bu, bv = R.bv, bden = R.bden;
    int bp = R.bp;
    int ns = T.nodes4 ? 1 : 0, nl = 0;
    if (stk && R.ns && T.nodes4) {
      const int e = lane < (int)R.ns ? stk[(size_t)r * LONG_SAVE + lane] : TRAV_DONE;
      const bool is_node = lane < (int)R.ns && e >= 0, is_leaf = lane < (int)R.ns && e < 0 && e != TRAV_DONE;
      const unsigned long long mi = ballot64(is_node), ml = ballot64(is_leaf);
      if (is_node) { s_ref[lanes_below(mi)] = e; s_tn[lanes_below(mi)] = 0.f; }
      if (is_leaf) { l_ref[lanes_below(ml)] = e; l_tn[lanes_below(ml)] = 0.f; }
      ns = __popcll(mi); nl = __popcll(ml);
    } else if (lane == 0) { s_ref[0] = 0; s_tn[0] = 0.f; }
    __builtin_amdgcn_wave_barrier();
    wave_run<false, false, LONG_CAP, LONG_PHYS>(T.nodes4, T.tris, O, D, S, tnear, WaveLists{ s_ref, s_tn, l_ref, l_tn }, ns, nl, bt, bp, bu, bv, bden, counter + (CW_TRAV_OVF - CW_LONG_WORK));
    { gvt_hip_hit h; h.t = bt; h.prim = bp; h.u = (bp >= 0) ? bu / bden : 0.f; h.v = (bp >= 0) ? bv / bden : 0.f; hits[R.j] = h; }
  }
}

__global__ __launch_bounds__(256) void k_long_seed(LongRec *__restrict__ recs, unsigned *__restrict__ count, const unsigned *__restrict__ idx, unsigned n,
                                                    const unsigned *__restrict__ n_dev) {
  if (n_dev) n = *n_dev;
  const unsigned j = blockIdx.x * blockDim.x + threadIdx.x;
  if (j == 0) *count = n;
  if (j >= n) return;
  LongRec R; R.j = j; R.i = idx ? idx[j] : j; R.bt = GVT_FLT_MAX; R.bp = -1; R.bu = 0.f; R.bv = 0.f; R.bden = 1.f; R.ns = 0u;
  recs[j] = R;
}

template <bool MULTI>
__global__ __launch_bounds__(256) void k_wave_any(RayPlanes q, const unsigned *__restrict__ n_dev, Mat4 minv, Trav T, float tnear, RayPlanes out,
                                                   unsigned *out_count, unsigned *counter, TermSink sink, MultiSrc MS) {
  __shared__ int s_ref_all[4][LONG_PHYS];
  __shared__ int l_ref_all[4][LONG_PHYS];
  const int wv = threadIdx.x >> 6;
  const int lane = (int)lane_id();
  volatile int *s_ref = s_ref_all[wv];
  volatile int *l_ref = l_ref_all[wv];
  const unsigned n = *n_dev;
  bool first = true;
  for (;;) {
    const unsigned r = wave_ticket(first, counter, wv);
    if (r >= n) break;
    const float4 a = q.p0[r], b = q.p1[r];
    int inst = sink.from;
    V3 O, D;
    if (MULTI) {
      inst = MS.ray_inst[r];
      const WaveInst *wi = MS.W.insts + inst;
      T.nodes4 = wi->nodes4; T.tris = wi->tris;
      O = xfm_point(wi->minv, mk3(a.x, a.y, a.z)); D = xfm_vector(wi->minv, mk3(b.x, b.y, b.z));
    } else {
      O = xfm_point(minv, mk3(a.x, a.y, a.z)); D = xfm_vector(minv, mk3(b.x, b.y, b.z));
    }
    const bool occluded = wave_any_run<false, LONG_CAP, LONG_PHYS>(T.nodes4, 0, T.tris, O, D, slab_of(O, D), tnear, s_ref, l_ref, counter + (CW_TRAV_OVF - CW_WORK));
    if (!occluded && lane == 0) {
      const float4 c = q.p2[r], d = q.p3[r];
      bool go_on = true;
      if (sink.fb) {
        float ret_t;
        go_on = top_nearest(a, b, sink.top, inst, ret_t) >= 0;
        if (!go_on) deposit_shadow(sink.fb, sink.n_pix, __float_as_int(d.w), mk3(c.x, c.y, c.z), d.z, (unsigned)__float_as_int(d.x));
      }
      if (go_on) {
        const unsigned slot = atomicAdd(out_count, 1u);
        out.p0[slot] = a; out.p1[slot] = b; out.p2[slot] = c; out.p3[slot] = d;
        if (out.p4) out.p4[slot] = 0u;
        store_no_known(out, slot);
        if (MULTI && MS.out_from) MS.out_from[slot] = inst;
      }
    }
    __builtin_amdgcn_wave_barrier();
  }
}
```

Baseline: 2506 Mrays/s.

## Record hit triangle slot during traversal and park best-hit UVs in LDS

Adds a hit_slot knob, off by default, under which closest-hit traversal records the storage slot of the winning triangle. Shading and the finish kernel then read that slot directly instead of going through the slot_of[prim] indirection. Separately, the lane-traversal kernel now always keeps the best-hit u, v and denominator in extra LDS words rather than registers, to reduce register pressure. The LDS parking is unconditional for non-ANY, non-MULTI traversal, which adds LDS traffic on every closer hit and enlarges shared memory per block, possibly lowering occupancy.

Measured after the change: 2496 Mrays/s. Within noise of the previous version (-0.4%).

```diff
diff --git a/gravit_amd/csrc/api.hip b/gravit_amd/csrc/api.hip
--- a/gravit_amd/csrc/api.hip
+++ b/gravit_amd/csrc/api.hip
@@ -240,6 +240,7 @@
   { "packet_min_rays", &Knobs::packet_min_rays, 0, 1 << 30, true },
   { "shadow_order", &Knobs::shadow_order, 0, 1, true },       { "shadow_order_min_rays", &Knobs::shadow_order_min_rays, 0, 1 << 30, true },
   { "xcd_stripes", &Knobs::xcd_stripes, 0, 1, true },           { "early_deposit", &Knobs::early_deposit, 0, 1, true },
+  { "hit_slot", &Knobs::hit_slot, 0, 1, true },
 
   { "inline_kb", &Knobs::inline_kb, 0, 1024, true },          { "comm_cus", &Knobs::comm_cus, 0, 128, true },
   { "comm_stream", &Knobs::comm_stream, 0, 1, true },         { "spec_ticks", &Knobs::spec_ticks, 0, 1, true },
diff --git a/gravit_amd/csrc/finish_kernel.inc b/gravit_amd/csrc/finish_kernel.inc
--- a/gravit_amd/csrc/finish_kernel.inc
+++ b/gravit_amd/csrc/finish_kernel.inc
@@ -21,6 +21,7 @@
   int n_inst;
   const unsigned *n_dev;
   const unsigned *valid;
+  int hit_slot;
 };
 
 __device__ __forceinline__ int uni(int x) { return __builtin_amdgcn_readfirstlane(x); }
@@ -37,13 +38,13 @@
 #define FIN_PHYS (FIN_CAP + 256)
 template <int CAP, int PHYS>
 __device__ inline void wave_closest(const uint4 *__restrict__ nodes4, const uint4 *__restrict__ nodes4c, int root_entry, const float4 *__restrict__ tris, V3 O, V3 D, float tnear,
-                                    const WaveLists &L, float &bt, int &bp, float &bu, float &bv, float &bden, unsigned *ovf_word) {
-  bt = GVT_FLT_MAX; bu = 0.f; bv = 0.f; bden = 1.f; bp = -1;
+                                    const WaveLists &L, float &bt, int &bp, float &bu, float &bv, float &bden, unsigned &bs, unsigned *ovf_word) {
+  bt = GVT_FLT_MAX; bu = 0.f; bv = 0.f; bden = 1.f; bp = -1; bs = 0u;
   if (lane_id() == 0) { L.s_ref[0] = nodes4c ? root_entry : 0; L.s_tn[0] = 0.f; }
   __builtin_amdgcn_wave_barrier();
-  if (nodes4c) wave_run<false, true, CAP, PHYS>(nodes4c, tris, O, D, slab_of(O, D), tnear, L, 1, 0, bt, bp, bu, bv, bden, ovf_word);
-  else wave_run<false, false, CAP, PHYS>(nodes4, tris, O, D, slab_of(O, D), tnear, L, nodes4 ? 1 : 0, 0, bt, bp, bu, bv, bden, ovf_word);
-  bt = uni(bt); bp = uni(bp); bu = uni(bu); bv = uni(bv); bden = uni(bden);
+  if (nodes4c) wave_run<false, true, CAP, PHYS>(nodes4c, tris, O, D, slab_of(O, D), tnear, L, 1, 0, bt, bp, bu, bv, bden, bs, ovf_word);
+  else wave_run<false, false, CAP, PHYS>(nodes4, tris, O, D, slab_of(O, D), tnear, L, nodes4 ? 1 : 0, 0, bt, bp, bu, bv, bden, bs, ovf_word);
+  bt = uni(bt); bp = uni(bp); bu = uni(bu); bv = uni(bv); bden = uni(bden); bs = uni(bs);
 }
 template <int CAP, int PHYS>
 __device__ inline bool wave_any(const uint4 *__restrict__ nodes4, const uint4 *__restrict__ nodes4c, int root_entry, const float4 *__restrict__ tris, V3 O, V3 D, float tnear,
@@ -109,7 +110,8 @@
       const WaveInst *wi = A.W.insts + inst;
       float bt, bu, bv, bden;
       int bp;
-      wave_closest<FIN_CAP, FIN_PHYS>(wi->nodes4, wi->nodes4c, wi->root_entry4c, wi->tris, xfm_point(wi->minv, r.o), xfm_vector(wi->minv, r.d), GVT_RAY_EPSILON, L, bt, bp, bu, bv, bden, A.trav_overflow);
+      unsigned bs;
+      wave_closest<FIN_CAP, FIN_PHYS>(wi->nodes4, wi->nodes4c, wi->root_entry4c, wi->tris, xfm_point(wi->minv, r.o), xfm_vector(wi->minv, r.d), GVT_RAY_EPSILON, L, bt, bp, bu, bv, bden, bs, A.trav_overflow);
       n_closest++;
       if (bp < 0) {
         int next;
@@ -124,7 +126,7 @@
       const MeshView *M = &wi->mv;
       float t = bt;
       r.t = t;
-      const float4 *sl = M->slots + 4 * (size_t)M->slot_of[bp];
+      const float4 *sl = M->slots + 4 * (size_t)(A.hit_slot ? bs : M->slot_of[bp]);
       const float4 q0 = sl[0], q1 = sl[1], q2 = sl[2], q3 = sl[3];
       const V3 v0 = mk3(q0.x, q0.y, q0.z), v1 = mk3(q1.w, q2.w, q3.x), v2 = mk3(q3.y, q3.z, q3.w);
       int ia = 0, ib = 0, ic = 0;
diff --git a/gravit_amd/csrc/gvt_internal.h b/gravit_amd/csrc/gvt_internal.h
--- a/gravit_amd/csrc/gvt_internal.h
+++ b/gravit_amd/csrc/gvt_internal.h
@@ -67,6 +67,7 @@
   int shadow_cls_lo = 24, shadow_cls_shift = 3;
   int xcd_stripes = 1;
   int early_deposit = 1;
+  int hit_slot = 0;
   int shadow_order_min_rays = 262144;
   int packet_min_rays = 524288;
   int packet_sah_max = 128;
diff --git a/gravit_amd/csrc/packet_kernel.inc b/gravit_amd/csrc/packet_kernel.inc
--- a/gravit_amd/csrc/packet_kernel.inc
+++ b/gravit_amd/csrc/packet_kernel.inc
@@ -118,7 +118,7 @@
       if (active) retry_idx[slot] = j;
     } else {
       const unsigned slot = wave_alloc(LQ.count, live);
-      if (live) { LongRec R; R.j = j; R.i = j; R.bt = bt; R.bp = bp; R.bu = bu; R.bv = bv; R.bden = bden; R.ns = 0u; LQ.recs[slot] = R; }
+      if (live) { LongRec R; R.j = j; R.i = j; R.bt = bt; R.bp = bp; R.bu = bu; R.bv = bv; R.bden = bden; R.ns = 0u; R.slot = 0u; LQ.recs[slot] = R; }
     }
     if (lane_id() == 0) atomicAdd(bail_count, 1u);
     return;
@@ -160,7 +160,7 @@
     const bool bail = packet_walk<false>(wi->nodes4, wi->tris, O, D, tnear, live, bt, bp, bu, bv, bden, active);
     if (bail) {
       const unsigned slot = wave_alloc(LQ.count, live);
-      if (live) { LongRec R; R.j = j; R.i = j; R.bt = bt; R.bp = bp; R.bu = bu; R.bv = bv; R.bden = bden; R.ns = 0u; LQ.recs[slot] = R; }
+      if (live) { LongRec R; R.j = j; R.i = j; R.bt = bt; R.bp = bp; R.bu = bu; R.bv = bv; R.bden = bden; R.ns = 0u; R.slot = 0u; LQ.recs[slot] = R; }
       if (lane_id() == 0) atomicAdd(bail_count, 1u);
     } else if (live) { gvt_hip_hit h; h.t = bt; h.prim = bp; h.u = (bp >= 0) ? bu / bden : 0.f; h.v = (bp >= 0) ? bv / bden : 0.f; hits[j] = h; }
   }
diff --git a/gravit_amd/csrc/shade.inc b/gravit_amd/csrc/shade.inc
--- a/gravit_amd/csrc/shade.inc
+++ b/gravit_amd/csrc/shade.inc
@@ -147,6 +147,7 @@
   unsigned n;
   unsigned long long index_base;
   const gvt_hip_hit *hits;
+  const unsigned *hit_slot;
   int first_pass;
   int carried_rng;
   RayPlanes out; unsigned *out_count;
@@ -231,6 +232,7 @@
   if (in_range) {
     r = load_ray(in, i);
     h = A.hits[j];
+    const unsigned hs = A.hit_slot ? A.hit_slot[j] : 0u;
     if (!LEAN) g_seed = (A.first_pass && (!A.carried_rng || r.rng == 0u)) ? ray_stream_seed(A.seed, A.index_base + gi) : r.rng;
     if (h.prim < 0) {
       miss = true;
@@ -238,7 +240,7 @@
       shaded = true;
       float t = h.t;
       r.t = t;
-      const float4 *sl = M->slots + 4 * (size_t)M->slot_of[h.prim];
+      const float4 *sl = M->slots + 4 * (size_t)(A.hit_slot ? hs : M->slot_of[h.prim]);
       const float4 s0 = sl[0], s1 = sl[1], s2 = sl[2], s3 = sl[3];
       const V3 v0 = mk3(s0.x, s0.y, s0.z), v1 = mk3(s1.w, s2.w, s3.x), v2 = mk3(s3.y, s3.z, s3.w);
       int ia = 0, ib = 0, ic = 0;
diff --git a/gravit_amd/csrc/trace.hip b/gravit_amd/csrc/trace.hip
--- a/gravit_amd/csrc/trace.hip
+++ b/gravit_amd/csrc/trace.hip
@@ -161,10 +161,12 @@
   gvt_hip_hit *hits; unsigned *idx_a, *idx_b; gvt_hip_light *lights;
   size_t shadow_cap; RayPlanes shadow;
   unsigned char *steps;
+  unsigned *hit_slot;
 };
 static int chain_bufs(ChainBufs &B, size_t n, int nL, const gvt_hip_light *lights_host, size_t ordered_slots = 0) {
   Ctx &C = gctx();
-  B.hits = (gvt_hip_hit *)scratch_get(SCR_GENERAL, sizeof(gvt_hip_hit) * n);
+  B.hits = (gvt_hip_hit *)scratch_get(SCR_GENERAL, (sizeof(gvt_hip_hit) + sizeof(unsigned)) * n);
+  B.hit_slot = (B.hits && C.hit_slot) ? (unsigned *)(B.hits + n) : nullptr;
   B.shadow_cap = n * (size_t)(nL > 0 ? nL : 1);
   size_t slots = ordered_slots ? ordered_slots : B.shadow_cap;
   float4 *d_shadow = (float4 *)scratch_get(SCR_SHADOW, sizeof(float4) * 4 * slots);
@@ -205,6 +207,7 @@
 struct TraceSrc { RayPlanes q; Mat4 minv; Trav T; WaveSet W; TermSink sink; MultiSrc MS; const int *hop; unsigned row; };
 static unsigned stripe_arg(unsigned row) { return (gctx().xcd_stripes && row) ? row : XCD_STRIPES_OFF; }
 enum StepMode { BY_LANES, BY_PACKETS, BY_WAVES };
+static bool closest_leaves_slots(StepMode mode) { return mode != BY_PACKETS; }
 static int wave_grid(size_t n) { return (int)std::min<size_t>((n + 3) / 4, (size_t)gctx().n_cu * 3); }
 
 template <bool XFORM, bool MULTI>
@@ -224,7 +227,7 @@
   } else if (mode == BY_WAVES) {
     ProfScope ps(KC_CLOSEST);
     k_long_seed<<<blocks_for(n), 256, 0, st>>>(d_long, c + CW_LONG, idx, (unsigned)n, n_dev);
-    k_long_closest<XFORM, MULTI><<<wave_grid(n), 256, 0, st>>>(S.q, d_long, c + CW_LONG, S.minv, S.T, tnear, d_hits, c + CW_LONG_WORK, S.W, nullptr, later_pass ? S.hop : nullptr);
+    k_long_closest<XFORM, MULTI><<<wave_grid(n), 256, 0, st>>>(S.q, d_long, c + CW_LONG, S.minv, S.T, tnear, d_hits, c + CW_LONG_WORK, S.W, nullptr, later_pass ? S.hop : nullptr, LQ.hit_slot);
   } else {
     {
       ProfScope ps(KC_CLOSEST);
@@ -233,7 +236,7 @@
     }
     if (LQ.steps) {
       ProfScope ps(KC_LONG);
-      k_long_closest<XFORM, MULTI><<<tail_grid, 256, 0, st>>>(S.q, LQ.recs, LQ.count, S.minv, S.T, tnear, d_hits, c + CW_LONG_WORK, S.W, LQ.stk, S.hop);
+      k_long_closest<XFORM, MULTI><<<tail_grid, 256, 0, st>>>(S.q, LQ.recs, LQ.count, S.minv, S.T, tnear, d_hits, c + CW_LONG_WORK, S.W, LQ.stk, S.hop, LQ.hit_slot);
     }
   }
 }
@@ -487,11 +490,14 @@
   LongQ LQ{};
   if (K.use_long && have4) LQ = long_queue(K.d_long, n);
   LQ.steps_out = K.B.steps;
+  LQ.hit_slot = K.B.hit_slot;
   const bool small1 = K.small && have4;
   const bool pkt = walks_packets(C, M, n) && W1.coherent && p.pass == 0 && have4 && !small1;
   const bool pkt_any = pkt && C.packet == 2;
-  closest_step<true, false>(pkt ? BY_PACKETS : small1 ? BY_WAVES : BY_LANES, S, p.idx, n, p.n_dev, GVT_RAY_EPSILON, K.B.hits, LQ, K.d_long);
+  const StepMode mode = pkt ? BY_PACKETS : small1 ? BY_WAVES : BY_LANES;
+  closest_step<true, false>(mode, S, p.idx, n, p.n_dev, GVT_RAY_EPSILON, K.B.hits, LQ, K.d_long);
   ShadeArgs A = shade_args(K.B, p.idx, n, p.pass, p.n_dev, p.next, p.c_next, K.outp, K.out->d_count, K.P);
+  A.hit_slot = closest_leaves_slots(mode) ? LQ.hit_slot : nullptr;
   A.in = W1.planes; A.normi = W1.normi; A.sink.from = W1.inst;
   if (pkt_any) { A.shadow_inst = K.d_shadow_inst; A.shadow_stride = (unsigned)n; }
   A.steps = K.B.steps; A.cls_cnt = by_class ? c + CW_SHADOW_CLS : nullptr; A.cls_stride = (unsigned)cls_stride; A.cls_lo = C.shadow_cls_lo; A.cls_shift = C.shadow_cls_shift;
@@ -523,8 +529,11 @@
   LongQ LQ{};
   if (K.use_long) LQ = long_queue(K.d_long, n);
   const bool pktm = O.multi_packets && p.pass == 0 && !K.small && p.idx == nullptr;
-  closest_step<true, true>(pktm ? BY_PACKETS : K.small ? BY_WAVES : BY_LANES, S, p.idx, n, p.n_dev, GVT_RAY_EPSILON, K.B.hits, LQ, K.d_long, p.pass > 0);
+  const StepMode mode = pktm ? BY_PACKETS : K.small ? BY_WAVES : BY_LANES;
+  if (mode == BY_WAVES) LQ.hit_slot = K.B.hit_slot;
+  closest_step<true, true>(mode, S, p.idx, n, p.n_dev, GVT_RAY_EPSILON, K.B.hits, LQ, K.d_long, p.pass > 0);
   ShadeArgs A = shade_args(K.B, p.idx, n, p.pass, p.n_dev, p.next, p.c_next, K.outp, K.out->d_count, P);
+  A.hit_slot = LQ.hit_slot;
   A.W = W; A.out_from = d_out_from; A.shadow_inst = K.d_shadow_inst; A.hop_inst = d_hop;
   const bool direct = C.shadow_direct && p.pass == 0 && !K.small;
   const bool direct_dev = direct && K.nd0 != nullptr && nL == 1;
@@ -602,6 +611,7 @@
   A.queue_overflow = d_queue_overflow; A.trav_overflow = C.d_counters + CW_TRAV_OVF;
   A.seed = P.seed; A.index_base = 0ull; A.skip_known = C.skip_known;
   A.count_ptr = d_count_ptr; A.clear_mask = d_mask; A.n_inst = W.n_inst;
+  A.hit_slot = C.hit_slot;
   {
     ProfScope ps(KC_CLOSEST);
     k_finish<<<(int)std::min<size_t>((n_total + 3) / 4, (size_t)C.n_cu * 4), 256, 0, C.stream>>>(A);
diff --git a/gravit_amd/csrc/trace_lane.inc b/gravit_amd/csrc/trace_lane.inc
--- a/gravit_amd/csrc/trace_lane.inc
+++ b/gravit_amd/csrc/trace_lane.inc
@@ -17,7 +17,7 @@
 
 #define LONG_SAVE 48
 #define LONG_STK_CAP 65536u
-struct LongRec { unsigned j, i; float bt; int bp; float bu, bv, bden; unsigned ns; };
+struct LongRec { unsigned j, i; float bt; int bp; float bu, bv, bden; unsigned ns; unsigned slot; };
 struct LongQ {
   LongRec *recs;
   unsigned *count;
@@ -26,6 +26,7 @@
   int steps;
   int steps_drain;
   unsigned char *steps_out;
+  unsigned *hit_slot;
 };
 
 typedef float f2 __attribute__((ext_vector_type(2)));
@@ -219,8 +220,10 @@
   const unsigned share_w = n / n_waves_total;
   const unsigned chunk = max(64u, ((share_w * (ANY ? 5u : 3u) / 8u) + 16u) & ~31u);
   const unsigned dyn = max(64u, (share_w / 16u) & ~63u);
-  __shared__ int stack[TRAV_STACK * TRAV_BLOCK];
+  constexpr bool PARK = !ANY && !MULTI;
+  __shared__ int stack[(TRAV_STACK + (PARK ? 4 : 0)) * TRAV_BLOCK];
   int *lds = &stack[threadIdx.x];
+#define KT_BEST(W) lds[(TRAV_STACK + (W)) * TRAV_BLOCK]
   int *spill_m = spill_base + (size_t)(blockIdx.x * TRAV_BLOCK + threadIdx.x) * TRAV_SPILL;
 #define KT_SPILL(K) (*(MULTI ? spill_m + (K) : kt_spill_ptr(spill_base, (K))))
   __shared__ KtInst s_inst[MULTI ? KT_TAB : 1];
@@ -257,7 +260,8 @@
   unsigned j = 0;
   V3 O = mk3(0, 0, 0), D = mk3(0, 0, 1);
   RaySlab S = make_slab(0.f, 0.f, 0.f, 0.f, 0.f, 0.f);
-  float bt = GVT_FLT_MAX, bu = 0.f, bv = 0.f, bden = 1.f;
+  float bt = GVT_FLT_MAX;
+  float bu = 0.f, bv = 0.f, bden = 1.f;
   int bp = -1, sp = 0, cur = TRAV_DONE;
   int sb = 0;
   bool sharing = false;
@@ -376,7 +380,8 @@
             const float dz = fabsf(D.z) < 1e-30f ? copysignf(1e-30f, D.z) : D.z;
             const float ix = 1.0f / dx, iy = 1.0f / dy, iz = 1.0f / dz;
             S = make_slab(ix, iy, iz, O.x * ix, O.y * iy, O.z * iz);
-            bt = GVT_FLT_MAX; bu = 0.f; bv = 0.f; bden = 1.f; bp = -1;
+            bt = GVT_FLT_MAX; bp = -1;
+            if (!PARK) { bu = 0.f; bv = 0.f; bden = 1.f; }
             sp = 0; sb = 0; nsteps = 0;
             cur = (MULTI ? nodes4_l : T.nodes4) != nullptr ? 0 : TRAV_DONE;
             active = true;
@@ -499,7 +504,11 @@
                   if (ANY) occluded = true;
                   else {
                     const int prim = __float_as_int(s0[k].w);
-                    if (bp < 0 || t < bt || (t == bt && prim < bp)) { bt = t; bp = prim; bu = U; bv = V; bden = aden; }
+                    if (bp < 0 || t < bt || (t == bt && prim < bp)) {
+                      bt = t; bp = prim;
+                      if (PARK) { KT_BEST(0) = (int)(first + kb + k); KT_BEST(1) = __float_as_int(U); KT_BEST(2) = __float_as_int(V); KT_BEST(3) = __float_as_int(aden); }
+                      else { bu = U; bv = V; bden = aden; }
+                    }
                   }
                 }
               }
@@ -599,7 +608,10 @@
         base = __shfl(base, __ffsll((long long)pm) - 1);
         if (fin && KT_PARKED) {
           const unsigned slot = base + lanes_below(pm);
-          LongRec R; R.j = j; R.i = MULTI ? gidx : (idx ? idx[j] : j); R.bt = bt; R.bp = bp; R.bu = bu; R.bv = bv; R.bden = bden; R.ns = 0u;
+          LongRec R; R.j = j; R.i = MULTI ? gidx : (idx ? idx[j] : j); R.bt = bt; R.bp = bp; R.ns = 0u;
+          const bool have = bp >= 0;
+          if (PARK) { R.slot = have ? (unsigned)KT_BEST(0) : 0u; R.bu = have ? __int_as_float(KT_BEST(1)) : 0.f; R.bv = have ? __int_as_float(KT_BEST(2)) : 0.f; R.bden = have ? __int_as_float(KT_BEST(3)) : 1.f; }
+          else { R.slot = 0u; R.bu = bu; R.bv = bv; R.bden = bden; }
           const int depth = sp - sb;
           if (LQ.stk && depth > 0 && depth <= LONG_SAVE && slot < LQ.stk_cap) {
             int *dst = LQ.stk + (size_t)slot * LONG_SAVE;
@@ -619,7 +631,11 @@
     if (fin) {
       if (ANY) { if (MODE == 0) flags[j] = (bp >= 0) ? 1 : 0; }
       else {
-        if (!KT_PARKED) { gvt_hip_hit h; h.t = bt; h.prim = bp; h.u = (bp >= 0) ? bu / bden : 0.f; h.v = (bp >= 0) ? bv / bden : 0.f; hits[j] = h; }
+        if (!KT_PARKED) {
+          if (PARK) { bu = __int_as_float(KT_BEST(1)); bv = __int_as_float(KT_BEST(2)); bden = __int_as_float(KT_BEST(3)); }
+          gvt_hip_hit h; h.t = bt; h.prim = bp; h.u = (bp >= 0) ? bu / bden : 0.f; h.v = (bp >= 0) ? bv / bden : 0.f; hits[j] = h;
+          if (PARK && LQ.hit_slot) LQ.hit_slot[j] = (unsigned)KT_BEST(0);
+        }
         if (LQ.steps_out) LQ.steps_out[j] = (unsigned char)(KT_PARKED ? 255 : min(nsteps, 254));
       }
       active = false;
@@ -636,4 +652,5 @@
 #undef KT_POP
 #undef KT_SPILL
 #undef KT_PARKED
-}
+#undef KT_BEST
+}
diff --git a/gravit_amd/csrc/trace_wave.inc b/gravit_amd/csrc/trace_wave.inc
--- a/gravit_amd/csrc/trace_wave.inc
+++ b/gravit_amd/csrc/trace_wave.inc
@@ -63,7 +63,7 @@
 
 template <bool ANY>
 __device__ __forceinline__ bool wave_leaves(const float4 *__restrict__ tris, V3 O, V3 D, float tnear, const WaveLists &L, int &nl,
-                                            float &bt, int &bp, float &bu, float &bv, float &bden) {
+                                            float &bt, int &bp, float &bu, float &bv, float &bden, unsigned &bs) {
   const int lane = (int)lane_id();
   const int take = min(nl, 64);
   const bool mine = lane < take;
@@ -74,6 +74,7 @@
   nl -= take;
   float lt = GVT_FLT_MAX, lu = 0.f, lv = 0.f, ld = 1.f;
   int lp = -1;
+  unsigned ls = 0u;
   bool hit_any = false;
   if (mine && (ANY || within_best(etn, bt))) {
     const unsigned code = (unsigned)~ref;
@@ -89,7 +90,7 @@
           if constexpr (ANY) hit_any = true;
           else {
             const int prim = __float_as_int(s0.w);
-            if (closer(t, prim, lt, lp)) { lt = t; lp = prim; lu = U; lv = V; ld = aden; }
+            if (closer(t, prim, lt, lp)) { lt = t; lp = prim; lu = U; lv = V; ld = aden; ls = first + k; }
           }
         }
       }
@@ -97,20 +98,23 @@
   }
   if constexpr (ANY) return ballot64(hit_any) != 0ull;
   if (ballot64(lp >= 0)) {
+    const int own = lp;
 #pragma unroll
     for (int off = 32; off >= 1; off >>= 1) {
       const float ot = __shfl_xor(lt, off), ou = __shfl_xor(lu, off), ov = __shfl_xor(lv, off), od = __shfl_xor(ld, off);
       const int op = __shfl_xor(lp, off);
       if (op >= 0 && closer(ot, op, lt, lp)) { lt = ot; lp = op; lu = ou; lv = ov; ld = od; }
     }
-    if (lp >= 0 && closer(lt, lp, bt, bp)) { bt = lt; bp = lp; bu = lu; bv = lv; bden = ld; }
+    const unsigned long long wm = ballot64(own == lp);
+    const unsigned ws = (unsigned)__builtin_amdgcn_readlane((int)ls, wm ? __ffsll((long long)wm) - 1 : 0);
+    if (lp >= 0 && closer(lt, lp, bt, bp)) { bt = lt; bp = lp; bu = lu; bv = lv; bden = ld; bs = ws; }
   }
   return false;
 }
 
 template <bool ANY, bool CLUSTER, int CAP, int PHYS>
 __device__ __forceinline__ bool wave_run(const uint4 *__restrict__ nodes, const float4 *__restrict__ tris, V3 O, V3 D, const RaySlab &S, float tnear, const WaveLists &L,
-                                          int ns, int nl, float &bt, int &bp, float &bu, float &bv, float &bden, unsigned *ovf_word) {
+                                          int ns, int nl, float &bt, int &bp, float &bu, float &bv, float &bden, unsigned &bs, unsigned *ovf_word) {
   using F = WaveFan<CLUSTER>;
   const int lane = (int)lane_id();
   bool occluded = false;
@@ -121,7 +125,7 @@
       take = max(take, 1);
       if (ns + F::NODES * take > PHYS || nl + F::LEAVES * take > PHYS) { if (lane == 0) atomicOr(ovf_word, 1u); break; }
       wave_nodes<ANY, CLUSTER>(nodes, S, L, take, ns, nl, bt);
-    } else occluded = wave_leaves<ANY>(tris, O, D, tnear, L, nl, bt, bp, bu, bv, bden);
+    } else occluded = wave_leaves<ANY>(tris, O, D, tnear, L, nl, bt, bp, bu, bv, bden, bs);
   }
   return occluded;
 }
@@ -132,7 +136,8 @@
   __builtin_amdgcn_wave_barrier();
   float bt = GVT_FLT_MAX, bu = 0.f, bv = 0.f, bden = 1.f;
   int bp = -1;
-  return wave_run<true, CLUSTER, CAP, PHYS>(nodes, tris, O, D, S, tnear, WaveLists{ s_ref, nullptr, l_ref, nullptr }, (CLUSTER || nodes) ? 1 : 0, 0, bt, bp, bu, bv, bden, ovf_word);
+  unsigned bs = 0u;
+  return wave_run<true, CLUSTER, CAP, PHYS>(nodes, tris, O, D, S, tnear, WaveLists{ s_ref, nullptr, l_ref, nullptr }, (CLUSTER || nodes) ? 1 : 0, 0, bt, bp, bu, bv, bden, bs, ovf_word);
 }
 __device__ __forceinline__ RaySlab slab_of(V3 O, V3 D) {
   const float dx = fabsf(D.x) < 1e-30f ? copysignf(1e-30f, D.x) : D.x;
@@ -152,7 +157,7 @@
 template <bool XFORM, bool MULTI = false>
 __global__ __launch_bounds__(256) void k_long_closest(RayPlanes q, const LongRec *__restrict__ recs, const unsigned *__restrict__ n_recs, Mat4 minv,
                                                        Trav T, float tnear, gvt_hip_hit *__restrict__ hits, unsigned *counter, WaveSet W = WaveSet{},
-                                                       const int *__restrict__ stk = nullptr, const int *__restrict__ hop_inst = nullptr) {
+                                                       const int *__restrict__ stk = nullptr, const int *__restrict__ hop_inst = nullptr, unsigned *__restrict__ hit_slot = nullptr) {
   __shared__ int s_ref_all[4][LONG_PHYS];
   __shared__ float s_tn_all[4][LONG_PHYS];
   __shared__ int l_ref_all[4][LONG_PHYS];
@@ -188,6 +193,7 @@
     const RaySlab S = slab_of(O, D);
     float bt = R.bt, bu = R.bu, bv = R.bv, bden = R.bden;
     int bp = R.bp;
+    unsigned bs = R.slot;
     int ns = T.nodes4 ? 1 : 0, nl = 0;
     if (stk && R.ns && T.nodes4) {
       const int e = lane < (int)R.ns ? stk[(size_t)r * LONG_SAVE + lane] : TRAV_DONE;
@@ -198,7 +204,8 @@
       ns = __popcll(mi); nl = __popcll(ml);
     } else if (lane == 0) { s_ref[0] = 0; s_tn[0] = 0.f; }
     __builtin_amdgcn_wave_barrier();
-    wave_run<false, false, LONG_CAP, LONG_PHYS>(T.nodes4, T.tris, O, D, S, tnear, WaveLists{ s_ref, s_tn, l_ref, l_tn }, ns, nl, bt, bp, bu, bv, bden, counter + (CW_TRAV_OVF - CW_LONG_WORK));
+    wave_run<false, false, LONG_CAP, LONG_PHYS>(T.nodes4, T.tris, O, D, S, tnear, WaveLists{ s_ref, s_tn, l_ref, l_tn }, ns, nl, bt, bp, bu, bv, bden, bs, counter + (CW_TRAV_OVF - CW_LONG_WORK));
+    if (hit_slot) hit_slot[R.j] = bs;
     { gvt_hip_hit h; h.t = bt; h.prim = bp; h.u = (bp >= 0) ? bu / bden : 0.f; h.v = (bp >= 0) ? bv / bden : 0.f; hits[R.j] = h; }
   }
 }
@@ -209,7 +216,7 @@
   const unsigned j = blockIdx.x * blockDim.x + threadIdx.x;
   if (j == 0) *count = n;
   if (j >= n) return;
-  LongRec R; R.j = j; R.i = idx ? idx[j] : j; R.bt = GVT_FLT_MAX; R.bp = -1; R.bu = 0.f; R.bv = 0.f; R.bden = 1.f; R.ns = 0u;
+  LongRec R; R.j = j; R.i = idx ? idx[j] : j; R.bt = GVT_FLT_MAX; R.bp = -1; R.bu = 0.f; R.bv = 0.f; R.bden = 1.f; R.ns = 0u; R.slot = 0u;
   recs[j] = R;
 }
 
```
